# gergely-flamich/relative-entropy-coding

Measured on AMD Instinct MI355X. Metric: encoded latents/sec, higher is better.
Workload: dtype f32

## Files before the change

relative-entropy-coding_amd/csrc/irec_host.cpp:

```cpp
#include <hip/hip_runtime.h>

#include <algorithm>
#include <atomic>
#include <exception>
#include <cfloat>
#include <cmath>
#include <cstdarg>
#include <cstdio>
#include <cstdlib>
#include <cstring>
#include <string>
#include <thread>
#include <vector>

#include "irec_internal.h"
#include "irec_kernels.h"

namespace {

thread_local std::string g_last_error;

irec_status fail(irec_status code, const char *fmt, ...) {
  char buf[512];
  va_list ap;
// ... 85 lines not shown
  const float first = z - logf_det(z) / z;
  const float rz = 1.0f / z;
  const float x_far = first - poly(rz, p2) / poly(rz, q2) / z;
  const float x_tail = first - poly(rz, p1) / poly(rz, q1) / z;
  const float x = sp > lo_cut ? x_centre : (z >= 8.0f ? x_far : x_tail);
  return p > hi_cut ? x : -x;
}

void tf_seed_pair(int64_t global_seed, int64_t op_seed, uint64_t &s1, uint64_t &s2) {
  const int64_t M = 2147483647LL;
  int64_t a = global_seed % M; if (a < 0) a += M;
  int64_t b = op_seed % M;     if (b < 0) b += M;
  if (a == 0 && b == 0) b = M;
  s1 = (uint64_t)a; s2 = (uint64_t)b;
}

struct Philox {
  uint32_t key[2], ctr[4];
  Philox(uint64_t seed1, uint64_t seed2) {
    key[0] = (uint32_t)seed1; key[1] = (uint32_t)(seed1 >> 32);
    ctr[0] = ctr[1] = 0; ctr[2] = (uint32_t)seed2; ctr[3] = (uint32_t)(seed2 >> 32);
  }
  void block(uint64_t index, uint32_t out[4]) const {
    uint32_t c0 = (uint32_t)index, c1 = (uint32_t)(index >> 32), c2 = ctr[2], c3 = ctr[3];
    uint32_t k0 = key[0], k1 = key[1];
    for (int r = 0; r < 10; ++r) {
      const uint64_t a = (uint64_t)0xD2511F53u * c0, b = (uint64_t)0xCD9E8D57u * c2;
      const uint32_t n0 = (uint32_t)(b >> 32) ^ c1 ^ k0, n2 = (uint32_t)(a >> 32) ^ c3 ^ k1;
      c1 = (uint32_t)b; c3 = (uint32_t)a; c0 = n0; c2 = n2;
      k0 += 0x9E3779B9u; k1 += 0xBB67AE85u;
    }
    out[0] = c0; out[1] = c1; out[2] = c2; out[3] = c3;
  }
  uint32_t element(uint64_t e) const {
    uint32_t o[4];
    block(e >> 2, o);
    return o[e & 3];
  }
};

struct MT19937 {
  uint32_t mt[624];
  int idx;
  void init_genrand(uint32_t s) {
    mt[0] = s;
    for (int i = 1; i < 624; ++i) mt[i] = 1812433253u * (mt[i - 1] ^ (mt[i - 1] >> 30)) + (uint32_t)i;
    idx = 624;
  }
  void init_by_array(const std::vector<uint32_t> &key) {
    init_genrand(19650218u);
    size_t i = 1, j = 0;
    for (size_t k = std::max<size_t>(624, key.size()); k; --k) {
      mt[i] = (mt[i] ^ ((mt[i - 1] ^ (mt[i - 1] >> 30)) * 1664525u)) + key[j] + (uint32_t)j;
      if (++i >= 624) { mt[0] = mt[623]; i = 1; }
      if (++j >= key.size()) j = 0;
    }
    for (size_t k = 623; k; --k) {
      mt[i] = (mt[i] ^ ((mt[i - 1] ^ (mt[i - 1] >> 30)) * 1566083941u)) - (uint32_t)i;
      if (++i >= 624) { mt[0] = mt[623]; i = 1; }
    }
    mt[0] = 0x80000000u;
  }
  uint32_t next() {
    if (idx >= 624) {
      for (int k = 0; k < 624; ++k) {
        const uint32_t y = (mt[k] & 0x80000000u) | (mt[(k + 1) % 624] & 0x7fffffffu);
        mt[k] = mt[(k + 397) % 624] ^ (y >> 1) ^ ((y & 1u) ? 0x9908b0dfu : 0u);
      }
      idx = 0;
    }
    uint32_t y = mt[idx++];
    y ^= y >> 11; y ^= (y << 7) & 0x9d2c5680u; y ^= (y << 15) & 0xefc60000u; y ^= y >> 18;
    return y;
  }
};

int64_t py_first_randint31(int64_t seed) {
  const uint64_t a = seed < 0 ? (uint64_t)(-(seed + 1)) + 1u : (uint64_t)seed;
  std::vector<uint32_t> key{(uint32_t)a};
  if (a >> 32) key.push_back((uint32_t)(a >> 32));
  MT19937 g;
  g.init_by_array(key);
  uint32_t r;
  do r = g.next(); while (r >= 0x80000000u);
  return (int64_t)r;
}

inline float u32_to_unit_float(uint32_t x) {
  const uint32_t bits = (127u << 23) | (x & 0x7fffffu);
  float f;
  std::memcpy(&f, &bits, 4);
  return f - 1.0f;
}
inline void box_muller(uint32_t x0, uint32_t x1, float &f0, float &f1) {
  float u1 = u32_to_unit_float(x0);
  if (u1 < 1.0e-7f) u1 = 1.0e-7f;
  const float v1 = (float)(2.0 * 3.14159265358979323846 * (double)u32_to_unit_float(x1));
  const float u2 = std::sqrt(-2.0f * std::log(u1));
  f0 = std::sin(v1) * u2;
  f1 = std::cos(v1) * u2;
}
struct TfNormalStream {
  Philox gen;
  uint64_t have = ~0ull;
  float f[4];
  explicit TfNormalStream(int64_t seed) : gen(0, 0) {
    uint64_t s1, s2;
    tf_seed_pair(seed, py_first_randint31(seed), s1, s2);
    gen = Philox(s1, s2);
  }
  float element(uint64_t e) {
    if ((e >> 2) != have) {
      uint32_t o[4];
      gen.block(e >> 2, o);
      box_muller(o[0], o[1], f[0], f[1]);
      box_muller(o[2], o[3], f[2], f[3]);
      have = e >> 2;
    }
    return f[e & 3];
  }
};

struct TfStatelessNormalStream {
  Philox gen;
  uint64_t have = ~0ull;
  float f[4];
  TfStatelessNormalStream(int64_t seed0, int64_t seed1) : gen(0, 0) {
    const Philox scramble(((uint64_t)0x02461e29u << 32) | 0x3ec8f720u, (uint64_t)seed1);
    uint32_t mix[4];
    scramble.block((uint64_t)seed0, mix);
    gen = Philox(((uint64_t)mix[1] << 32) | mix[0], ((uint64_t)mix[3] << 32) | mix[2]);
  }
  float element(uint64_t e) {
    if ((e >> 2) != have) {
      uint32_t o[4];
      gen.block(e >> 2, o);
      box_muller(o[0], o[1], f[0], f[1]);
      box_muller(o[2], o[3], f[2], f[3]);
      have = e >> 2;
    }
    return f[e & 3];
  }
};

int round_up(int v, int m) { return (v + m - 1) / m * m; }
size_t round_up_sz(size_t v, size_t m) { return (v + m - 1) / m * m; }

}

struct irec_context {
  int device = -1;
  int n_cu = 0;
  int clock_mhz = 0;
  float *d_lut = nullptr;
  float *d_lut2 = nullptr;
  uint16_t *d_dlog4r = nullptr;
  float *d_rho = nullptr;
  int32_t n_rho = IREC_MAX_PARTITIONS;
  unsigned long long *d_dbg = nullptr;
};

namespace irec {
irec_status set_last_error(irec_status code, const char *who, const char *what) { return fail(code, "%s: %s", who, what); }
int context_device(const irec_context *ctx) { return ctx->device; }
int context_cus(const irec_context *ctx) { return ctx->n_cu > 0 ? ctx->n_cu : 256; }
}

extern "C" {

const char *irec_last_error(void) { return g_last_error.c_str(); }
const char *irec_version(void) { return "irec-hip 0.1 (gfx950)"; }

int32_t irec_n_samples(double kl_per_partition, double extra_samples) {
  const double s = std::exp(kl_per_partition * extra_samples);
  if (!(s >= 0.0)) return 0;
  return s >= 2147483647.0 ? INT32_MAX : (int32_t)s;
}

double irec_codelength(int64_t n_indices, int32_t n_samples) { return (double)n_indices * std::log((double)n_samples); }

irec_status irec_build_lut(float *lut) {
  if (!lut) return fail(IREC_E_INVALID, "irec_build_lut: null output");
  lut[0] = 0.0f;
  for (int k = 1; k < IREC_BIG_PRIME; ++k) lut[k] = ndtri_f32((float)k / (float)IREC_BIG_PRIME);
  return IREC_OK;
}

irec_status irec_tf_shuffle_perm(int64_t seed, int64_t n, int64_t *perm) {
  if (n < 0 || (n > 0 && !perm)) return fail(IREC_E_INVALID, "irec_tf_shuffle_perm: bad arguments");
  if (n > 0xFFFFFFFFLL) return fail(IREC_E_INVALID, "irec_tf_shuffle_perm: n too large");
  for (int64_t i = 0; i < n; ++i) perm[i] = i;
  if (n <= 1) return IREC_OK;
  uint64_t s1, s2;
  tf_seed_pair(seed, py_first_randint31(seed), s1, s2);
  const Philox gen(s1, s2);
  uint32_t blk[4];
  for (int64_t i = 0; i < n - 1; ++i) {
    if ((i & 3) == 0) gen.block((uint64_t)i >> 2, blk);
    const int64_t j = i + (int64_t)(blk[i & 3] % (uint32_t)(n - i));
    std::swap(perm[i], perm[j]);
  }
  return IREC_OK;
}

irec_status irec_philox_uniform_int(int64_t seed, int64_t n, int32_t *out) {
  if (n < 0 || (n > 0 && !out)) return fail(IREC_E_INVALID, "irec_philox_uniform_int: bad arguments");
  uint64_t s1, s2;
  tf_seed_pair(seed, seed, s1, s2);
  const Philox gen(s1, s2);
  for (int64_t e = 0; e < n; ++e) out[e] = 1 + (int32_t)(gen.element((uint64_t)e) % (uint32_t)(IREC_BIG_PRIME - 1));
  return IREC_OK;
}

int64_t irec_importance_n_samples(double coding_bits) {
  const float n = std::ceil(std::exp((float)coding_bits * std::log(2.0f)));
  if (!(n >= 1.0f) || !(n < 2147483648.0f)) return -1;
  return (int64_t)n;
}

irec_status irec_tf_random_normal(int64_t seed, int64_t count, float *out) {
  if (count < 0 || (count > 0 && !out)) return fail(IREC_E_INVALID, "irec_tf_random_normal: bad arguments");
  TfNormalStream st(seed);
  for (int64_t e = 0; e < count; ++e) out[e] = st.element((uint64_t)e);
  return IREC_OK;
}

irec_status irec_tf_stateless_normal(int64_t seed0, int64_t seed1, int64_t count, float *out) {
  if (count < 0 || (count > 0 && !out)) return fail(IREC_E_INVALID, "irec_tf_stateless_normal: bad arguments");
  TfStatelessNormalStream st(seed0, seed1);
  for (int64_t e = 0; e < count; ++e) out[e] = st.element((uint64_t)e);
  return IREC_OK;
}

irec_status irec_importance_encode(const float *t_loc, const float *t_scale, const float *p_loc, const float *p_scale,
                                   int64_t n, double coding_bits, double alpha, int64_t seed, int64_t *out_index,
                                   float *out_sample) try {
  if (!t_loc || !t_scale || !p_loc || !p_scale || !out_index || !out_sample || n < 1)
    return fail(IREC_E_INVALID, "irec_importance_encode: bad arguments");
  if (!(alpha >= 1.0)) return fail(IREC_E_INVALID, "Alpha must be in the range [1, inf), but %g was given!", alpha);
  const int64_t S = irec_importance_n_samples(coding_bits);
  if (S < 1) return fail(IREC_E_INVALID, "irec_importance_encode: coding_bits %g gives no valid sample count", coding_bits);
  const float half_log_2pi = (float)(0.5 * std::log(2.0 * 3.14159265358979323846));
  std::vector<float> tl(n), ts(n), ln_t(n);
  for (int64_t d = 0; d < n; ++d) {
    tl[d] = (t_loc[d] - p_loc[d]) / p_scale[d];
    ts[d] = t_scale[d] / p_scale[d];
    ln_t[d] = half_log_2pi + std::log(ts[d]);
  }
  TfNormalStream st(seed);
  const bool gumbel = !std::isinf(alpha);
  TfStatelessNormalStream gst(seed + 1, seed + 2);
  float best = -FLT_MAX;
  int64_t best_s = 0;
  for (int64_t s = 0; s < S; ++s) {
    double acc = 0.0;
    for (int64_t d = 0; d < n; ++d) {
      const float x = st.element((uint64_t)(s * n + d));
      const float dt = x / ts[d] - tl[d] / ts[d];
      const float lp_t = -0.5f * (dt * dt) - ln_t[d];
      const float dp = x / 1.0f - 0.0f / 1.0f;
      const float lp_p = -0.5f * (dp * dp) - (half_log_2pi + 0.0f);
      acc += (double)(lp_t - lp_p);
    }
    float w = (float)acc;
    if (gumbel) w = (float)alpha * w + (-std::log(-std::log(gst.element((uint64_t)s))));
    if (w > best) { best = w; best_s = s; }
  }
  *out_index = best_s;
  for (int64_t d = 0; d < n; ++d) out_sample[d] = p_scale[d] * st.element((uint64_t)(best_s * n + d)) + p_loc[d];
  return IREC_OK;
} catch (const std::exception &e) { return fail(IREC_E_INVALID, "irec_importance_encode: %s", e.what()); }

irec_status irec_importance_decode(const float *p_loc, const float *p_scale, int64_t n, int64_t index, int64_t seed,
                                   float *out_sample) {
  if (!p_loc || !p_scale || !out_sample || n < 1 || index < 0)
    return fail(IREC_E_INVALID, "irec_importance_decode: bad arguments");
  TfNormalStream st(seed);
  for (int64_t d = 0; d < n; ++d) out_sample[d] = p_scale[d] * st.element((uint64_t)(index * n + d)) + p_loc[d];
  return IREC_OK;
}

irec_status irec_create(int device, irec_context **out) { return irec_create_ex(device, nullptr, out); }

irec_status irec_create_ex(int device, const float *lut10007, irec_context **out) {
  irec_tables t{};
  t.lut10007 = lut10007;
  return irec_create_with(device, &t, out);
}

int32_t irec_max_partitions(const irec_context *ctx) { return ctx ? ctx->n_rho : 0; }

irec_status irec_create_with(int device, const irec_tables *tables, irec_context **out) try {
  if (!out) return fail(IREC_E_INVALID, "irec_create: null output");
  *out = nullptr;
  const float *lut10007 = tables ? tables->lut10007 : nullptr;
  const float *aux_ratios = tables ? tables->aux_ratios : nullptr;
  const int32_t n_aux = tables ? tables->n_aux_ratios : 0;
  if (aux_ratios) {
    if (n_aux < 1 || n_aux > IREC_MAX_PARTITIONS) return fail(IREC_E_INVALID, "irec_create_with: n_aux_ratios %d out of range [1, %d]", n_aux, IREC_MAX_PARTITIONS);
    for (int i = 0; i < n_aux; ++i)
      if (!(aux_ratios[i] > 0.0f) || !(aux_ratios[i] <= 1.0f)) return fail(IREC_E_INVALID, "irec_create_with: aux_ratios[%d] is not in (0, 1]", i);
  } else if (n_aux != 0) return fail(IREC_E_INVALID, "irec_create_with: n_aux_ratios without aux_ratios");
  if (lut10007)
    for (int k = 1; k < IREC_BIG_PRIME; ++k)
      if (!std::isfinite(lut10007[k])) return fail(IREC_E_INVALID, "irec_create_ex: lut10007[%d] is not finite", k);
  int count = 0;
  if (hipGetDeviceCount(&count) != hipSuccess || count <= 0)
    return fail(IREC_E_NO_DEVICE, "irec_create: no HIP device visible (this library has no CPU fallback)");
  if (device < 0 || device >= count) return fail(IREC_E_INVALID, "irec_create: device %d out of range (%d)", device, count);
  hipDeviceProp_t prop;
  HIP_TRY(hipGetDeviceProperties(&prop, device));
  if (std::strncmp(prop.gcnArchName, "gfx950", 6) != 0)
    return fail(IREC_E_NO_DEVICE, "irec_create: device %d is %s; this build targets gfx950 only", device, prop.gcnArchName);
  IREC_ON_DEVICE(device);

  const int P = IREC_BIG_PRIME;
  std::vector<float> lut(P);
  if (lut10007) { std::memcpy(lut.data(), lut10007, (size_t)P * sizeof(float)); lut[0] = 0.0f; }
  else irec_build_lut(lut.data());
  auto mulmod = [&](uint32_t a, uint32_t b) { return (uint32_t)(((uint64_t)a * b) % P); };
  uint32_t g = 0;
  std::vector<uint32_t> powers(P - 1);
  for (uint32_t cand = 2; cand < (uint32_t)P && !g; ++cand) {
    uint32_t x = 1;
    bool ok = true;
    std::vector<char> seen(P, 0);
    for (int e = 0; e < P - 1; ++e) {
      if (seen[x]) { ok = false; break; }
      seen[x] = 1; powers[e] = x; x = mulmod(x, cand);
    }
    if (ok) g = cand;
  }
  if (!g) return fail(IREC_E_INVALID, "irec_create: no primitive root found");
  std::vector<float> lut2(P - 1);
  std::vector<uint16_t> dlog4r(P - 1);
  for (int e = 0; e < P - 1; ++e) {
    lut2[e] = lut[powers[e]];
    dlog4r[powers[e] - 1] = (uint16_t)(4 * e);
  }
  std::vector<float> rho(IREC_MAX_PARTITIONS);
  for (int i = 0; i < IREC_MAX_PARTITIONS; ++i)
    rho[i] = (float)std::pow((double)i + 1.0, -0.7864636765648174);
  if (aux_ratios)
    for (int i = 0; i < IREC_MAX_PARTITIONS; ++i) rho[i] = i < n_aux ? aux_ratios[i] : 1.0f;

  irec_context *ctx = new irec_context();
  ctx->device = device;
  ctx->n_cu = prop.multiProcessorCount;
  ctx->clock_mhz = prop.clockRate / 1000;
  ctx->n_rho = aux_ratios ? n_aux : IREC_MAX_PARTITIONS;
  const irec_status st = [&]() -> irec_status {
    HIP_TRY(hipMalloc(&ctx->d_lut, P * sizeof(float)));
    HIP_TRY(hipMalloc(&ctx->d_lut2, (P - 1) * sizeof(float)));
    HIP_TRY(hipMalloc(&ctx->d_dlog4r, (P - 1) * sizeof(uint16_t)));
    HIP_TRY(hipMalloc(&ctx->d_rho, rho.size() * sizeof(float)));
    HIP_TRY(hipMemcpy(ctx->d_lut, lut.data(), P * sizeof(float), hipMemcpyHostToDevice));
    HIP_TRY(hipMemcpy(ctx->d_lut2, lut2.data(), (P - 1) * sizeof(float), hipMemcpyHostToDevice));
    HIP_TRY(hipMemcpy(ctx->d_dlog4r, dlog4r.data(), (P - 1) * sizeof(uint16_t), hipMemcpyHostToDevice));
    HIP_TRY(hipMemcpy(ctx->d_rho, rho.data(), rho.size() * sizeof(float), hipMemcpyHostToDevice));
#ifdef IREC_HOST_STAMPS
    if (const char *e = std::getenv("IREC_STAMPS"); e && e[0] == '1') {
      HIP_TRY(hipMalloc(&ctx->d_dbg, 4096 * 16 * sizeof(unsigned long long)));
    }
#endif
    return IREC_OK;
  }();
  if (st != IREC_OK) { irec_destroy(ctx); return st; }
  *out = ctx;
  return IREC_OK;
} catch (const std::exception &e) { return fail(IREC_E_INVALID, "irec_create: %s", e.what()); }

void irec_destroy(irec_context *ctx) {
  if (!ctx) return;
  DeviceGuard guard_;
  (void)guard_.enter(ctx->device);
  (void)hipFree(ctx->d_lut); (void)hipFree(ctx->d_lut2); (void)hipFree(ctx->d_dlog4r); (void)hipFree(ctx->d_rho);
  (void)hipFree(ctx->d_dbg);
  delete ctx;
}

}

namespace {

struct Plan {
  bool fast;
  bool table;
  bool team;
  bool team_only;
  bool lone;
  bool chunk;
  int shape;
  int grid_cap;
  int one_grid_cap;
  int fast_grid_cap;
  size_t ws_per_wg;
  int dpad;
  int K_tab;
  int n_tab;
  int tab_dim[4];
  size_t tab_off[4];
  size_t tab_bytes;
  int gang_blocks;
  size_t gang_stride, gang_bytes;
};
size_t plan_ws_bytes(const Plan &pl) { return irec::WS_HEAD_BYTES + pl.tab_bytes + (size_t)pl.grid_cap * pl.ws_per_wg + pl.gang_bytes; }

size_t table_steps_that_fit(size_t per_step, bool big = false) {
  const size_t soft = (big ? (size_t)IREC_TABLE_BYTES_BIG : (size_t)IREC_TABLE_BYTES_MAX) / per_step;
  const size_t hard = (big ? (size_t)IREC_TABLE_BYTES_BIG : (size_t)IREC_TABLE_BYTES_HARD) / per_step;
  return std::max(soft, std::min<size_t>((size_t)IREC_TABLE_STEPS_FLOOR, hard));
}

irec_status check_params(const irec_params *p) {
  if (!p) return fail(IREC_E_INVALID, "null irec_params");
  if (!(p->kl_per_partition > 0.0f)) return fail(IREC_E_INVALID, "kl_per_partition must be > 0");
  if (p->n_samples < 1 || p->n_samples > (1 << 24)) return fail(IREC_E_INVALID, "n_samples %d out of range", p->n_samples);
  if (p->n_beams < 1 || p->n_beams > IREC_MAX_BEAMS) return fail(IREC_E_INVALID, "n_beams %d out of range [1,%d]", p->n_beams, IREC_MAX_BEAMS);
  if (p->table_steps < 0) return fail(IREC_E_INVALID, "table_steps %d < 0", p->table_steps);
  { const int sh = (p->flags & IREC_FLAG_SHAPE_MASK) >> IREC_FLAG_SHAPE_SHIFT;
    if (sh > 6 || sh == 1 || sh == 4) return fail(IREC_E_INVALID, "unknown IREC_FLAG_SHAPE_* value"); }
  return IREC_OK;
}

Plan make_plan(const irec_context *ctx, const irec_params *p, int32_t max_dim, int32_t max_K) {
  Plan pl;
  const int B = p->n_beams, S = p->n_samples;
  const int n_cu = ctx->n_cu > 0 ? ctx->n_cu : 256;
  pl.shape = (p->flags & IREC_FLAG_SHAPE_MASK) >> IREC_FLAG_SHAPE_SHIFT;
  pl.dpad = round_up(max_dim > 0 ? max_dim : 1, 256);
  pl.fast = !(p->flags & IREC_FLAG_FORCE_GENERIC) && max_dim <= irec::FAST_MAX_DIM && irec::fast_nb_for(B) != 0 &&
            irec::fast_lds_for(B, S, false) <= irec::FAST_LDS_LIMIT && (int64_t)S * B < (1 << 24);
  pl.grid_cap = 2 * n_cu;
  pl.table = false; pl.team = false; pl.lone = false; pl.chunk = false; pl.n_tab = 0; pl.tab_bytes = 0;
  pl.gang_blocks = 0; pl.gang_stride = 0; pl.gang_bytes = 0;
  const int want = p->table_steps > 0 ? p->table_steps : IREC_TABLE_STEPS_DEFAULT;
  pl.K_tab = std::max(1, std::min(std::min(want, IREC_TABLE_STEPS_MAX), max_K > 0 ? max_K : 1));
  {
    size_t per_step = 0;
    for (int q = 0; q < 4 && p->table_dims[q] > 0; ++q) per_step += (size_t)S * round_up(p->table_dims[q], 4) * 2;
    if (per_step > 0) pl.K_tab = std::max(1, (int)std::min<size_t>((size_t)pl.K_tab, table_steps_that_fit(per_step, max_dim > irec::FAST_MAX_DIM)));
  }
  pl.team_only = !pl.fast && !(p->flags & IREC_FLAG_FORCE_GENERIC) && max_dim <= irec::FAST_MAX_DIM && (int64_t)S * B < (1 << 24) &&
                 !(p->flags & (IREC_FLAG_FUSED_PHILOX | IREC_FLAG_ONE_TABLE)) && irec::team_lds_for(B, S, pl.shape) != (size_t)-1;
  if ((pl.fast || pl.team_only) && !(p->flags & IREC_FLAG_FUSED_PHILOX) && p->table_dims[0] > 0) {
    pl.table = true;
    for (int q = 0; q < 4 && p->table_dims[q] > 0; ++q) {
      if (p->table_dims[q] > irec::FAST_MAX_DIM) { pl.table = false; break; }
      pl.tab_dim[pl.n_tab] = p->table_dims[q];
      pl.tab_off[pl.n_tab] = pl.tab_bytes;
      pl.tab_bytes += round_up_sz((size_t)pl.K_tab * S * round_up(p->table_dims[q], 4) * 2, 256);
      ++pl.n_tab;
    }
    if (!pl.table) { pl.n_tab = 0; pl.tab_bytes = 0; }
    pl.team = pl.table && !(p->flags & IREC_FLAG_ONE_TABLE) && irec::team_lds_for(B, S, pl.shape) != (size_t)-1;
    if (pl.team_only && !pl.team) { pl.table = false; pl.n_tab = 0; pl.tab_bytes = 0; }
    if (pl.team) pl.grid_cap = std::max(irec::team_count_for(B, S, pl.shape), (p->flags & IREC_FLAG_NO_TEN) ? 0 : irec::team_ten_teams(B, S, pl.shape)) * n_cu;
    pl.lone = pl.team && irec::lone_applies(B, pl.shape);
  }
  if (!pl.table) pl.team_only = false;
  pl.chunk = !pl.fast && !pl.team_only && !(p->flags & (IREC_FLAG_FORCE_GENERIC | IREC_FLAG_FUSED_PHILOX | IREC_FLAG_ONE_TABLE)) &&
             p->table_dims[0] > 0 && irec::chunk_applies(B, S, max_dim);
  if (pl.chunk) {
    pl.table = true;
    for (int q = 0; q < 4 && p->table_dims[q] > 0; ++q) {
      if (p->table_dims[q] > max_dim) { pl.table = false; break; }
      pl.tab_dim[pl.n_tab] = p->table_dims[q];
      pl.tab_off[pl.n_tab] = pl.tab_bytes;
      pl.tab_bytes += round_up_sz((size_t)pl.K_tab * S * round_up(p->table_dims[q], 4) * 2, 256);
      ++pl.n_tab;
    }
    if (!pl.table) { pl.chunk = false; pl.n_tab = 0; pl.tab_bytes = 0; }
  }
  auto one_cap = [&](bool table) { return (irec::fast_waves_for(B, S, table) == 8 ? 1 : 2) * n_cu; };
  if (pl.fast) {
    pl.one_grid_cap = one_cap(pl.table);
    pl.fast_grid_cap = pl.table ? one_cap(false) : 0;
    if (!pl.team) pl.grid_cap = pl.one_grid_cap;
    pl.grid_cap = std::max(pl.grid_cap, pl.fast_grid_cap);
    pl.ws_per_wg = round_up_sz(irec::fast_ws_for(B, max_K) + (pl.team ? irec::team_ws_extra_for(B, S, pl.shape) : 0), 256);
    if (pl.team) pl.ws_per_wg = std::max(pl.ws_per_wg, round_up_sz(irec::team_ws_bytes_for(B, S, pl.shape, max_K), 256));
    if (pl.lone) pl.ws_per_wg = std::max(pl.ws_per_wg, round_up_sz(((size_t)n_cu * irec::lone_ws_bytes_per_wg() + pl.grid_cap - 1) / pl.grid_cap, 256));
  } else {
    const size_t generic_ws = round_up_sz((size_t)10 * pl.dpad * 4 + (size_t)3 * B * pl.dpad * 4 +
                                          (size_t)(max_K > 0 ? max_K : 1) * B * 4 + (size_t)S * B * 4, 256);
    if (pl.team_only) {
      pl.one_grid_cap = 0;
      pl.fast_grid_cap = 2 * n_cu;
      pl.grid_cap = std::max(pl.grid_cap, pl.fast_grid_cap);
      pl.ws_per_wg = std::max(generic_ws, round_up_sz(irec::team_ws_bytes_for(B, S, pl.shape, max_K), 256));
    } else if (pl.chunk) {
      pl.one_grid_cap = 0;
      pl.fast_grid_cap = 0;
      pl.ws_per_wg = round_up_sz(irec::chunk_ws_for(B, pl.dpad, max_K), 256);
      const int teams = irec::chunk_teams(B, S);
      const size_t fit = (size_t)IREC_SLAB_BYTES_MAX / pl.ws_per_wg;
      pl.grid_cap = (int)std::max<size_t>((size_t)teams, std::min<size_t>((size_t)teams * n_cu, fit / teams * teams));
      if (const int gnb = irec::chunk_gang_nb(B, S); gnb && irec::chunk_gang_teams(B, S) > 0 && !(p->flags & (IREC_FLAG_NO_SPLIT | IREC_FLAG_MARGINS))) {
        pl.gang_stride = irec::gang_xch_bytes(gnb, S, pl.dpad);
        pl.gang_blocks = (int)std::min<size_t>((size_t)irec::GANG_MAX_BLOCKS, irec::GANG_XCH_BYTES_MAX / pl.gang_stride);
        pl.gang_bytes = (size_t)pl.gang_blocks * pl.gang_stride;
      }
    } else {
      pl.one_grid_cap = pl.grid_cap; pl.fast_grid_cap = 0;
      pl.ws_per_wg = generic_ws;
    }
  }
  if (p->flags & IREC_FLAG_MARGINS) {
    const size_t generic_ws = round_up_sz((size_t)10 * pl.dpad * 4 + (size_t)3 * B * pl.dpad * 4 +
                                          (size_t)(max_K > 0 ? max_K : 1) * B * 4 + (size_t)S * B * 4, 256);
    pl.ws_per_wg = std::max(pl.ws_per_wg, generic_ws);
    pl.grid_cap = std::max(pl.grid_cap, 2 * n_cu);
    if (max_dim > irec::FAST_MAX_DIM)
      pl.grid_cap = (int)std::max<size_t>(1, std::min<size_t>((size_t)pl.grid_cap, (size_t)IREC_SLAB_BYTES_MAX / pl.ws_per_wg));
  }
  if (!pl.table) pl.K_tab = 0;
  return pl;
}

static int chunk_grid(const irec_context *ctx, const Plan &pl, const irec_params *p, int64_t n_blocks);

static int batch_grid(int64_t n_blocks, int cap) {
  const int64_t g = std::min<int64_t>(n_blocks, cap), r = (g + 7) & ~(int64_t)7;
  return (int)(r <= cap ? r : g);
}

static int chunk_grid(const irec_context *ctx, const Plan &pl, const irec_params *p, int64_t n_blocks) {
  const int n_cu = ctx->n_cu > 0 ? ctx->n_cu : 256;
  const int teams = std::max(1, irec::chunk_teams(p->n_beams, p->n_samples));
  return batch_grid(n_blocks, std::min(n_cu, std::max(1, pl.grid_cap / teams)));
}
int gang_width(const irec_context *ctx, const Plan &pl, const irec_params *p, int64_t n_blocks, int32_t max_block_dim, int *grid, int *chunk_owners) {
  if (!pl.chunk || pl.gang_blocks < 1 || n_blocks < 1 || n_blocks > pl.gang_blocks || (p->flags & (IREC_FLAG_NO_SPLIT | IREC_FLAG_MARGINS))) return 0;
  if (!irec::IREC_COOP_GRANULES_ON) return 0;
  const int n_cu = ctx->n_cu > 0 ? ctx->n_cu : 256;
  const int teams = irec::chunk_gang_teams(p->n_beams, p->n_samples);
  if (teams < 1) return 0;
  const int wgs = std::min(n_cu, std::max(1, pl.grid_cap / teams));
  const int64_t slots = (int64_t)wgs * teams;
  const int64_t chunks = ((int64_t)max_block_dim + 1023) >> 10;
  const int64_t GC = std::min(chunks, slots / n_blocks);
  if (GC < 1) return 0;
  const int want = (p->flags & IREC_FLAG_SPLIT_MASK) >> IREC_FLAG_SPLIT_SHIFT;
  const int64_t n_sch = irec::chunk_gang_nb(p->n_beams, p->n_samples) == 32 ? p->n_samples : (p->n_samples + 1) / 2;
  int64_t SP = std::min<int64_t>(wgs / (n_blocks * GC), want >= 1 ? want : IREC_GANG_STRIPES);
  SP = std::max<int64_t>(1, std::min<int64_t>(SP, n_sch));
  SP = (n_sch + (n_sch + SP - 1) / SP - 1) / ((n_sch + SP - 1) / SP);
  const int64_t G = GC * SP;
  if (G < 2) return 0;
  const int64_t n_slots = n_blocks * G;
  if (grid) *grid = (int)std::min<int64_t>(wgs, n_slots);
  if (chunk_owners) *chunk_owners = (int)GC;
  return (int)G;
}

int small_call_blocks(const irec_context *ctx) {
  const int n_cu = ctx->n_cu > 0 ? ctx->n_cu : 256;
  return std::max(8, std::min(irec::COOP_SPLIT_MAX_BLOCKS, n_cu / 4));
}

int split_width(const irec_context *ctx, const Plan &pl, const irec_params *p, int64_t n_blocks) {
  if (!pl.table || pl.chunk || (p->flags & IREC_FLAG_NO_SPLIT)) return 0;
  const int B = p->n_beams, S = p->n_samples, nb = irec::fast_nb_for(B);
  if (!nb || irec::fast_waves_for(B, S, true) != 4 || (int64_t)S * nb > 1024) return 0;
  if (n_blocks < 1 || n_blocks > irec::COOP_SPLIT_MAX_BLOCKS) return 0;
  const int n_cu = ctx->n_cu > 0 ? ctx->n_cu : 256;
  int64_t W = (n_cu / 2) / n_blocks;
  W = std::min<int64_t>(W, S);
  const int want = (p->flags & IREC_FLAG_SPLIT_MASK) >> IREC_FLAG_SPLIT_SHIFT;
  W = std::min<int64_t>(W, want >= 2 ? want : 12);
  return W >= 2 ? (int)W : 0;
}
int split_beam_width(const irec_params *p, int W) {
  if (W < 2) return 0;
  const int B = p->n_beams;
  if (W > B) W = B;
  if (W < 2) return 0;
  const int per = (B + W - 1) / W;
  if (per > 2) return 0;
  while (W > 2 && (B + (W - 1) - 1) / (W - 1) == per) --W;
  return W;
}

bool share_all_auto(const irec_context *ctx, const Plan &pl, const irec_params *p, int64_t n_blocks) {
  if (!pl.team || pl.lone || pl.team_only || pl.chunk || !pl.table || (p->flags & IREC_FLAG_NO_SPLIT)) return false;
  if ((p->flags & IREC_FLAG_SHAPE_MASK) != 0 || n_blocks < small_call_blocks(ctx) || n_blocks > irec::COOP_MAX_BLOCKS) return false;
  const int n_cu = ctx->n_cu > 0 ? ctx->n_cu : 256;
  const int B = p->n_beams, S = p->n_samples;
  if (B > 20 || irec::team_shareable(B, S, 2) != 2 || irec::team_lds_for(B, S, 2) == (size_t)-1 ||
      irec::team_ws_extra_for(B, S, 2) > irec::team_ws_extra_for(B, S, 0) || irec::team_count_for(B, S, 0) < 2)
    return false;
  const int64_t W = std::min<int64_t>(std::min<int64_t>(8, S), 2LL * n_cu / n_blocks);
  if (B <= 10 && !(p->flags & IREC_FLAG_NO_TEN) && irec::ten_applies(B, S)) return false;
  return B > 10 ? W >= 3 : (W >= 2 && n_blocks <= n_cu);
}
int team_share_width(const irec_context *ctx, const Plan &pl, const irec_params *p, int64_t n_blocks, int shape, int64_t *first, int *grid) {
  if (!pl.team || pl.lone || pl.team_only || (p->flags & IREC_FLAG_NO_SPLIT)) return 0;
  const int n_cu = ctx->n_cu > 0 ? ctx->n_cu : 256;
  const int teams = irec::team_shareable(p->n_beams, p->n_samples, shape);
  if (teams < 2) return 0;
  const int want = (p->flags & IREC_FLAG_SPLIT_MASK) >> IREC_FLAG_SPLIT_SHIFT;
  const int64_t cap = std::min<int64_t>(8, p->n_samples);
  const int64_t slots = (int64_t)teams * n_cu;
  int64_t W = 0, f = 0;
  if (shape == 2 && share_all_auto(ctx, pl, p, n_blocks)) {
    if (n_blocks < small_call_blocks(ctx) || n_blocks > irec::COOP_MAX_BLOCKS || 2 * n_blocks > slots) return 0;
    W = slots / n_blocks;
  } else {
    if (p->n_beams <= 10 || n_blocks <= n_cu || n_blocks >= slots || n_blocks - n_cu > irec::COOP_MAX_BLOCKS) return 0;
    f = n_cu;
    W = (slots - n_cu) / (n_blocks - n_cu);
  }
  W = std::min(W, cap);
  if (want >= 2) W = std::min<int64_t>(W, want);
  if (W < 2) return 0;
  const int64_t n_slots = f + (n_blocks - f) * W;
  int64_t g = n_cu;
  if (f == 0) { g = (n_slots + teams - 1) / teams; g = std::min<int64_t>(n_cu, (g + 7) & ~(int64_t)7); }
  if (g * teams < n_slots) return 0;
  if (first) *first = f;
  if (grid) *grid = (int)g;
  return (int)W;
}

int call_teams(const irec_params *p, int shape, int share_W, bool margins) {
  const int tt = (share_W >= 2 || margins || (p->flags & IREC_FLAG_NO_TEN)) ? 0 : irec::team_ten_teams(p->n_beams, p->n_samples, shape);
  return tt ? tt : irec::team_count_for(p->n_beams, p->n_samples, shape);
}
bool team_for_call(const irec_context *ctx, const Plan &pl, const irec_params *p, int64_t n_blocks) {
  return pl.team && (pl.team_only || (p->flags & IREC_FLAG_TEAM) || n_blocks >= small_call_blocks(ctx));
}
int shape_for_call(const irec_context *ctx, const Plan &pl, const irec_params *p, int64_t n_blocks) {
  const int n_cu = ctx->n_cu > 0 ? ctx->n_cu : 256;
  const int B = p->n_beams, S = p->n_samples;
  if (share_all_auto(ctx, pl, p, n_blocks)) return 2;
  if (pl.shape != 0 || !pl.team || pl.lone || n_blocks < small_call_blocks(ctx) || n_blocks > 2 * (int64_t)n_cu || B > 20) return pl.shape;
  if (irec::team_count_for(B, S, 0) < 2) return pl.shape;
  if (n_blocks <= n_cu && B <= 10) return pl.shape;
  if (n_blocks > n_cu) {
    if (irec::team_count_for(B, S, 0) < 3 || irec::team_lds_for(B, S, 2) == (size_t)-1 ||
        irec::team_ws_extra_for(B, S, 2) > irec::team_ws_extra_for(B, S, 0))
      return pl.shape;
    return 2;
  }
  if (irec::team_lds_for(B, S, 5) == (size_t)-1 || irec::team_ws_extra_for(B, S, 5) > irec::team_ws_extra_for(B, S, 0))
    return pl.shape;
  return 5;
}

int margin_team_shape(const irec_context *ctx, const Plan &pl, const irec_params *p, int64_t n_blocks) {
  if (!pl.table || !pl.team || pl.lone || pl.chunk || (p->flags & (IREC_FLAG_FORCE_GENERIC | IREC_FLAG_FUSED_PHILOX | IREC_FLAG_ONE_TABLE))) return -1;
  const int shape = shape_for_call(ctx, pl, p, n_blocks);
  if (irec::team_margin_build(p->n_beams, p->n_samples, shape)) return shape;
  if (irec::team_margin_build(p->n_beams, p->n_samples, pl.shape)) return pl.shape;
  return -1;
}

struct CallDetail {
  int kind = 0;
  int grid = 0;
  int teams = 1;
  int W = 0;
  int coop_beams = 0;
  int gang_chunks = 0;
  int64_t share_first = 0;
  int64_t n_slots = 0;
  int placed = 0;
  int split_blocks = 0;
};
CallDetail call_detail(const irec_context *ctx, const Plan &pl, const irec_params *p, int64_t n_blocks, int32_t max_block_dim, bool margins) {
  CallDetail d;
  const int n_cu = ctx->n_cu > 0 ? ctx->n_cu : 256;
  d.n_slots = n_blocks;
  if (pl.table && !pl.team && split_width(ctx, pl, p, n_blocks) >= 2) d.split_blocks = (int)n_blocks;
  int share_grid = 0;
  const int share_W = (pl.table && pl.team) ? team_share_width(ctx, pl, p, n_blocks, pl.shape, &d.share_first, &share_grid) : 0;
  if (share_W >= 2) d.split_blocks = (int)(n_blocks - d.share_first);
  if (pl.chunk && gang_width(ctx, pl, p, n_blocks, max_block_dim, nullptr, nullptr) >= 2) d.split_blocks = (int)n_blocks;
  if (pl.table && pl.chunk) {
    d.kind = 1;
    d.teams = std::max(1, irec::chunk_teams(p->n_beams, p->n_samples));
    d.grid = chunk_grid(ctx, pl, p, n_blocks);
    int ggrid = 0, gchunks = 0;
    if (const int G = gang_width(ctx, pl, p, n_blocks, max_block_dim, &ggrid, &gchunks)) {
      d.W = G; d.gang_chunks = gchunks; d.grid = ggrid; d.n_slots = n_blocks * G;
      d.teams = std::max(1, irec::chunk_gang_teams(p->n_beams, p->n_samples));
    }
  } else if (pl.table && pl.team && pl.lone) {
    d.kind = 2; d.grid = batch_grid(n_blocks, n_cu); d.teams = irec::lone_waves();
  } else if (pl.table && pl.team) {
    d.kind = 3;
    d.teams = call_teams(p, pl.shape, share_W, margins);
    d.grid = batch_grid(n_blocks, std::min(pl.grid_cap / d.teams, n_cu));
    if (share_W >= 2) {
      d.W = share_W; d.grid = share_grid; d.n_slots = d.share_first + (n_blocks - d.share_first) * share_W;
    }
    if (!pl.lone && !pl.chunk && !(p->flags & IREC_FLAG_LISTED_ORDER) && n_blocks <= irec::COST_MAX_ROWS) {
      const int n_teams = irec::team_count_for(p->n_beams, p->n_samples, pl.shape);
      const int64_t tg = share_W >= 2 ? share_grid : batch_grid(n_blocks, std::min(pl.grid_cap / n_teams, n_cu));
      if (n_blocks > tg && d.n_slots <= tg * n_teams && n_teams == 2 && p->n_beams > 10 && irec::team_placeable(p->n_beams, p->n_samples, pl.shape)) d.placed = 1;
    }
  } else if (pl.table) {
    d.kind = 4;
    d.grid = (int)std::min<int64_t>(n_blocks, pl.one_grid_cap);
    int W = split_width(ctx, pl, p, n_blocks);
    if (const int wb = split_beam_width(p, W)) { W = wb; d.coop_beams = 1; }
    if (W >= 2) { d.W = W; d.grid = (int)(n_blocks * W); d.n_slots = n_blocks * W; }
  } else if (pl.fast) {
    d.kind = 5; d.grid = (int)std::min<int64_t>(n_blocks, pl.one_grid_cap);
  } else {
    d.kind = 6;
    d.grid = margins ? (int)std::min<int64_t>(n_blocks, std::min(pl.grid_cap, 2 * n_cu)) : (int)std::min<int64_t>(n_blocks, pl.grid_cap);
  }
  return d;
}

}

extern "C" {

size_t irec_encode_workspace_bytes(const irec_context *ctx, const irec_params *p, int32_t max_dim, int32_t max_K) {
  if (!ctx || check_params(p) != IREC_OK || max_dim < 1 || max_K < 0) return 0;
  const Plan pl = make_plan(ctx, p, max_dim, max_K);
  return plan_ws_bytes(pl);
}

size_t irec_encode_workspace_bytes_for(const irec_context *ctx, const irec_params *p, int64_t n_blocks, int32_t max_dim, int32_t max_K) {
  if (!ctx || check_params(p) != IREC_OK || max_dim < 1 || max_K < 0 || n_blocks < 0) return 0;
  irec_params pm = *p;
  if (pm.flags & IREC_FLAG_MARGINS) pm.flags |= IREC_FLAG_NO_SPLIT;
  Plan pl = make_plan(ctx, &pm, max_dim, max_K);
  if (pl.chunk && !(pm.flags & IREC_FLAG_MARGINS) && n_blocks > 0) {
    const int teams = std::max(1, irec::chunk_teams(pm.n_beams, pm.n_samples));
    int grid = chunk_grid(ctx, pl, &pm, n_blocks), ggrid = 0;
    int gteams = teams;
    if (gang_width(ctx, pl, &pm, n_blocks, max_dim, &ggrid, nullptr) >= 2) { grid = ggrid; gteams = std::max(1, irec::chunk_gang_teams(pm.n_beams, pm.n_samples)); }
    pl.grid_cap = std::min(pl.grid_cap, std::max(teams, grid * std::max(teams, gteams)));
  }
  return plan_ws_bytes(pl);
}

irec_status irec_encode_plan(const irec_context *ctx, const irec_params *p, int64_t n_blocks, int32_t max_block_dim,
                             int32_t max_K, irec_plan_info *out) {
  if (!ctx || !out) return fail(IREC_E_INVALID, "irec_encode_plan: null argument");
  if (irec_status s = check_params(p)) return s;
  if (n_blocks < 0 || max_block_dim < 1 || max_K < 0) return fail(IREC_E_INVALID, "irec_encode_plan: bad sizes");
  irec_params pm = *p;
  if (pm.flags & IREC_FLAG_MARGINS) { pm.flags |= IREC_FLAG_NO_SPLIT; p = &pm; }
  const Plan pl = make_plan(ctx, p, max_block_dim, max_K);
  const bool team = team_for_call(ctx, pl, p, n_blocks);
  std::memset(out, 0, sizeof(*out));
  const int B = p->n_beams, S = p->n_samples;
  if (p->flags & IREC_FLAG_MARGINS) {
    const int n_cu = ctx->n_cu > 0 ? ctx->n_cu : 256;
    const int mshape = margin_team_shape(ctx, pl, p, n_blocks);
    if (mshape >= 0) {
      const int n_teams = irec::team_count_for(B, S, mshape);
      std::string nm = irec::team_kernel_name(B, S, mshape);
      nm.insert(nm.size() - 1, ",margins");
      std::snprintf(out->kernel, sizeof out->kernel, "%s", nm.c_str());
      std::snprintf(out->table_kernel, sizeof out->table_kernel, "prep_kernel (copy bits)");
      out->grid = batch_grid(n_blocks, std::min(pl.grid_cap / n_teams, n_cu));
      out->waves_per_wg = irec::team_waves_for(B, S, mshape);
      out->teams_per_wg = n_teams;
      out->lds_bytes = (int32_t)irec::team_lds_for(B, S, mshape);
      out->table_steps = pl.K_tab; out->n_tables = pl.n_tab; out->table_bytes = (int64_t)pl.tab_bytes;
    } else {
      std::snprintf(out->kernel, sizeof out->kernel, "encode_generic_kernel (margins)");
      out->grid = (int32_t)std::min<int64_t>(n_blocks, std::min(pl.grid_cap, 2 * n_cu));
      out->waves_per_wg = 4; out->teams_per_wg = 1;
      out->lds_bytes = (int32_t)irec::generic_lds_bytes();
    }
    out->n_cu = ctx->n_cu; out->clock_mhz = ctx->clock_mhz;
    out->workspace_bytes = (int64_t)plan_ws_bytes(pl);
    return IREC_OK;
  }
  if (pl.chunk) {
    std::snprintf(out->kernel, sizeof out->kernel, "%s", irec::chunk_kernel_name(B, S));
    std::snprintf(out->table_kernel, sizeof out->table_kernel, "prep_kernel (copy bits)");
    out->grid = chunk_grid(ctx, pl, p, n_blocks);
    {
      int ggrid = 0;
      out->split = gang_width(ctx, pl, p, n_blocks, max_block_dim, &ggrid, nullptr);
      if (out->split >= 2) out->grid = ggrid;
    }
    out->waves_per_wg = irec::chunk_teams(B, S) * 4;
    out->teams_per_wg = irec::chunk_teams(B, S);
    out->lds_bytes = (int32_t)irec::chunk_lds_for(B, S);
    if (out->split >= 2) {
      std::snprintf(out->kernel, sizeof out->kernel, "%s", irec::chunk_gang_kernel_name(B, S));
      out->teams_per_wg = irec::chunk_gang_teams(B, S); out->waves_per_wg = out->teams_per_wg * 4;
      out->lds_bytes = (int32_t)irec::chunk_gang_lds_for(B, S);
    }
  } else if (team && pl.lone) {
    const int n_cu = ctx->n_cu > 0 ? ctx->n_cu : 256;
    std::snprintf(out->kernel, sizeof out->kernel, "%s", irec::lone_kernel_name());
    std::snprintf(out->table_kernel, sizeof out->table_kernel, "prep_kernel (copy bits)");
    out->grid = batch_grid(n_blocks, n_cu);
    out->waves_per_wg = irec::lone_waves();
    out->teams_per_wg = irec::lone_waves();
    out->lds_bytes = (int32_t)irec::lone_lds_bytes();
  } else if (team) {
    const int shape = shape_for_call(ctx, pl, p, n_blocks);
    const int n_teams = irec::team_count_for(B, S, shape);
    const int n_cu = ctx->n_cu > 0 ? ctx->n_cu : 256;
    std::snprintf(out->kernel, sizeof out->kernel, "%s", irec::team_kernel_name(B, S, shape));
    std::snprintf(out->table_kernel, sizeof out->table_kernel, "prep_kernel (copy bits)");
    out->grid = batch_grid(n_blocks, std::min(pl.grid_cap / n_teams, n_cu));
    {
      int sgrid = 0;
      out->split = team_share_width(ctx, pl, p, n_blocks, shape, nullptr, &sgrid);
      if (out->split >= 2) out->grid = sgrid;
    }
    out->waves_per_wg = irec::team_waves_for(B, S, shape);
    out->teams_per_wg = n_teams;
    out->lds_bytes = (int32_t)irec::team_lds_for(B, S, shape);
    if (const int tt = irec::team_ten_teams(B, S, shape); tt && out->split < 2 && !(p->flags & IREC_FLAG_NO_TEN)) {
      std::snprintf(out->kernel, sizeof out->kernel, "encode_ten_kernel<%d>", tt);
      out->lds_bytes = (int32_t)irec::ten_lds_for(tt);
      out->teams_per_wg = tt; out->waves_per_wg = 4 * tt;
      out->grid = batch_grid(n_blocks, std::min(pl.grid_cap / tt, n_cu));
    }
  } else if (pl.fast) {
    std::snprintf(out->kernel, sizeof out->kernel, "%s", irec::fast_kernel_name(B, S, pl.table));
    if (pl.table) std::snprintf(out->table_kernel, sizeof out->table_kernel, "prep_kernel (plain rows)");
    out->grid = (int32_t)std::min<int64_t>(n_blocks, pl.one_grid_cap);
    out->split = split_width(ctx, pl, p, n_blocks);
    if (const int wb = split_beam_width(p, out->split)) { out->split = wb; out->split_beams = 1; }
    if (out->split >= 2) {
      out->grid = (int32_t)(n_blocks * out->split);
      std::snprintf(out->kernel, sizeof out->kernel, "encode_fast_kernel<%d,%d,true,%d>", irec::fast_nb_for(B),
                    out->split_beams ? irec::fast_split_beam_waves(B) : 4, out->split_beams ? 2 : 1);
    }
    out->waves_per_wg = (out->split >= 2 && out->split_beams) ? irec::fast_split_beam_waves(B) : irec::fast_waves_for(B, S, pl.table);
    out->teams_per_wg = 1;
    out->lds_bytes = (int32_t)irec::fast_lds_for(B, S, pl.table) + (out->split >= 2 && out->split_beams ? 40024 : 0);
  } else {
    std::snprintf(out->kernel, sizeof out->kernel, "encode_generic_kernel");
    out->grid = (int32_t)std::min<int64_t>(n_blocks, pl.grid_cap);
    out->waves_per_wg = 4;
    out->teams_per_wg = 1;
    out->lds_bytes = (int32_t)irec::generic_lds_bytes();
  }
  out->table_steps = pl.K_tab;
  out->n_tables = pl.n_tab;
  out->n_cu = ctx->n_cu;
  out->clock_mhz = ctx->clock_mhz;
  out->table_bytes = (int64_t)pl.tab_bytes;
  out->workspace_bytes = (int64_t)plan_ws_bytes(pl);
  return IREC_OK;
}

irec_status irec_test_plan(int32_t n_cu, int32_t clock_mhz, const irec_params *p, int64_t n_blocks, int32_t max_block_dim, int32_t max_K,
                           irec_plan_info *info, irec_plan_detail *detail) {
  if (!info || !detail || n_cu < 1) return fail(IREC_E_INVALID, "irec_test_plan: bad argument");
  irec_context fake;
  fake.n_cu = n_cu; fake.clock_mhz = clock_mhz;
  if (irec_status st = irec_encode_plan(&fake, p, n_blocks, max_block_dim, max_K, info)) return st;
  const bool margins = (p->flags & IREC_FLAG_MARGINS) != 0;
  irec_params pm = *p;
  if (margins) pm.flags |= IREC_FLAG_NO_SPLIT;
  Plan pl = make_plan(&fake, &pm, max_block_dim, max_K);
  const int mshape = margins ? margin_team_shape(&fake, pl, &pm, n_blocks) : -1;
  if (margins && mshape < 0) { pl.table = false; pl.team = false; pl.lone = false; pl.chunk = false; pl.fast = false; pl.team_only = false; pl.n_tab = 0; pl.K_tab = 0; }
  pl.team = mshape >= 0 ? true : team_for_call(&fake, pl, &pm, n_blocks);
  if (mshape >= 0) pl.shape = mshape;
  else if (pl.team) pl.shape = shape_for_call(&fake, pl, &pm, n_blocks);
  const CallDetail cd = call_detail(&fake, pl, &pm, n_blocks, max_block_dim, margins);
  std::memset(detail, 0, sizeof(*detail));
  detail->kind = cd.kind; detail->grid = cd.grid; detail->teams_per_wg = cd.teams; detail->coop_width = cd.W; detail->coop_beams = cd.coop_beams;
  detail->gang_chunks = cd.gang_chunks; detail->placed = cd.placed; detail->split_blocks = cd.split_blocks;
  detail->share_first = cd.share_first; detail->n_slots = cd.n_slots;
  detail->slabs_in_workspace = pl.grid_cap; detail->slab_bytes = (int64_t)pl.ws_per_wg;
  detail->fixed_bytes = (int64_t)(irec::WS_HEAD_BYTES + pl.tab_bytes + pl.gang_bytes);
  detail->exchange_rows = irec::COOP_MAX_BLOCKS; detail->exchange_keys = irec::COOP_KEYS;
  return IREC_OK;
}

irec_status irec_block_kl(irec_context *ctx, const irec_params *p, int64_t n_blocks, const int64_t *block_base,
                          const int32_t *block_pos, const int32_t *block_dim, const int32_t *perm, const float *q_loc,
                          const float *q_scale, const float *p_loc, const float *p_scale, float *out_kl, int32_t *out_K,
                          void *hip_stream) {
  if (!ctx) return fail(IREC_E_INVALID, "irec_block_kl: null context");
  if (irec_status s = check_params(p)) return s;
  if (n_blocks < 0) return fail(IREC_E_INVALID, "irec_block_kl: n_blocks < 0");
  if (n_blocks == 0) return IREC_OK;
  if (!block_base || !block_pos || !block_dim || !q_loc || !q_scale || !p_loc || !p_scale || !out_K)
    return fail(IREC_E_INVALID, "irec_block_kl: null pointer argument");
  IREC_ON_DEVICE(ctx->device);
  irec::EncArgs A{};
  A.block_base = block_base; A.block_pos = block_pos; A.block_dim = block_dim; A.perm = perm;
  A.q_loc = q_loc; A.q_scale = q_scale; A.p_loc = p_loc; A.p_scale = p_scale;
  A.n_blocks = n_blocks; A.omega = p->kl_per_partition; A.S = p->n_samples; A.B = p->n_beams; A.out_K = out_K;
  A.K_limit = ctx->n_rho;
  const int grid = (int)std::min<int64_t>(n_blocks, 8LL * ctx->n_cu);
  HIP_TRY(irec::launch_block_kl(A, out_kl, grid, (hipStream_t)hip_stream));
  return IREC_OK;
}

irec_status irec_beam_encode(irec_context *ctx, const irec_params *p, int64_t n_blocks, const int64_t *block_base,
                             const int32_t *block_pos, const int32_t *block_dim, int32_t max_block_dim,
                             const int32_t *perm, const float *q_loc, const float *q_scale, const float *p_loc,
                             const float *p_scale, int64_t seed, int32_t max_K, int32_t *out_K, int32_t *out_indices,
                             float *out_sample, void *workspace, size_t workspace_bytes, void *hip_stream) {
  if (p && (p->flags & IREC_FLAG_MARGINS)) return fail(IREC_E_INVALID, "irec_beam_encode: IREC_FLAG_MARGINS needs irec_beam_encode_ex (out_margin)");
  return irec_beam_encode_ex(ctx, p, n_blocks, block_base, block_pos, block_dim, max_block_dim, perm, q_loc, q_scale, p_loc, p_scale, seed,
                             max_K, out_K, out_indices, out_sample, nullptr, workspace, workspace_bytes, hip_stream);
}

irec_status irec_beam_encode_ex(irec_context *ctx, const irec_params *p, int64_t n_blocks, const int64_t *block_base,
                                const int32_t *block_pos, const int32_t *block_dim, int32_t max_block_dim,
                                const int32_t *perm, const float *q_loc, const float *q_scale, const float *p_loc,
                                const float *p_scale, int64_t seed, int32_t max_K, int32_t *out_K, int32_t *out_indices,
                                float *out_sample, float *out_margin, void *workspace, size_t workspace_bytes, void *hip_stream) {
  if (!ctx) return fail(IREC_E_INVALID, "irec_beam_encode: null context");
  if (irec_status s = check_params(p)) return s;
  if (((p->flags & IREC_FLAG_MARGINS) != 0) != (out_margin != nullptr))
    return fail(IREC_E_INVALID, "irec_beam_encode_ex: out_margin and IREC_FLAG_MARGINS go together (the flag sizes the workspace)");
  irec_params pm = *p;
  if (out_margin) { pm.flags |= IREC_FLAG_NO_SPLIT; p = &pm; }
  if (n_blocks < 0) return fail(IREC_E_INVALID, "irec_beam_encode: n_blocks < 0");
  if (n_blocks > 0x7FFF0000ll) return fail(IREC_E_INVALID, "irec_beam_encode: more than 2^31 - 65536 blocks in one call");
  if (n_blocks == 0) return IREC_OK;
  if (!block_base || !block_pos || !block_dim || !q_loc || !q_scale || !p_loc || !p_scale || !out_K || !out_sample)
    return fail(IREC_E_INVALID, "irec_beam_encode: null pointer argument");
  if (max_K < 0 || max_K > IREC_MAX_PARTITIONS) return fail(IREC_E_INVALID, "irec_beam_encode: max_K %d out of range", max_K);
  if (max_K > 0 && !out_indices) return fail(IREC_E_INVALID, "irec_beam_encode: null out_indices");
  if (max_block_dim < 1 || max_block_dim > (1 << 22)) return fail(IREC_E_INVALID, "irec_beam_encode: max_block_dim %d out of range", max_block_dim);
  Plan pl = make_plan(ctx, p, max_block_dim, max_K);
  size_t need = plan_ws_bytes(pl);
  if (workspace && workspace_bytes < need && pl.chunk && !out_margin) {
    const int teams = std::max(std::max(1, irec::chunk_teams(p->n_beams, p->n_samples)), std::max(1, irec::chunk_gang_teams(p->n_beams, p->n_samples)));
    const size_t fixed = irec::WS_HEAD_BYTES + pl.tab_bytes + pl.gang_bytes;
    const size_t fit = workspace_bytes > fixed ? (workspace_bytes - fixed) / pl.ws_per_wg : 0;
    if (fit >= (size_t)teams) { pl.grid_cap = (int)std::min<size_t>((size_t)pl.grid_cap, fit / teams * teams); need = plan_ws_bytes(pl); }
  }
  if (!workspace || workspace_bytes < need)
    return fail(IREC_E_WORKSPACE, "irec_beam_encode: workspace %zu bytes < required %zu", workspace_bytes, need);
  const int mshape = out_margin ? margin_team_shape(ctx, pl, p, n_blocks) : -1;
  if (out_margin && mshape < 0) { pl.table = false; pl.team = false; pl.lone = false; pl.chunk = false; pl.fast = false; pl.team_only = false; pl.n_tab = 0; pl.K_tab = 0; }
  pl.team = mshape >= 0 ? true : team_for_call(ctx, pl, p, n_blocks);
  if (((uintptr_t)workspace & 255) != 0) return fail(IREC_E_WORKSPACE, "irec_beam_encode: workspace must be 256-byte aligned");
  IREC_ON_DEVICE(ctx->device);
  hipStream_t st = (hipStream_t)hip_stream;
  irec::EncArgs A{};
  A.block_base = block_base; A.block_pos = block_pos; A.block_dim = block_dim; A.perm = perm;
  A.q_loc = q_loc; A.q_scale = q_scale; A.p_loc = p_loc; A.p_scale = p_scale;
  A.n_blocks = n_blocks; A.seed = seed;
  A.omega = p->kl_per_partition; A.S = p->n_samples; A.B = p->n_beams; A.max_K = max_K;
  A.K_limit = ctx->n_rho;
  A.out_K = out_K; A.out_indices = out_indices; A.out_sample = out_sample;
  A.lut = ctx->d_lut; A.lut2 = ctx->d_lut2; A.dlog4r = ctx->d_dlog4r; A.rho = ctx->d_rho;
  A.counter = (unsigned int *)workspace;
  A.xcd_counter = (unsigned int *)workspace + irec::WS_XCD_WORD;
  A.defer_count = (unsigned int *)workspace + 1;
  if (mshape >= 0) pl.shape = mshape;
  else if (pl.team) pl.shape = shape_for_call(ctx, pl, p, n_blocks);
  A.K_tab = pl.K_tab; A.deferred_pass = 0; A.shape_override = pl.shape; A.no_ten = (p->flags & IREC_FLAG_NO_TEN) ? 1 : 0;
  A.coop_W = 1; A.coop_err = (unsigned int *)workspace + 3; A.coop_arrive = (unsigned int *)workspace + 64;
  A.coop_xch = (uint32_t *)((char *)workspace + irec::WS_COUNTER_BYTES);
  A.ws = (char *)workspace + irec::WS_HEAD_BYTES + pl.tab_bytes;
  A.ws_per_wg = pl.ws_per_wg;
  A.max_dim_pad = pl.dpad;
  A.out_margin = out_margin;
  irec::TableStamps stamps{};
  if (pl.table)
    for (int q = 0; q < pl.n_tab; ++q) {
      uint32_t *w = stamps.w[q];
      w[0] = 0x7ab1e000u | ((pl.team || pl.chunk) ? 1u : 2u);
      w[1] = (uint32_t)(uint64_t)seed; w[2] = (uint32_t)((uint64_t)seed >> 32);
      w[3] = (uint32_t)p->n_samples; w[4] = (uint32_t)pl.tab_dim[q]; w[5] = (uint32_t)pl.K_tab;
      w[6] = (uint32_t)pl.tab_off[q];
      w[7] = ~(w[1] ^ w[2] ^ w[3] ^ w[4] ^ w[5] ^ w[6]);
    }
  stamps.reuse = (p->flags & IREC_FLAG_REUSE_TABLES) ? 1 : 0;
  const CallDetail cd = call_detail(ctx, pl, p, n_blocks, max_block_dim, out_margin != nullptr);
  const int split_blocks = cd.split_blocks;
  if (cd.placed) A.row_cost = (const uint32_t *)((char *)workspace + irec::WS_COUNTER_BYTES + irec::WS_XCH_BYTES);
  int grid = (int)std::min<int64_t>(n_blocks, pl.one_grid_cap);
  A.dbg = nullptr;
#ifdef IREC_HOST_STAMPS
  A.dbg = ctx->d_dbg;
  if (ctx->d_dbg) HIP_TRY(hipMemsetAsync(ctx->d_dbg, 0, 4096 * 16 * sizeof(unsigned long long), st));
#endif
  irec::PrepArgs P{};
  P.head = (uint32_t *)workspace; P.ts = stamps;
  P.n_granule = irec::IREC_COOP_GRANULES_ON && split_blocks > 0 ? std::min(split_blocks, irec::COOP_MAX_BLOCKS) : 0;
  P.n_cost = A.row_cost ? (int32_t)n_blocks : 0;
  P.cost = const_cast<uint32_t *>(A.row_cost);
  P.seed = seed; P.S = p->n_samples; P.K_tab = pl.K_tab; P.dlog4r = ctx->d_dlog4r;
  A.ws_head = (uint32_t *)workspace;
  for (int q = 0; q < 4; ++q) { A.tab[q] = nullptr; A.tab_dim[q] = -1; }
  if (pl.table) {
    for (int q = 0; q < pl.n_tab; ++q) {
      uint16_t *tab = (uint16_t *)((char *)workspace + irec::WS_HEAD_BYTES + pl.tab_off[q]);
      A.tab[q] = tab; A.tab_dim[q] = pl.tab_dim[q];
      P.jobs.tab[q] = tab; P.jobs.keep[q] = nullptr;
    }
    if (pl.n_tab > 0 && !(p->flags & IREC_FLAG_TABLES_PRESENT)) {
      P.table_kind = (pl.team || pl.chunk) ? 1 : 2;
      P.n_table_wgs = (int32_t)irec::prep_table_wgs(P.table_kind, p->n_samples, pl.K_tab, pl.n_tab, pl.tab_dim, &P.jobs);
    }
  }
  HIP_TRY(irec::launch_prep(P, A, st));
  if (pl.table) {
    auto deferred_pass = [&]() -> irec_status {
      if (pl.K_tab >= max_K) return IREC_OK;
      irec::EncArgs A2 = A;
      A2.deferred_pass = 1; A2.coop_W = 1;
      A2.counter = (unsigned int *)workspace + 2;
      for (int q = 0; q < 4; ++q) { A2.tab[q] = nullptr; A2.tab_dim[q] = -1; }
      if (out_margin) HIP_TRY(irec::launch_encode_generic(A2, (int)std::min<int64_t>(n_blocks, std::min(pl.grid_cap, 2 * (ctx->n_cu > 0 ? ctx->n_cu : 256))), st));
      else if (pl.team_only || pl.chunk) HIP_TRY(irec::launch_encode_generic(A2, (int)std::min<int64_t>(n_blocks, pl.fast_grid_cap), st));
      else HIP_TRY(irec::launch_encode_fast(A2, false, (int)std::min<int64_t>(n_blocks, pl.fast_grid_cap), st));
      return IREC_OK;
    };
    if (pl.chunk) {
      const int cgrid = cd.grid;
      if (cd.W >= 2) {
        A.coop_W = cd.W; A.gang_chunks = cd.gang_chunks;
        A.gang_xch = (char *)workspace + irec::WS_HEAD_BYTES + pl.tab_bytes + (size_t)pl.grid_cap * pl.ws_per_wg;
        A.gang_stride = pl.gang_stride;
        A.coop_test_orphan = (p->flags & IREC_FLAG_TEST_SPLIT_ORPHAN) ? 1 : 0;
      }
      HIP_TRY(irec::launch_encode_chunk(A, cgrid, st));
    } else if (pl.team && pl.lone) {
      HIP_TRY(irec::launch_encode_lone(A, cd.grid, st));
      if (irec_status s2 = deferred_pass()) return s2;
#ifdef IREC_HOST_STAMPS
      if (ctx->d_dbg) {
        const int lgrid = batch_grid(n_blocks, ctx->n_cu > 0 ? ctx->n_cu : 256), nwv = irec::lone_waves();
        std::vector<unsigned long long> h((size_t)lgrid * nwv * 16);
        HIP_TRY(hipStreamSynchronize(st));
        HIP_TRY(hipMemcpy(h.data(), ctx->d_dbg, h.size() * sizeof(unsigned long long), hipMemcpyDeviceToHost));
        static const char *nm[6] = {"prologue (fetch, KL)", "step constants", "scoring", "selection", "update", "epilogue"};
        double sum[6] = {0}, tot = 0;
        for (size_t w = 0; w < (size_t)lgrid * nwv; ++w) for (int k = 0; k < 6; ++k) { sum[k] += (double)h[w * 16 + k]; tot += (double)h[w * 16 + k]; }
        fprintf(stderr, "[irec lone stamps] share of wave time:\n");
        for (int k = 0; k < 6; ++k) fprintf(stderr, "  %-22s %5.1f%%\n", nm[k], 100 * sum[k] / tot);
        fprintf(stderr, "  cycles per wave: %.0f\n", tot / (lgrid * nwv));
        return IREC_OK;
      }
#endif
    } else if (pl.team) {
      const int tgrid = cd.grid;
#ifdef IREC_HOST_STAMPS
      const int n_teams = cd.teams;
#endif
      if (cd.W >= 2) {
        A.coop_W = cd.W; A.tsplit_first = cd.share_first;
        A.coop_test_orphan = (p->flags & IREC_FLAG_TEST_SPLIT_ORPHAN) ? 1 : 0;
      }
      if (out_margin) HIP_TRY(irec::launch_encode_team_margin(A, tgrid, st));
      else HIP_TRY(irec::launch_encode_team(A, tgrid, st));
#ifndef IREC_HOST_STAMPS
      if (irec_status s2 = deferred_pass()) return s2;
#else
      if (!ctx->d_dbg) { if (irec_status s2 = deferred_pass()) return s2; }
      if (ctx->d_dbg) {
        const bool ten_call = !cd.W && !out_margin && !(p->flags & IREC_FLAG_NO_TEN) && irec::team_ten_teams(p->n_beams, p->n_samples, pl.shape) != 0;
        const int nwv = ten_call ? 4 * n_teams : irec::team_waves_for(p->n_beams, p->n_samples, pl.shape);
        std::vector<unsigned long long> h((size_t)tgrid * nwv * 16);
        HIP_TRY(hipStreamSynchronize(st));
        HIP_TRY(hipMemcpy(h.data(), ctx->d_dbg, h.size() * sizeof(unsigned long long), hipMemcpyDeviceToHost));
        static const char *nm[12] = {"fetch", "prologue", "scoring", "wait-score", "combine", "select", "update-tail", "wait-update", "epilogue",
                                     "upd:sel+issue+consts", "upd:batches", "-"};
        const int nwt = nwv / n_teams;
        double w0[12] = {0}, wo[12] = {0}, t0 = 0, to = 0;
        int n0 = 0, no = 0;
        for (int w = 0; w < tgrid * nwv; ++w) {
          if (h[(size_t)w * 16 + 1] == 0ull) continue;
          if ((w % nwt) == 0) ++n0; else ++no;
          for (int k = 0; k < 12; ++k) { const double v = (double)h[(size_t)w * 16 + k]; if ((w % nwt) == 0) { w0[k] += v; t0 += v; } else { wo[k] += v; to += v; } }
        }
        fprintf(stderr, "[irec team stamps] %d of %d teams coded blocks; share of wave time (cycles per wave), wave 0 of a team | the others:\n", n0, tgrid * n_teams);
        t0 -= w0[11]; to -= wo[11];
        for (int k = 0; k < 11; ++k) fprintf(stderr, "  %-20s %5.1f%% (%8.0f) | %5.1f%% (%8.0f)\n", nm[k], 100 * w0[k] / t0, w0[k] / (n0 ? n0 : 1), 100 * wo[k] / to, wo[k] / (no ? no : 1));
        fprintf(stderr, "  cycles per wave: %.0f | %.0f;  block-steps per wave: %.2f;  cycles per block-step: %.0f\n", t0 / (n0 ? n0 : 1), to / (no ? no : 1),
                w0[11] / (n0 ? n0 : 1), w0[11] > 0 ? t0 / w0[11] : 0.0);
        {
          double life_max = 0, life_sum = 0, life_min = 1e300;
          int nlife = 0;
          for (int w = 0; w < tgrid * nwv; ++w) {
            const double v = (double)h[(size_t)w * 16 + 12];
            if (v <= 0) continue;
            life_max = std::max(life_max, v); life_min = std::min(life_min, v); life_sum += v; ++nlife;
          }
          if (nlife) fprintf(stderr, "  idle tail: %.1f%% of the grid's wave-time lies behind a wave's exit (first exit at %.1f%% of the longest lifetime)\n",
                             100.0 * (1.0 - life_sum / (nlife * life_max)), 100.0 * life_min / life_max);
        }
        if (h[13]) fprintf(stderr, "  shader clock of workgroup 0, wave 0: %.0f MHz over %.3f ms (s_memtime / s_memrealtime)\n",
                           100.0 * (double)h[12] / (double)h[13], (double)h[13] / 1e5);
        return IREC_OK;
      }
#endif
    } else {
      const int W = cd.W;
      A.coop_beams = cd.coop_beams;
      if (W >= 2) {
        A.coop_W = W;
        A.coop_test_orphan = (p->flags & IREC_FLAG_TEST_SPLIT_ORPHAN) ? 1 : 0;
        HIP_TRY(irec::launch_encode_fast(A, true, cd.grid, st));
#ifdef IREC_HOST_STAMPS
        if (ctx->d_dbg) grid = cd.grid;
#endif
      } else HIP_TRY(irec::launch_encode_fast(A, true, grid, st));
      if (irec_status s2 = deferred_pass()) return s2;
    }
  } else if (pl.fast) {
    HIP_TRY(irec::launch_encode_fast(A, false, grid, st));
  } else {
    if (out_margin) grid = (int)std::min<int64_t>(n_blocks, std::min(pl.grid_cap, 2 * (ctx->n_cu > 0 ? ctx->n_cu : 256)));
    HIP_TRY(irec::launch_encode_generic(A, grid, st));
  }
#ifdef IREC_HOST_STAMPS
  if (ctx->d_dbg) {
    std::vector<unsigned long long> h((size_t)grid * 16);
    HIP_TRY(hipStreamSynchronize(st));
    HIP_TRY(hipMemcpy(h.data(), ctx->d_dbg, h.size() * sizeof(unsigned long long), hipMemcpyDeviceToHost));
    double sum[16] = {0};
    for (int w = 0; w < grid; ++w) for (int k = 0; k < 16; ++k) sum[k] += (double)h[(size_t)w * 16 + k];
    const double tot = sum[0] + sum[1] + sum[2] + sum[3];
    {
      int zero = 0; unsigned long long t0 = ~0ull, late = 0;
      for (int w = 0; w < grid; ++w) { if (h[(size_t)w * 16 + 4] == 0) ++zero; else if (h[(size_t)w * 16 + 5] < t0) t0 = h[(size_t)w * 16 + 5]; }
      for (int w = 0; w < grid; ++w) if (h[(size_t)w * 16 + 4] && h[(size_t)w * 16 + 5] - t0 > 100000ull) ++late;
      fprintf(stderr, "[irec stamps] census: %d of %d workgroups coded no block, %llu started > 1 ms after the first\n", zero, grid, late);
    }
    fprintf(stderr, "[irec stamps] top-B detail cycles/WG: combine %.0f, wait-for-keys barrier %.0f, wave-0 select %.0f, closing barrier %.0f\n",
            sum[11] / grid, sum[8] / grid, sum[9] / grid, sum[10] / grid);
    if (sum[12] + sum[13] + sum[14] > 0)
      fprintf(stderr, "[irec stamps] split exchange cycles/WG: publish %.0f, wait for partners %.0f, read back %.0f\n",
              sum[12] / grid, sum[13] / grid, sum[14] / grid);
    fprintf(stderr, "[irec stamps] waves/workgroup %d, LDS %zu B\n",
            irec::fast_waves_for(p->n_beams, p->n_samples, pl.table), irec::fast_lds_for(p->n_beams, p->n_samples, pl.table));
    fprintf(stderr, "[irec stamps] %s grid=%d cycles/WG: prologue %.0f (%.1f%%) scoring %.0f (%.1f%%) select %.0f (%.1f%%) update %.0f (%.1f%%)\n",
            pl.table ? "table" : pl.fast ? "fused" : "generic", grid, sum[0] / grid, 100 * sum[0] / tot, sum[1] / grid,
            100 * sum[1] / tot, sum[2] / grid, 100 * sum[2] / tot, sum[3] / grid, 100 * sum[3] / tot);
  }
#endif
  return IREC_OK;
}

struct DecPlan { int upb; int K_tab; int n_tab; int tab_dim[4]; size_t tab_off[4]; size_t bytes; };
static DecPlan make_dec_plan(const irec_params *p, int64_t n_blocks, int32_t max_block_dim, int32_t max_K, bool have_ws) {
  DecPlan d{};
  int maxd = max_block_dim;
  for (int q = 0; q < 4 && p->table_dims[q] > 0; ++q) maxd = std::max(maxd, p->table_dims[q]);
  d.upb = maxd > 0 ? (maxd + 255) / 256 : 0;
  if (!have_ws || p->table_dims[0] <= 0 || max_K < 1 || (p->flags & IREC_FLAG_FUSED_PHILOX)) return d;
  if (n_blocks >= 0 && (int64_t)p->n_samples > 2 * n_blocks) return d;
  size_t per_step = 0;
  for (int q = 0; q < 4 && p->table_dims[q] > 0; ++q) per_step += (size_t)p->n_samples * round_up(p->table_dims[q], 4) * 2;
  const int want = p->table_steps > 0 ? p->table_steps : IREC_TABLE_STEPS_DEFAULT;
// ... 299 lines not shown
```

relative-entropy-coding_amd/csrc/irec_internal.h:

```cpp
#ifndef IREC_INTERNAL_H_
#define IREC_INTERNAL_H_

#include "irec.h"

#ifdef __cplusplus
extern "C" {
#endif

#define IREC_FLAG_FUSED_PHILOX 2
#define IREC_FLAG_ONE_TABLE 4
#define IREC_FLAG_TEAM 8
#define IREC_FLAG_TEST_SPLIT_ORPHAN 32
#define IREC_FLAG_LISTED_ORDER 262144
#define IREC_FLAG_NO_TEN 1048576
#define IREC_FLAG_SPLIT_SHIFT 12
#define IREC_FLAG_SPLIT_MASK (0xF << IREC_FLAG_SPLIT_SHIFT)
#define IREC_FLAG_SHAPE_SHIFT 8
#define IREC_FLAG_SHAPE_MASK (0xF << IREC_FLAG_SHAPE_SHIFT)
#define IREC_FLAG_SHAPE_2 (2 << IREC_FLAG_SHAPE_SHIFT)
#define IREC_FLAG_SHAPE_3 (3 << IREC_FLAG_SHAPE_SHIFT)
#define IREC_FLAG_SHAPE_1X2 (5 << IREC_FLAG_SHAPE_SHIFT)
#define IREC_FLAG_SHAPE_TEAM (6 << IREC_FLAG_SHAPE_SHIFT)


typedef struct {
  int32_t kind, grid, teams_per_wg;
  int32_t coop_width;
  int32_t coop_beams, gang_chunks;
  int32_t placed;
  int32_t split_blocks;
  int64_t share_first, n_slots;
  int64_t slabs_in_workspace, slab_bytes, fixed_bytes;
  int32_t exchange_rows, exchange_keys;
} irec_plan_detail;
irec_status irec_test_plan(int32_t n_cu, int32_t clock_mhz, const irec_params *p, int64_t n_blocks, int32_t max_block_dim, int32_t max_K,
                           irec_plan_info *info, irec_plan_detail *detail);
irec_status irec_tf_random_normal(int64_t seed, int64_t count, float *out);
irec_status irec_tf_stateless_normal(int64_t seed0, int64_t seed1, int64_t count, float *out);

int32_t irec_test_fit_chunk(int32_t chunk);
irec_status irec_test_det_exp(const double *in, int64_t n, double *out);

irec_status irec_shim_stats(irec_context *ctx, const float *y, const float *infer_heads, float *out, int32_t n_stats, int32_t n,
                            int32_t channels_y, int32_t channels_infer, int32_t stochastic, int32_t hw, const float *bias_y,
                            const float *bias_infer, void *hip_stream);
irec_status irec_shim_cat_elu(irec_context *ctx, const float *y, const float *latent, float *out, int32_t n, int32_t channels_y,
                              int32_t channel_offset, int32_t deterministic, int32_t stochastic, int32_t hw, const float *bias_y,
                              void *hip_stream);
irec_status irec_shim_residual_elu(irec_context *ctx, const float *input, const float *tensor, float alpha, float *out, float *out_elu,
                                   int32_t n, int32_t channels, int32_t hw, const float *bias_tensor, void *hip_stream);

irec_status irec_device_uniform_int(irec_context *ctx, int64_t seed, int64_t n, int32_t *out, void *hip_stream);
irec_status irec_test_decoder_sqrt(irec_context *ctx, uint64_t *out2, void *hip_stream);
irec_status irec_test_reduce_scatter(irec_context *ctx, const float *in, float *out, int32_t width, void *hip_stream);
irec_status irec_test_select(irec_context *ctx, const float *scores, int32_t n, int32_t n_select, int32_t n_beams_cur,
                             uint32_t *scratch_keys, int32_t *out_sel, void *hip_stream);
irec_status irec_test_select_quick(irec_context *ctx, const float *scores, int32_t n, int32_t n_select, int32_t n_beams_cur,
                                   uint32_t *scratch_keys, int32_t *out_sel, void *hip_stream);
irec_status irec_test_proposal_table(irec_context *ctx, int64_t seed, int32_t n_samples, int32_t dim, int32_t n_steps,
                                     uint16_t *out_tab, void *hip_stream);
irec_status irec_device_tables(irec_context *ctx, const float **lut, const float **lut2, const uint16_t **dlog4r,
                               const float **rho);

#ifdef __cplusplus
}
#endif
#endif
```

relative-entropy-coding_amd/csrc/irec_kernels.h:

```cpp
#pragma once
#include <hip/hip_runtime.h>
#include <stddef.h>
#include <stdint.h>

#define IREC_MAX_PARTITIONS_DEV 65536

namespace irec {

constexpr int FAST_NW = 4;
constexpr int FAST_MAX_DIM = 1024;
constexpr size_t FAST_LDS_LIMIT = 160 * 1024;

struct EncArgs {
  const int64_t *block_base; const int32_t *block_pos; const int32_t *block_dim; const int32_t *perm;
  const float *q_loc, *q_scale, *p_loc, *p_scale;
  int64_t n_blocks; int64_t seed;
  float omega; int32_t S, B, max_K;
  int32_t K_limit;
  int32_t *out_K; int32_t *out_indices; float *out_sample;
  const float *lut;
  const float *lut2;
  const uint16_t *dlog4r;
  const float *rho;
  unsigned int *counter; char *ws; size_t ws_per_wg; int32_t max_dim_pad;
  unsigned int *xcd_counter;
  const uint16_t *tab[4]; int32_t tab_dim[4];
  int32_t K_tab; int32_t deferred_pass; unsigned int *defer_count;
  int32_t shape_override;
  int32_t no_ten;
  int32_t coop_W; unsigned int *coop_arrive; uint32_t *coop_xch; unsigned int *coop_err;
  int64_t tsplit_first;
  const uint32_t *row_cost;
  uint32_t *ws_head;
  char *gang_xch; size_t gang_stride;
  int32_t gang_chunks;
  int32_t coop_beams;
  int32_t coop_test_orphan;
  float *out_margin;
  unsigned long long *dbg;
};

struct DecArgs {
  const int64_t *block_base; const int32_t *block_pos; const int32_t *block_dim; const int32_t *perm;
  const float *p_loc, *p_scale;
  int64_t n_blocks; int64_t seed;
  int32_t max_K; const int32_t *K; const int32_t *indices; float *out_sample;
  int32_t K_limit;
  const float *lut; const float *rho;
  int32_t upb; int32_t S; int32_t K_tab;
  const float *lut2; const uint16_t *dlog4r;
  const uint16_t *tab[4]; int32_t tab_dim[4];
  int64_t n_tensors; int32_t tn, tbs, tbpt; const int32_t *block_row;
};

hipError_t launch_block_kl(const EncArgs &A, float *out_kl, int grid, hipStream_t st);
size_t generic_lds_bytes();
hipError_t launch_encode_generic(const EncArgs &A, int grid, hipStream_t st);
int fast_nb_for(int B);
size_t fast_lds_for(int B, int S, bool table);
size_t fast_ws_for(int B, int max_K);
size_t fast_ws_bytes_nb(int NB, int max_K);
hipError_t launch_encode_fast(const EncArgs &A, bool table, int grid, hipStream_t st);
int fast_waves_for(int B, int S, bool table);
int fast_split_beam_waves(int B);
hipError_t launch_alpha_table(int64_t seed, int32_t S, int32_t D, int32_t K_tab, const uint16_t *dlog4r, uint16_t *tab,
                              const uint32_t *keep, hipStream_t st);
int team_count_for(int B, int S, int shape_override);
int team_shareable(int B, int S, int shape_override);
bool team_placeable(int B, int S, int shape_override);
int team_waves_for(int B, int S, int shape_override);
size_t team_ws_extra_for(int B, int S, int shape_override);
size_t team_ws_bytes_for(int B, int S, int shape_override, int max_K);
size_t team_lds_for(int B, int S, int shape_override);
hipError_t launch_encode_team(const EncArgs &A, int grid, hipStream_t st);
bool team_margin_build(int B, int S, int shape_override);
hipError_t launch_encode_team_margin(const EncArgs &A, int grid, hipStream_t st);
const char *team_kernel_name(int B, int S, int shape_override);
const char *fast_kernel_name(int B, int S, bool table);
hipError_t launch_alpha_choice(int64_t seed, int32_t S, int32_t D, int32_t K_tab, const uint16_t *dlog4r, uint16_t *tab,
                               const uint32_t *keep, hipStream_t st);
hipError_t launch_alpha_choice_all(int64_t seed, int32_t S, int32_t K_tab, const uint16_t *dlog4r, int n, const int32_t *dims,
                                   uint16_t *const *tabs, const uint32_t *const *keeps, hipStream_t st);
bool ten_applies(int B, int S);
size_t ten_lds_for(int teams);
hipError_t launch_encode_ten(const EncArgs &A, int teams, int grid, hipStream_t st);
int team_ten_teams(int B, int S, int shape_override);
bool chunk_applies(int B, int S, int max_dim);
int chunk_teams(int B, int S);
size_t chunk_lds_for(int B, int S);
size_t chunk_ws_for(int B, int dpad, int max_K);
const char *chunk_kernel_name(int B, int S);
int chunk_gang_teams(int B, int S);
int chunk_gang_nb(int B, int S);
size_t chunk_gang_lds_for(int B, int S);
const char *chunk_gang_kernel_name(int B, int S);
hipError_t launch_encode_chunk_gang(const EncArgs &A, int grid, hipStream_t st);
hipError_t launch_encode_chunk(const EncArgs &A, int grid, hipStream_t st);
bool lone_applies(int B, int shape_override);
int lone_waves();
size_t lone_lds_bytes();
size_t lone_ws_bytes_per_wg();
const char *lone_kernel_name();
hipError_t launch_encode_lone(const EncArgs &A, int grid, hipStream_t st);
constexpr int WS_KEEP_WORD = 8, WS_STAMP_WORD = 16, WS_STAMP_WORDS = 8, WS_XCD_WORD = 128, WS_XCD_STRIDE = 64;
constexpr int WS_PENDING_WORD = 132;
struct TableStamps { uint32_t w[4][WS_STAMP_WORDS]; int32_t reuse; };
struct ChoiceJobs { int32_t D[4]; uint16_t *tab[4]; const uint32_t *keep[4]; int64_t hw_end[4]; int32_t n; };
struct PrepArgs {
  uint32_t *head; TableStamps ts;
  int32_t n_granule, n_cost, n_table_wgs, table_kind;
  int64_t seed; int32_t S, K_tab; const uint16_t *dlog4r; ChoiceJobs jobs; uint32_t *cost;
};
hipError_t launch_prep(const PrepArgs &P, const EncArgs &A, hipStream_t st);
int64_t prep_table_wgs(int kind, int32_t S, int32_t K_tab, int n, const int32_t *dims, ChoiceJobs *jobs);
constexpr size_t WS_COUNTER_BYTES = 512 + 8 * 256;
constexpr int COOP_MAX_BLOCKS = 384, COOP_KEYS = 1024;
constexpr unsigned long long COOP_GIVE_UP_TICKS = 10000000ull;
constexpr int COOP_SPLIT_MAX_BLOCKS = 64;
#ifndef IREC_COOP_GRANULES
#define IREC_COOP_GRANULES 1
#endif
constexpr bool IREC_COOP_GRANULES_ON = IREC_COOP_GRANULES != 0;
constexpr size_t WS_XCH_BYTES = (size_t)2 * COOP_MAX_BLOCKS * COOP_KEYS * 8;
__host__ __device__ inline size_t gang_xch_bytes(int nb, int S, int dpad) {
  const size_t NGm = (size_t)4 * (((size_t)dpad + 1023) >> 10), NC_ = (size_t)S * nb;
  return (4 * NGm * (NC_ + nb) + 8 * NGm + 4 * NC_ + 255) & ~(size_t)255;
}
#ifndef IREC_GANG_STRIPES
#define IREC_GANG_STRIPES 9
#endif
constexpr int GANG_MAX_BLOCKS = COOP_MAX_BLOCKS;
constexpr size_t GANG_XCH_BYTES_MAX = (size_t)1 << 30;
constexpr int COST_MAX_ROWS = 1024;
constexpr size_t WS_COST_BYTES = (size_t)COST_MAX_ROWS * 4;
constexpr size_t WS_HEAD_BYTES = WS_COUNTER_BYTES + WS_XCH_BYTES + WS_COST_BYTES;
hipError_t launch_decode(const DecArgs &A, int n_cu, hipStream_t st);
int decode_tensor_waves(int n, int bs, bool table, size_t *lds_out);
hipError_t launch_shim_stats(const float *y, const float *inf, float *out, int n_stats, int N, int Cy, int Ci, int s, int HW,
                             const float *by, const float *bi, hipStream_t st);
hipError_t launch_shim_cat_elu(const float *y, const float *latent, float *out, int N, int Cy, int c_off, int d, int s, int HW,
                               const float *by, hipStream_t st);
hipError_t launch_shim_residual_elu(const float *inp, const float *t, float alpha, float *out, float *out_elu, int64_t count,
                                    const float *bt, int C, int HW, hipStream_t st);
constexpr int GC_MAX_DIM = 1024;
struct GcArgs {
  const int64_t *block_base; const int32_t *block_pos; const int32_t *block_dim; const int32_t *perm;
  const float *q_loc, *q_scale, *p_loc, *p_scale;
  int64_t n_blocks;
  int32_t S, S_pad, steps, max_K;
  int32_t K_limit;
  const float *rho;
  const float *tab[4]; int32_t tab_dim[4];
  int32_t *out_K; int32_t *out_indices;
  const int32_t *K; const int32_t *indices;
  float *out_sample;
};
int gc_encode_threads(int S);
hipError_t launch_gc_importance_encode(const GcArgs &A, int grid, hipStream_t st);
hipError_t launch_gc_importance_decode(const GcArgs &A, int grid, hipStream_t st);
hipError_t launch_dec_sqrt_test(unsigned long long *out, hipStream_t st);
hipError_t launch_uniform_int(int64_t seed, int64_t n, int32_t *out, hipStream_t st);
hipError_t launch_select_test(const float *scores, int N, int Bnew, int Bcur, uint32_t *keys, int32_t *sel, bool quick, hipStream_t st);
hipError_t launch_reduce_scatter_test(const float *in, float *out, int width, hipStream_t st);

}
```

relative-entropy-coding_amd/csrc/irec_team.hip:

```cpp
#include <hip/hip_runtime.h>
#include <algorithm>
#include <stdint.h>
#include <stdio.h>

#include "irec_device.h"
#include "irec_kernels.h"
#include "irec_fast_common.h"
#include "irec_team_common.h"

#ifndef IREC_GANG_ABLATE
#define IREC_GANG_ABLATE 0
#endif
#ifndef IREC_PK_ADDR
#define IREC_PK_ADDR 1
#endif
#if defined(IREC_TEAM_MARGIN_TU) || defined(IREC_TEAM_GANG_TU)
#define IREC_TEAM_AUX_TU 1
#endif
namespace irec {

__host__ __device__ constexpr int team_mb(int NB) { return NB <= 32 ? 32 : 64; }
template <int NB> using TeamLdsT = SmallLdsT<(NB <= 32 ? 32 : 64), (NB <= 32 ? 32 : 64), (NB <= 32 ? 64 : 512)>;
__host__ __device__ inline size_t team_small_bytes(int NB) {
  return NB <= 32 ? ((sizeof(TeamLdsT<32>) + 15) & ~(size_t)15) : ((sizeof(TeamLdsT<64>) + 15) & ~(size_t)15);
}
__host__ __device__ inline int team_row(int NB, int B) { return (NB == 10 && B == 1) ? 1 : NB; }
__host__ __device__ inline size_t team_key_bytes(int ps, int S) { return (((size_t)S * ps * 4) + 15) & ~(size_t)15; }
__host__ __device__ inline bool team_keys_in_lds(int NB, int S, int teams, bool passes, int ps = 0) {
  if (ps <= 0) ps = NB;
  const long long avail = (long long)((FAST_LDS_LIMIT - T3_BYTES) / (size_t)teams) - (long long)team_key_bytes(ps, S) -
                          (long long)team_small_bytes(NB) - 32;
  return (teams > 1 && !passes) || avail / (4LL * ps * 4) >= (S < 16 ? S : 16);
}
__host__ __device__ inline bool team_keys_alias(int NB, int teams) { return teams >= 3 && NB == 20; }
__host__ __device__ inline int team_s_pass(int NB, int S, int teams, int cmax, bool passes = false, int ps = 0) {
  if (ps <= 0) ps = NB;
  const long long avail = (long long)((FAST_LDS_LIMIT - T3_BYTES) / (size_t)teams) -
                          ((team_keys_in_lds(NB, S, teams, passes, ps) && !(team_keys_alias(NB, teams) && !passes)) ? (long long)team_key_bytes(ps, S) : 0) -
                          (long long)team_small_bytes(NB) - 32;
  long long fit = avail / (4LL * ps * 4);
  if (fit > cmax / ps) fit = cmax / ps;
  if (fit < 1) return 0;
  if (fit >= S) return S;
  const int n_pass = (int)((S + fit - 1) / fit);
  return (S + n_pass - 1) / n_pass;
}
__host__ __device__ inline size_t team_part_bytes(int ps, int SP) { return (((size_t)4 * SP * ps * 4) + 15) & ~(size_t)15; }
__host__ __device__ inline size_t team_lds_one(int NB, int S, int SP, int teams, bool passes = false, int ps = 0) {
  if (ps <= 0) ps = NB;
  return team_part_bytes(ps, SP) + ((team_keys_in_lds(NB, S, teams, passes, ps) && !(team_keys_alias(NB, teams) && !passes)) ? team_key_bytes(ps, S) : 0) +
         team_small_bytes(NB) + 16;
}
__host__ __device__ inline size_t team_lds_total(int NB, int S, int SP, int teams, bool passes = false, int ps = 0) {
  return T3_BYTES + (size_t)teams * team_lds_one(NB, S, SP, teams, passes, ps);
}

#ifdef IREC_TEAM_STAMPS
#define TSTAMP(slot) do { const unsigned long long now_ = __builtin_amdgcn_s_memtime(); st_acc[slot] += now_ - st_prev; st_prev = now_; } while (0)
#else
#define TSTAMP(slot) do { } while (0)
#endif

template <int NB, int TEAMS, int BS, bool PASSES = false, bool ONE = false, bool SHARE = false, bool MARGIN = false>
__global__ __launch_bounds__(TEAMS * BS * TEAM_NT, 1) void encode_team_kernel(EncArgs A) {
  using TeamLds = TeamLdsT<NB>;
  constexpr int TEAM_MB = team_mb(NB);
  constexpr size_t TEAM_SMALL_BYTES = (sizeof(TeamLds) + 15) & ~(size_t)15;
  constexpr bool MULTI_PASS = TEAMS == 1 || PASSES;
  constexpr bool SHORT = TEAMS * BS >= 3 && NB / BS == 20;
  constexpr int NW = TEAM_NW;
  constexpr int NWT = TEAM_NW * BS, NT = 64 * NWT;
  constexpr int NBW = NB / BS;
  static_assert(NB % BS == 0, "beam stripes must divide the beam count");
  static_assert(NBW == 10 || NBW == 16 || NBW == 18 || NBW == 20, "the team encoder is built for 10, 16, 18 or 20 beams per wave");
  static_assert(NB <= TEAM_MB && NB <= 64, "beam indices are lane indices and 6-bit back-pointers");
  constexpr int CMAX = TEAMS == 1 ? 2048 : 1024;
  constexpr int SPC = BS >= 2 ? 1 : 20 / NBW;
  constexpr int RW = NBW * SPC;
  constexpr int ACC_ROOM = rsn_room(RW);
  extern __shared__ __attribute__((aligned(16))) char smem[];
  const int S = A.S, B = A.B;
  const int lane = threadIdx.x & 63;
  const int wave_wg = __builtin_amdgcn_readfirstlane((int)(threadIdx.x >> 6));
  const int team = wave_wg / NWT, wave_t = wave_wg % NWT;
  const int wave = wave_t & 3, bs = wave_t >> 2;
  const int b_lo = bs * NBW;
  const int tid = (int)threadIdx.x - team * NT;
  const int PS = NB == 10 ? team_row(NB, B) : NB;
  const int SP = MULTI_PASS ? team_s_pass(NB, S, TEAMS, CMAX, PASSES, PS) : S;
  const bool keys_lds = !MULTI_PASS || team_keys_in_lds(NB, S, TEAMS, PASSES, PS);
  constexpr bool KEYS_ALIAS = TEAMS >= 3 && NB == 20 && !PASSES;
  const size_t key_lds_bytes = (keys_lds && !KEYS_ALIAS) ? team_key_bytes(PS, S) : 0;
  char *tbase = smem + T3_BYTES + (size_t)team * team_lds_one(NB, S, SP, TEAMS, PASSES, PS);
  float *part_s = reinterpret_cast<float *>(tbase);
  TeamLds *sm = reinterpret_cast<TeamLds *>(tbase + team_part_bytes(PS, SP) + key_lds_bytes);
  uint32_t *bar_word = reinterpret_cast<uint32_t *>(tbase + team_part_bytes(PS, SP) + key_lds_bytes + TEAM_SMALL_BYTES);
  double *gpart = sm->gpart;
  int32_t *sel_s = sm->sel_s, *sel_b = sm->sel_b;
  int32_t *hsum = &sm->hsum[0][0];
  uint32_t *beta4 = &sm->beta4[0][0];
  int32_t *misc = sm->misc;
  float *cpart_s = &sm->cpart[0][0];
  const uint16_t *dlog_s = A.dlog4r;
  const int rs_p = rsn_owner<RW>(lane);
  const int rs_p20 = RW == 20 ? rs20_owner(lane) : -1;
  const int rs_c = rsn_owner<NBW>(lane);

  if ((uint32_t)(uintptr_t)(__attribute__((address_space(3))) char *)smem != 0u) __builtin_trap();
  commit_table_stamps(A);
  constexpr bool CAN_SHARE = SHARE && TEAMS >= 2 && BS == 1 && !PASSES && !ONE;
  const int Wsh = (CAN_SHARE && A.coop_W > 1) ? A.coop_W : 1;
  const int64_t n_whole = Wsh > 1 ? (A.tsplit_first < A.n_blocks ? A.tsplit_first : A.n_blocks) : A.n_blocks;
  const int64_t n_slots = n_whole + (A.n_blocks - n_whole) * Wsh;
  const int64_t n_static = (int64_t)TEAMS * (int64_t)gridDim.x < n_slots ? (int64_t)TEAMS * (int64_t)gridDim.x : n_slots;
  constexpr bool CAN_PLACE = NB == 20 && TEAMS == 2 && BS == 1 && !PASSES && !ONE;
  const bool placed = CAN_PLACE && A.row_cost != nullptr && n_static == n_slots;
  const int64_t lo_rank = (int64_t)gridDim.x < n_whole ? (int64_t)gridDim.x : n_whole;
  int32_t placed_row = -1;
  if (placed) {
    uint32_t *cs = reinterpret_cast<uint32_t *>(smem);
    const int n = (int)A.n_blocks;
    for (int k = (int)threadIdx.x; k < n; k += TEAMS * NT) cs[k] = A.row_cost[k];
    if ((int)threadIdx.x < TEAMS) cs[n + (int)threadIdx.x] = 0xFFFFFFFFu;
    int want[TEAMS];
#pragma unroll
    for (int tm = 0; tm < TEAMS; ++tm) {
      const int64_t u = (int64_t)tm * (int64_t)gridDim.x + (int64_t)blockIdx.x;
      want[tm] = u >= n_static ? -1 : u < lo_rank ? (int)u : n - 1 - (int)((u - lo_rank) / (u < n_whole ? 1 : Wsh));
    }
    __syncthreads();
    for (int i = (int)threadIdx.x; i < n; i += TEAMS * NT) {
      const uint32_t ci = cs[i];
      int rk = 0;
#pragma unroll 8
      for (int j = 0; j < n; ++j) rk += cs[j] < ci ? 1 : 0;
#pragma unroll
      for (int tm = 0; tm < TEAMS; ++tm)
        if (rk == want[tm]) cs[n + tm] = (uint32_t)i;
    }
    __syncthreads();
    placed_row = (int32_t)cs[n + team];
    __syncthreads();
  }
  {
    float *l3 = reinterpret_cast<float *>(smem);
    for (int k = (int)threadIdx.x; k < (int)IREC_PM1; k += TEAMS * NT) {
      const float v = A.lut2[k];
      l3[k] = v; l3[k + IREC_PM1] = v; l3[k + 2 * IREC_PM1] = v;
    }
    if (tid == 0) *bar_word = 0u;
  }
  __syncthreads();
  TeamBarrier tsync{bar_word, 0u, (uint32_t)NWT};

  char *slab = A.ws + ((size_t)blockIdx.x * TEAMS + team) * A.ws_per_wg;
  const size_t key_glb_bytes = keys_lds ? 0 : ((team_key_bytes(PS, S) + 255) & ~(size_t)255);
  uint32_t *key_s = KEYS_ALIAS ? reinterpret_cast<uint32_t *>(tbase)
                    : keys_lds ? reinterpret_cast<uint32_t *>(tbase + team_part_bytes(PS, SP))
                               : reinterpret_cast<uint32_t *>(slab + A.ws_per_wg - key_glb_bytes);
  int32_t *bp = reinterpret_cast<int32_t *>(slab);
  float *beams_g = reinterpret_cast<float *>(slab + A.ws_per_wg - key_glb_bytes - (size_t)2 * NB * FAST_MAX_DIM * 4);
  float *stats_g = beams_g - 3 * FAST_MAX_DIM;
  float *park_g = stats_g - 2 * FAST_MAX_DIM;
  constexpr bool PARK = SHORT;
  constexpr bool LATE_G = false;

#ifdef IREC_TEAM_STAMPS
  unsigned long long st_acc[12] = {0, 0, 0, 0, 0, 0, 0, 0, 0, 0, 0, 0};
  unsigned long long st_prev = __builtin_amdgcn_s_memtime();
  const unsigned long long st_t0 = st_prev, st_r0 = __builtin_amdgcn_s_memrealtime();
#endif
  bool first_block = true;
  int steal = 0;
  for (;;) {
    tsync();
    if (tid == 0) {
      int64_t r;
      if (first_block) {
        r = (int64_t)team * (int64_t)gridDim.x + (int64_t)blockIdx.x;
        r = r < n_static ? (placed ? r : xcd_static_row(r, n_static, (int)gridDim.x)) : n_slots;
      } else r = placed ? n_slots : xcd_pull_row(A, n_static, n_slots, steal);
      misc[0] = (int32_t)r;
      misc[6] = 0;
    }
    first_block = false;
    tsync();
    const int64_t slot = misc[0];
    TSTAMP(0);
    if (slot >= n_slots) break;
    int64_t blk = slot < n_whole ? slot : n_whole + (slot - n_whole) / Wsh;
    const int64_t xrow = slot < n_whole ? 0 : (slot - n_whole) / Wsh;
    const int qsh = slot < n_whole ? 0 : (int)((slot - n_whole) % Wsh);
    const int Wrow = slot < n_whole ? 1 : Wsh;
    if (placed) {
      blk = placed_row;
      if (blk < 0 || blk >= A.n_blocks) __builtin_trap();
    }
    if (Wrow > 1 && A.coop_test_orphan && qsh != 0) continue;
    const int D = A.block_dim[blk];
    const int64_t base = A.block_base[blk];
    const int32_t pos = A.block_pos[blk];
    const uint16_t *tab = nullptr;
#pragma unroll
    for (int q = 0; q < 4; ++q)
      if (A.tab_dim[q] == D) tab = A.tab[q];
    if (D < 1 || D > FAST_MAX_DIM || tab == nullptr) {
      if (tid == 0 && qsh == 0) A.out_K[blk] = -1;
      continue;
    }
    const int Dp = (D + 3) & ~3;
    const int NG = (D + 255) >> 8;
    const int NSW = NW / NG;
    const bool active = wave < NG * NSW;
    const int g = wave % NG, sw = wave / NG;
    const int NSWe = NSW * Wrow, swe = sw * Wrow + qsh;
    const int d0 = g * 256 + lane * 4;

    float c[4];
    bool valid[4];
    float own_dmu[4], own_vq[4], own_vp[4];
    const bool own_stats = active && sw == 0 && bs == 0 && TEAMS < 3 && !SHORT;
    double klacc = 0.0;
#pragma unroll
    for (int i = 0; i < 4; ++i) {
      const int d = d0 + i;
      valid[i] = d < D;
      c[i] = 0.f;
      const int64_t ixi = valid[i] ? src_index(A, base, pos, d) : src_index(A, base, pos, 0);
      float st3[3] = {0.f, 1.f, 1.f};
      if (valid[i] && active && sw == 0 && bs == 0) {
        const float mq_ = A.q_loc[ixi], sq_ = A.q_scale[ixi], mp_ = A.p_loc[ixi], sp_ = A.p_scale[ixi];
        klacc = klacc + kl_dim(mq_, sq_, mp_, sp_);
        st3[0] = mq_ - mp_; st3[1] = sq_ * sq_; st3[2] = sp_ * sp_;
      }
      own_dmu[i] = st3[0]; own_vq[i] = st3[1]; own_vp[i] = st3[2];
      if (active && sw == 0 && bs == 0 && (NSW > 1 || BS > 1 || TEAMS >= 3)) {
        stats_g[d0 + i] = st3[0]; stats_g[FAST_MAX_DIM + d0 + i] = st3[1]; stats_g[2 * FAST_MAX_DIM + d0 + i] = st3[2];
      }
    }
    {
      const double gs = wave_tree_sum(klacc);
      if (sw == 0 && bs == 0 && active && lane == 0) gpart[g] = gs;
      tsync();
      if (tid == 0) {
        double tot = gpart[0];
        for (int gg = 1; gg < NG; ++gg) tot = tot + gpart[gg];
        const int32_t K = num_aux((float)tot, A.omega);
        misc[1] = K;
        if (qsh == 0) A.out_K[blk] = K;
        hsum[0] = 0;
        beta4[0] = 0u;
        if constexpr (MARGIN) { if (qsh == 0) margin_write(A.out_margin, blk, MarginAcc()); }
      }
      tsync();
    }
    const int K = misc[1];
    MarginAcc macc;
    if (K > A.max_K || K > A.K_limit) continue;
    if (K > A.K_tab) {
      if (tid == 0 && qsh == 0) atomicAdd(A.defer_count, 1u);
      continue;
    }
    if (K == 0) {
      if (active && sw == 0 && bs == 0 && qsh == 0) {
#pragma unroll
        for (int i = 0; i < 4; ++i)
          if (valid[i]) { const int64_t ixo = src_index(A, base, pos, d0 + i); A.out_sample[ixo] = 0.f + A.p_loc[ixo]; }
      }
      continue;
    }

    float sa[4], cH[4];
    float G[NBW][4];
    auto step_consts = [&](int t_next, float (&m)[4], float (&cA)[4], float (&cBv)[4]) {
      const float rho = A.rho[K - 1 - t_next];
      float dmu_[4], vq_[4], vp_[4];
      if (own_stats) {
#pragma unroll
        for (int i = 0; i < 4; ++i) { dmu_[i] = own_dmu[i]; vq_[i] = own_vq[i]; vp_[i] = own_vp[i]; }
      } else {
        const float4 q0 = *reinterpret_cast<const float4 *>(stats_g + d0);
        const float4 q1 = *reinterpret_cast<const float4 *>(stats_g + FAST_MAX_DIM + d0);
        const float4 q2 = *reinterpret_cast<const float4 *>(stats_g + 2 * FAST_MAX_DIM + d0);
        dmu_[0] = q0.x; dmu_[1] = q0.y; dmu_[2] = q0.z; dmu_[3] = q0.w;
        vq_[0] = q1.x; vq_[1] = q1.y; vq_[2] = q1.z; vq_[3] = q1.w;
        vp_[0] = q2.x; vp_[1] = q2.y; vp_[2] = q2.z; vp_[3] = q2.w;
      }
#pragma unroll
      for (int i = 0; i < 4; ++i) {
        const StepConst sc = step_constants(rho, dmu_[i], vq_[i], vp_[i], c[i]);
        sa[i] = valid[i] ? sc.sa : 0.f; cH[i] = valid[i] ? sc.H : 0.f;
        m[i] = valid[i] ? sc.m : 0.f; cA[i] = valid[i] ? sc.A : 0.f; cBv[i] = valid[i] ? sc.Bv : 0.f;
        c[i] = c[i] + sc.a;
        __builtin_amdgcn_sched_barrier(0);
      }
    };
    auto park = [&]() {
      if (PARK && active) {
        *reinterpret_cast<float4 *>(park_g + d0) = make_float4(c[0], c[1], c[2], c[3]);
        *reinterpret_cast<float4 *>(park_g + FAST_MAX_DIM + d0) = make_float4(sa[0], sa[1], sa[2], sa[3]);
      }
    };
    auto unpark = [&]() {
      if (PARK && active) {
        asm volatile("" ::: "memory");
        const float4 pc = *reinterpret_cast<const float4 *>(park_g + d0);
        const float4 ps = *reinterpret_cast<const float4 *>(park_g + FAST_MAX_DIM + d0);
        c[0] = pc.x; c[1] = pc.y; c[2] = pc.z; c[3] = pc.w;
        sa[0] = ps.x; sa[1] = ps.y; sa[2] = ps.z; sa[3] = ps.w;
      }
    };
    {
      float m[4], cA[4], cBv[4];
      step_consts(0, m, cA, cBv);
      park();
      float cacc = 0.f;
#pragma unroll
      for (int b = 0; b < NBW; ++b)
#pragma unroll
        for (int i = 0; i < 4; ++i) G[b][i] = 0.f;
#pragma unroll
      for (int i = 0; i < 4; ++i) {
        if (bs == 0) G[0][i] = beam_G(0.f, m[i], cA[i], cBv[i], sa[i]);
        cacc = beam_C_term(cacc, 0.f, m[i], cA[i], cBv[i]);
      }
      const float cg = wave_tree_sum(cacc);
      if (active && sw == 0 && bs == 0 && lane == 0) cpart_s[g * TEAM_MB + 0] = cg;
    }

    TSTAMP(1);
    bool abandoned = false;
    int cur = 0, Bcur = 1;
    uint32_t bv_cur = 0u;
    for (int t = 0; t < K; ++t) {
#ifdef IREC_TEAM_STAMPS
      st_acc[11] += 1ull;
#endif
      const uint16_t *tab_tu = tab + (size_t)t * S * Dp;
      const uint32_t tab_lo = (uint32_t)(d0 < Dp ? d0 : Dp - 4);
      const uint16_t *tab_t = tab_tu + tab_lo;
      uint32_t bet[NBW];
      {
#pragma unroll
        for (int b = 0; b < NBW; ++b) bet[b] = (uint32_t)__builtin_amdgcn_readlane((int)bv_cur, b_lo + b);
      }
      const int nlive = Bcur - b_lo < 0 ? 0 : (Bcur - b_lo < NBW ? Bcur - b_lo : NBW);

      const int N = S * Bcur;
      for (int s_base = 0; s_base < S; s_base += SP) {
      const int s_end = s_base + SP < S ? s_base + SP : S;
      const int Sp = s_end - s_base;
#ifdef IREC_ABLATE_SCORING
      if (false) {
#else
      if (active && Bcur > 1 && (nlive == NBW || 2 * nlive >= NBW)) {
        const int n_mine = Sp > swe ? (Sp - swe + NSWe - 1) / NSWe : 0;
        const int n_chunks = (n_mine + SPC - 1) / SPC;
        auto row = [&](int m) {
          uint2 r = make_uint2(0u, 0u);
          if (m < n_mine) r = *reinterpret_cast<const uint2 *>(tab_tu + ((uint32_t)(s_base + m * NSWe + swe) * (uint32_t)Dp + tab_lo));
          return r;
        };
        uint2 ap_cur[SPC], ap_nxt[SPC];
#pragma unroll
        for (int cc = 0; cc < SPC; ++cc) { ap_cur[cc] = row(cc); ap_nxt[cc] = row(SPC + cc); }
#define IREC_AL(CC, I) ((((I) & 2) ? (((I) & 1) ? (ap_cur[CC].y >> 16) : (ap_cur[CC].y & 0xFFFFu)) : (((I) & 1) ? (ap_cur[CC].x >> 16) : (ap_cur[CC].x & 0xFFFFu))) << 2)
        typedef float f2 __attribute__((ext_vector_type(2)));
        constexpr int NP = NBW / 2;
        constexpr int NQ = 4 * SPC;
        static_assert(NBW % 2 == 0, "beams are processed in pairs");
        constexpr int NH = SHORT ? 2 : 1;
        constexpr int HP = NP / NH;
        constexpr int NQH = NQ * NH;
        static_assert(NP % NH == 0 && NQH % 2 == 0, "granules must tile the slots and alternate buffers cleanly");
        f2 zz[2][HP];
#if IREC_PK_ADDR
        f2 betf[NP];
#pragma unroll
        for (int k = 0; k < NP; ++k) betf[k] = (f2){__uint_as_float(bet[2 * k]), __uint_as_float(bet[2 * k + 1])};
#define IREC_ISSUE(Z, AD, K0) do { const float adf_ = __uint_as_float(AD); const f2 ad2_ = {adf_, adf_}; \
                               _Pragma("unroll") for (int k = 0; k < HP; ++k) { const f2 a2_ = ad2_ + betf[(K0) + k]; \
                                 Z[k].x = lds_abs_f32(__float_as_uint(a2_.x)); Z[k].y = lds_abs_f32(__float_as_uint(a2_.y)); } \
                               __builtin_amdgcn_sched_barrier(0); } while (0)
#else
#define IREC_ISSUE(Z, AD, K0) do { _Pragma("unroll") for (int k = 0; k < HP; ++k) { Z[k].x = lds_abs_f32((AD) + bet[2 * ((K0) + k)]); Z[k].y = lds_abs_f32((AD) + bet[2 * ((K0) + k) + 1]); } \
                               __builtin_amdgcn_sched_barrier(0); } while (0)
#endif
#define IREC_CONSUME(Z, I, ACC, K0) do { _Pragma("unroll") for (int k = 0; k < HP; ++k) asm volatile("" : "+v"(Z[k])); \
                                f2 t2_[HP]; \
                                _Pragma("unroll") for (int k = 0; k < HP; ++k) { \
                                  const f2 h2 = {cH[I], cH[I]}, g2 = {G[2 * ((K0) + k)][I], G[2 * ((K0) + k) + 1][I]}; \
                                  t2_[k] = __builtin_elementwise_fma(h2, Z[k], g2); }  \
                                _Pragma("unroll") for (int k = 0; k < HP; ++k)  \
                                  ACC[(K0) + k] = __builtin_elementwise_fma(t2_[k], Z[k], ACC[(K0) + k]); \
                                _Pragma("unroll") for (int k = 0; k < HP; ++k) asm volatile("" : "+v"(ACC[(K0) + k])); \
                                __builtin_amdgcn_sched_barrier(0); } while (0)
        if constexpr (PARK) {
#pragma unroll
          for (int b = 0; b < NBW; ++b)
#pragma unroll
            for (int i = 0; i < 4; ++i) asm volatile("" : "+v"(G[b][i]));
        }
        IREC_ISSUE(zz[0], IREC_AL(0, 0), 0);
        for (int ch = 0; ch < n_chunks; ++ch) {
          if constexpr (BS >= 2) {
            if ((((ch >> 2) + bs) % BS) == 0) __builtin_amdgcn_s_setprio(1);
            else __builtin_amdgcn_s_setprio(0);
          }
          f2 acc2[SPC][NP];
#pragma unroll
          for (int cc = 0; cc < SPC; ++cc)
#pragma unroll
            for (int k = 0; k < NP; ++k) acc2[cc][k] = (f2){0.f, 0.f};
          uint2 ap_new[SPC];
#pragma unroll
          for (int cc = 0; cc < SPC; ++cc) ap_new[cc] = row((ch + 2) * SPC + cc);
#pragma unroll
          for (int qh = 0; qh < NQH; ++qh) {
            constexpr int dummy_ = 0; (void)dummy_;
            const int q = qh / NH, h = qh % NH;
            if (qh + 1 < NQH) {
              const int qn = (qh + 1) / NH, hn = (qh + 1) % NH;
              IREC_ISSUE(zz[(qh + 1) & 1], IREC_AL(qn >> 2, qn & 3), hn * HP);
            } else {
#pragma unroll
              for (int cc = 0; cc < SPC; ++cc) { ap_cur[cc] = ap_nxt[cc]; ap_nxt[cc] = ap_new[cc]; }
              IREC_ISSUE(zz[0], IREC_AL(0, 0), 0);
            }
            IREC_CONSUME(zz[qh & 1], q & 3, acc2[q >> 2], h * HP);
          }
          float tot;
          int own;
          if constexpr (RW == 20) {
            rs_f2 a20[10];
#pragma unroll
            for (int cc = 0; cc < SPC; ++cc)
#pragma unroll
              for (int k = 0; k < NP; ++k) a20[cc * NP + k] = acc2[cc][k];
            tot = reduce_scatter_20(a20, lane);
            own = rs_p20;
          } else {
            float acc[ACC_ROOM];
#pragma unroll
            for (int cc = 0; cc < SPC; ++cc)
#pragma unroll
              for (int k = 0; k < NP; ++k) { acc[cc * NBW + 2 * k] = acc2[cc][k].x; acc[cc * NBW + 2 * k + 1] = acc2[cc][k].y; }
            tot = reduce_scatter_n<RW>(acc, lane);
            own = rs_p;
          }
          const int cc = own / NBW, b = own - cc * NBW;
          const int m = ch * SPC + cc;
          if (own >= 0 && (lane & 1) == 0 && m < n_mine && b < nlive) part_s[((size_t)g * SP + m * NSWe + swe) * PS + b_lo + b] = tot;
        }
        if constexpr (BS >= 2) __builtin_amdgcn_s_setprio(0);
#pragma unroll
        for (int k = 0; k < HP; ++k) asm volatile("" : "+v"(zz[0][k]));
#undef IREC_ISSUE
#undef IREC_CONSUME
#undef IREC_AL
      } else if (active && Bcur == 1 && bs == 0) {
        const int n_mine = Sp > swe ? (Sp - swe + NSWe - 1) / NSWe : 0;
        const uint32_t bet0 = bet[0];
        if constexpr (ONE) {
        constexpr int HA = ((RW / 2) + 1) & ~1, HBb = RW - HA;
        static_assert(RW % 2 == 0 && HBb >= 2 && HBb % 2 == 0, "half batches of sample pairs");
        typedef float f2w __attribute__((ext_vector_type(2)));
        const uint32_t lane_off = tab_lo * 2u;
        auto rows = [&](int m_first, auto &ap) {
          constexpr int H = (int)(sizeof(ap) / sizeof(ap[0]));
#pragma unroll
          for (int k = 0; k < H; ++k) {
            int m = m_first + k;
            m = m < n_mine ? m : n_mine - 1;
            const char *rowp = reinterpret_cast<const char *>(tab_tu) + (size_t)((uint32_t)(s_base + m * NSWe + swe) * (uint32_t)Dp) * 2u;
            ap[k] = *reinterpret_cast<const uint2 *>(rowp + lane_off);
          }
        };
        auto half = [&](const auto &ap, f2w *acc2) {
          constexpr int H = (int)(sizeof(ap) / sizeof(ap[0]));
#pragma unroll
          for (int i = 0; i < 4; ++i) {
            float z[H];
#pragma unroll
            for (int k = 0; k < H; ++k) {
              const uint32_t w = (i & 2) ? ap[k].y : ap[k].x;
              const uint32_t e = __builtin_amdgcn_ubfe(w, (i & 1) ? 16u : 0u, 16u);
              z[k] = lds_abs_f32((e << 2) + bet0);
            }
            const f2w h2 = {cH[i], cH[i]}, g2 = {G[0][i], G[0][i]};
#pragma unroll
            for (int k = 0; k < H / 2; ++k) {
              const f2w z2 = {z[2 * k], z[2 * k + 1]};
              acc2[k] = __builtin_elementwise_fma(__builtin_elementwise_fma(h2, z2, g2), z2, acc2[k]);
            }
            __builtin_amdgcn_sched_barrier(0);
          }
        };
        uint2 apA[HA], apB[HBb];
        rows(0, apA);
        for (int m0 = 0; m0 < n_mine; m0 += RW) {
          f2w acc2[RW / 2];
#pragma unroll
          for (int p = 0; p < RW / 2; ++p) acc2[p] = (f2w){0.f, 0.f};
          rows(m0 + HA, apB);
          half(apA, &acc2[0]);
          rows(m0 + RW, apA);
          half(apB, &acc2[HA / 2]);
          float tot;
          int own;
          if constexpr (RW == 20) {
            rs_f2 a20[10];
#pragma unroll
            for (int k = 0; k < 10; ++k) a20[k] = acc2[k];
            tot = reduce_scatter_20(a20, lane);
            own = rs_p20;
          } else {
            float acc[ACC_ROOM];
#pragma unroll
            for (int k = 0; k < RW / 2; ++k) { acc[2 * k] = acc2[k].x; acc[2 * k + 1] = acc2[k].y; }
            tot = reduce_scatter_n<RW>(acc, lane);
            own = rs_p;
          }
          const int m = m0 + own;
          if (own >= 0 && (lane & 1) == 0 && m < n_mine) part_s[((size_t)g * SP + m * NSWe + swe) * PS] = tot;
        }
        } else {
          constexpr int HB = RW / 2;
          static_assert(RW % 2 == 0, "half batches");
          for (int m0 = 0; m0 < n_mine; m0 += RW) {
            float acc[ACC_ROOM];
#pragma unroll
            for (int p = 0; p < RW; ++p) acc[p] = 0.f;
#pragma unroll
            for (int h = 0; h < 2; ++h) {
              uint2 ap[HB];
#pragma unroll
              for (int k = 0; k < HB; ++k) {
                const int m = m0 + h * HB + k;
                ap[k] = make_uint2(0u, 0u);
                if (m < n_mine) ap[k] = *reinterpret_cast<const uint2 *>(tab_tu + ((uint32_t)(s_base + m * NSWe + swe) * (uint32_t)Dp + tab_lo));
              }
#pragma unroll
              for (int i = 0; i < 4; ++i) {
                float z[HB];
#pragma unroll
                for (int k = 0; k < HB; ++k) {
                  const uint32_t w = (i & 2) ? ap[k].y : ap[k].x;
                  z[k] = lds_abs_f32((((i & 1) ? (w >> 16) : (w & 0xFFFFu)) << 2) + bet0);
                }
#pragma unroll
                for (int k = 0; k < HB; ++k) acc[h * HB + k] = proposal_term(acc[h * HB + k], z[k], cH[i], G[0][i]);
                __builtin_amdgcn_sched_barrier(0);
              }
            }
            const float tot = reduce_scatter_n<RW>(acc, lane);
            const int m = m0 + rs_p;
            if (rs_p >= 0 && (lane & 1) == 0 && m < n_mine) part_s[((size_t)g * SP + m * NSWe + swe) * PS] = tot;
// ... 43 lines not shown
                  if (b < nlive) {
#pragma unroll
                    for (int i = 0; i < 4; ++i) {
                      const float z = lds_abs_f32(al[i] + bet[b]);
                      acc[cc * NBW + b] = proposal_term(acc[cc * NBW + b], z, cH[i], G[b][i]);
                    }
                  }
                }
              }
            }
          }
          const float tot = reduce_scatter_n<RW>(acc, lane);
          const int cc = rs_p / NBW, b = rs_p - cc * NBW;
          const int s = (ch * SPC + cc) * NSWe + swe;
          if (rs_p >= 0 && (lane & 1) == 0 && s < Sp && b < nlive) part_s[((size_t)g * SP + s) * PS + b_lo + b] = tot;
        }
      }
      TSTAMP(2);
      tsync();
      TSTAMP(3);
      {
        constexpr int MK = (CMAX + NT - 1) / NT;
        const int Np = Sp * Bcur, f_base = s_base * Bcur;
        {
          float pr[MK][4], cbv[MK][4];
          const int gstride = SP * PS;
#pragma unroll
          for (int q = 0; q < MK; ++q) {
            const int f = q * NT + tid, fs = f < Np ? f : 0;
            const int s = Bcur == NB ? fs / NB : fs / Bcur, b = fs - s * Bcur;
#pragma unroll
            for (int gg = 0; gg < 4; ++gg) pr[q][gg] = part_s[(gg < NG ? gg : 0) * gstride + s * PS + b];
#pragma unroll
            for (int gg = 0; gg < 4; ++gg) cbv[q][gg] = cpart_s[(gg < NG ? gg : 0) * TEAM_MB + b];
          }
          if (KEYS_ALIAS && Bcur != NB) {
#pragma unroll
            for (int q = 0; q < MK; ++q)
#pragma unroll
              for (int gg = 0; gg < 4; ++gg) asm volatile("" : "+v"(pr[q][gg]));
            tsync();
          }
          unsigned long long *xg = nullptr;
          if (CAN_SHARE && Wrow > 1)
            xg = reinterpret_cast<unsigned long long *>(A.coop_xch) + ((size_t)(t & 1) * COOP_MAX_BLOCKS + (size_t)xrow) * COOP_KEYS;
          const unsigned long long tag64 = (unsigned long long)(uint32_t)(t + 1) << 32;
          uint32_t foreign = 0u;
#pragma unroll
          for (int q = 0; q < MK; ++q) {
            float sc = pr[q][0];
            if (NG > 1) sc = sc + pr[q][1];
            if (NG > 2) sc = sc + pr[q][2];
            if (NG > 3) sc = sc + pr[q][3];
            float cb = cbv[q][0];
            if (NG > 1) cb = cb + cbv[q][1];
            if (NG > 2) cb = cb + cbv[q][2];
            if (NG > 3) cb = cb + cbv[q][3];
            const int f = q * NT + tid;
            if (f < Np) {
              bool mine = true;
              if (CAN_SHARE && Wrow > 1) {
                const int s_ = Bcur == NB ? f / NB : f / Bcur;
                mine = ((s_ % NSWe) % Wrow) == qsh;
              }
              if (mine) {
                const uint32_t key = score_key(sc + cb);
                key_s[f_base + f] = key;
                if (CAN_SHARE && Wrow > 1) __hip_atomic_store(&xg[f], tag64 | (unsigned long long)key, __ATOMIC_RELAXED, __HIP_MEMORY_SCOPE_AGENT);
              } else foreign |= 1u << q;
            }
          }
          if (CAN_SHARE && Wrow > 1) {
            const uint32_t tag = (uint32_t)(t + 1);
            const unsigned long long t0 = __builtin_amdgcn_s_memrealtime();
            int32_t bad = 0;
            for (uint32_t turn = 1; foreign != 0u; ++turn) {
              unsigned long long gq[MK];
#pragma unroll
              for (int q = 0; q < MK; ++q)
                gq[q] = (foreign >> q) & 1u ? __hip_atomic_load(&xg[q * NT + tid], __ATOMIC_RELAXED, __HIP_MEMORY_SCOPE_AGENT) : 0ull;
#pragma unroll
              for (int q = 0; q < MK; ++q)
                if (((foreign >> q) & 1u) && (uint32_t)(gq[q] >> 32) == tag) { key_s[f_base + q * NT + tid] = (uint32_t)gq[q]; foreign &= ~(1u << q); }
              if (foreign == 0u || (turn & 63u) != 0u) continue;
              if (__hip_atomic_load(A.coop_err, __ATOMIC_RELAXED, __HIP_MEMORY_SCOPE_AGENT) != 0u) { bad = 1; break; }
              if (__builtin_amdgcn_s_memrealtime() - t0 > COOP_GIVE_UP_TICKS) {
                __hip_atomic_store(A.coop_err, 1u, __ATOMIC_RELAXED, __HIP_MEMORY_SCOPE_AGENT);
                bad = 1; break;
              }
            }
            if (bad) misc[6] = 1;
          }
        }
      }
      if (s_end < S) tsync();
      }
      if (CAN_SHARE && Wrow > 1) {
        tsync();
        if (misc[6]) { abandoned = true; break; }
      }
      const int Bnew = B < N ? B : N;
      TSTAMP(4);
#ifdef IREC_ABLATE_SELECT
      tsync();
      if (tid < Bnew) { sel_s[tid] = tid % S; sel_b[tid] = tid % Bcur; sm->sel_bo[tid] = beta4[cur * TEAM_MB + tid % Bcur];
                        hsum[(cur ^ 1) * TEAM_MB + tid] = 0; beta4[(cur ^ 1) * TEAM_MB + tid] = 0u; }
      tsync();
#else
      constexpr bool QUICK_SEL = TEAMS <= 2 && !MULTI_PASS;
      if constexpr (QUICK_SEL) __builtin_assume(N <= 1024);
      select_topB_sync<NT, QUICK_SEL>(key_s, N, Bnew, Bcur, sm, tid, tsync, nullptr, [&](int j, int32_t sp_, int32_t bp_, uint32_t key_) {
        const int32_t nh = (int32_t)((uint32_t)hsum[cur * TEAM_MB + bp_] + (uint32_t)sp_ * (uint32_t)(69 + t));
        hsum[(cur ^ 1) * TEAM_MB + j] = nh;
        sm->sel_bo[j] = beta4[cur * TEAM_MB + bp_];
        bp[(size_t)t * NB + j] = (sp_ << 6) | bp_;
        if constexpr (MARGIN) margin_stash(sm, j, key_);
      });
      if constexpr (MARGIN) {
        if (tid < 64) margin_step(key_s, N, Bnew, Bcur, sm, lane, t == K - 1, macc);
        tsync();
      }
#endif
      TSTAMP(5);
      const bool last = (t == K - 1);
      __builtin_amdgcn_s_setprio(2);
      uint32_t bv_new;
      {
        const int32_t nh = hsum[(cur ^ 1) * TEAM_MB + (lane < Bnew ? lane : 0)];
        bv_new = dlog_s[hash_from_sum(nh) - 1u];
      }
#ifdef IREC_ABLATE_UPDATE
      if (false) {
#else
      if (active) {
#endif
        unpark();
        const float sa_t[4] = {sa[0], sa[1], sa[2], sa[3]};
        const float *bold = beams_g + ((size_t)cur * NB) * FAST_MAX_DIM + d0;
        float *bnew = beams_g + ((size_t)(cur ^ 1) * NB) * FAST_MAX_DIM + d0;
#pragma unroll
        for (int j = 0; j < NBW; ++j)
#pragma unroll
          for (int i = 0; i < 4; ++i) G[j][i] = 0.f;
        float m[4], cA[4], cBv[4];
#pragma unroll
        for (int i = 0; i < 4; ++i) { m[i] = 0.f; cA[i] = 0.f; cBv[i] = 0.f; }
        float cacc[rsn_room(NBW)];
#pragma unroll
        for (int j = 0; j < rsn_room(NBW); ++j) cacc[j] = 0.f;
        constexpr int UB = (TEAMS >= 3 || BS >= 2) ? 5 : NBW;
        const int Bupd = last ? 1 : Bnew;
        const int32_t v_sp = sel_s[lane < Bnew ? lane : 0], v_bp = sel_b[lane < Bnew ? lane : 0];
        const uint32_t v_bo = sm->sel_bo[lane < Bnew ? lane : 0];
#pragma unroll
        for (int j0 = 0; j0 < NBW; j0 += UB) {
          uint2 apv[UB];
          float4 obv4[UB];
          uint32_t bet_old[UB];
#pragma unroll
          for (int u = 0; u < UB; ++u) {
            const int jj = j0 + u, j = b_lo + jj;
            apv[u] = make_uint2(0u, 0u);
            obv4[u] = make_float4(0.f, 0.f, 0.f, 0.f);
            bet_old[u] = 0u;
            if (jj < NBW && j < Bupd) {
              const int32_t sp_ = __builtin_amdgcn_readlane(v_sp, j);
              const int32_t bp_ = __builtin_amdgcn_readlane(v_bp, j);
              bet_old[u] = (uint32_t)__builtin_amdgcn_readlane((int)v_bo, j);
              apv[u] = *reinterpret_cast<const uint2 *>(tab_t + (size_t)sp_ * Dp);
#ifndef IREC_ABLATE_SLAB
              if (t) obv4[u] = *reinterpret_cast<const float4 *>(bold + (size_t)bp_ * FAST_MAX_DIM);
#endif
            }
          }
          if (j0 == 0 && !last) { step_consts(t + 1, m, cA, cBv); park(); }
          if (j0 == 0) TSTAMP(9);
          constexpr int YB = 5;
          float zy[YB][4];
#pragma unroll
          for (int u = 0; u < UB; ++u) {
            if (u % YB == 0) {
#pragma unroll
              for (int v = 0; v < YB; ++v) {
                const int uu = u + v < UB ? u + v : UB - 1;
                const uint32_t al[4] = {(apv[uu].x & 0xFFFFu) << 2, (apv[uu].x >> 16) << 2, (apv[uu].y & 0xFFFFu) << 2, (apv[uu].y >> 16) << 2};
#pragma unroll
                for (int i = 0; i < 4; ++i) zy[v][i] = lds_abs_f32(al[i] + bet_old[uu]);
              }
            }
            const int jj = j0 + u, j = b_lo + jj;
            if (jj < NBW && j < Bupd) {
              const float obv[4] = {obv4[u].x, obv4[u].y, obv4[u].z, obv4[u].w};
              float nb[4];
#pragma unroll
              for (int i = 0; i < 4; ++i) {
                const float y = sa_t[i] * zy[u % YB][i];
                nb[i] = obv[i] + y;
              }
              if (last) {
                if (j == 0 && sw == 0 && qsh == 0) {
#pragma unroll
                  for (int i = 0; i < 4; ++i)
                    if (valid[i]) {
                      const int64_t ixo = src_index(A, base, pos, d0 + i);
                      A.out_sample[ixo] = nb[i] + A.p_loc[ixo];
                    }
                }
              } else {
#ifndef IREC_ABLATE_SLAB
                if (sw == 0) *reinterpret_cast<float4 *>(bnew + (size_t)j * FAST_MAX_DIM) = make_float4(nb[0], nb[1], nb[2], nb[3]);
#endif
                if constexpr (LATE_G) {
#pragma unroll
                  for (int i = 0; i < 4; ++i) G[jj][i] = nb[i];
                } else {
#pragma unroll
                  for (int i = 0; i < 4; ++i) {
                    G[jj][i] = beam_G(nb[i], m[i], cA[i], cBv[i], sa[i]);
                    cacc[jj] = beam_C_term(cacc[jj], nb[i], m[i], cA[i], cBv[i]);
                  }
                }
              }
            }
          }
          __builtin_amdgcn_sched_barrier(0);
        }
        if constexpr (LATE_G) {
          if (!last) {
#pragma unroll
            for (int jj = 0; jj < NBW; ++jj) {
              if (b_lo + jj < Bnew) {
#pragma unroll
                for (int i = 0; i < 4; ++i) {
                  const float nbv = G[jj][i];
                  G[jj][i] = beam_G(nbv, m[i], cA[i], cBv[i], sa[i]);
                  cacc[jj] = beam_C_term(cacc[jj], nbv, m[i], cA[i], cBv[i]);
                }
              }
              __builtin_amdgcn_sched_barrier(0);
            }
          }
        }
        TSTAMP(10);
        if (!last) {
          const float ctot = reduce_scatter_n<NBW>(cacc, lane);
          if (sw == 0 && (lane & 1) == 0 && rs_c >= 0 && b_lo + rs_c < Bnew) cpart_s[g * TEAM_MB + b_lo + rs_c] = ctot;
        }
      }
      TSTAMP(6);
      __builtin_amdgcn_s_setprio(0);
      if (tid < Bnew) beta4[(cur ^ 1) * TEAM_MB + tid] = bv_new;
      bv_cur = bv_new;
      cur ^= 1;
      Bcur = Bnew;
    }
    tsync();
    if (abandoned) {
      if (tid == 0 && qsh == 0) A.out_K[blk] = -2;
      continue;
    }
    if (tid == 0 && qsh == 0) {
      int j = 0;
      for (int t = K - 1; t >= 0; --t) {
        const int32_t v = __builtin_nontemporal_load(&bp[(size_t)t * NB + j]);
        A.out_indices[blk * (int64_t)A.max_K + t] = v >> 6;
        j = v & 63;
      }
      if constexpr (MARGIN) margin_write(A.out_margin, blk, macc);
    }
    TSTAMP(8);
  }
#ifdef IREC_TEAM_STAMPS
  if (A.dbg && lane == 0)
    for (int k = 0; k < 12; ++k) A.dbg[((size_t)blockIdx.x * (TEAMS * BS * 4) + wave_wg) * 16 + k] = st_acc[k];
  if (A.dbg && lane == 0) {
    A.dbg[((size_t)blockIdx.x * (TEAMS * BS * 4) + wave_wg) * 16 + 12] = __builtin_amdgcn_s_memtime() - st_t0;
    A.dbg[((size_t)blockIdx.x * (TEAMS * BS * 4) + wave_wg) * 16 + 13] = __builtin_amdgcn_s_memrealtime() - st_r0;
  }
#endif
}

#ifndef IREC_TEAM_MARGIN_TU
constexpr int CHUNK_MAX_DIM = 1 << 22;
__host__ __device__ inline size_t chunk_ws_bytes(int NB, int dpad, int max_K) {
  return (size_t)(6 + 2 * NB) * dpad * 4 + ((((size_t)(max_K > 0 ? max_K : 1) * NB * 4) + 255) & ~(size_t)255);
}
__host__ __device__ inline size_t chunk_lds_one(int NB, int NBP, int S) {
  return team_part_bytes(NBP, S) + team_key_bytes(NB, S) + team_small_bytes(NB) + 16;
}
__host__ __device__ inline size_t chunk_lds_total(int NB, int NBP, int S, int teams) { return T3_BYTES + (size_t)teams * chunk_lds_one(NB, NBP, S); }

template <int NB, int NBP, int TEAMS, bool GANG = false>
__global__ __launch_bounds__(TEAMS * TEAM_NT, 1) void encode_chunk_kernel(EncArgs A) {
  using TeamLds = TeamLdsT<NB>;
  constexpr int TEAM_MB = team_mb(NB);
  constexpr size_t TEAM_SMALL_BYTES = (sizeof(TeamLds) + 15) & ~(size_t)15;
  constexpr int NT = TEAM_NT;
  constexpr int SPC = NBP <= 10 ? 20 / NBP : 1;
  constexpr int RW = NBP * SPC;
  static_assert(NB % NBP == 0 && (NBP == 10 || NBP == 16 || NBP == 20) && NB <= 60, "chunked encoder: passes of 10, 16 or 20 beams, at most 60 beam slots (6-bit back-pointers)");
  extern __shared__ __attribute__((aligned(16))) char smem[];
  const int S = A.S, B = A.B;
  const int lane = threadIdx.x & 63;
  const int wave_wg = __builtin_amdgcn_readfirstlane((int)(threadIdx.x >> 6));
  const int team = wave_wg / TEAM_NW, g = wave_wg % TEAM_NW;
  const int tid = (int)threadIdx.x - team * NT;
  char *tbase = smem + T3_BYTES + (size_t)team * chunk_lds_one(NB, NBP, S);
  float *part_s = reinterpret_cast<float *>(tbase);
  float *run_s = reinterpret_cast<float *>(tbase + team_part_bytes(NBP, S));
  uint32_t *key_s = reinterpret_cast<uint32_t *>(run_s);
  TeamLds *sm = reinterpret_cast<TeamLds *>(tbase + team_part_bytes(NBP, S) + team_key_bytes(NB, S));
  uint32_t *bar_word = reinterpret_cast<uint32_t *>(tbase + team_part_bytes(NBP, S) + team_key_bytes(NB, S) + TEAM_SMALL_BYTES);
  double *gpart = sm->gpart;
  int32_t *sel_s = sm->sel_s, *sel_b = sm->sel_b;
  int32_t *hsum = &sm->hsum[0][0];
  uint32_t *beta4 = &sm->beta4[0][0];
  int32_t *misc = sm->misc;
  float *cpart_s = &sm->cpart[0][0];
  float *Cb_s = sm->Cb;
  const uint16_t *dlog_s = A.dlog4r;
  const int rs_p = rsn_owner<RW>(lane), rs_c = rsn_owner<NBP>(lane);
  const int rs_p20 = RW == 20 ? rs20_owner(lane) : -1;
  double *kl_tot = reinterpret_cast<double *>(sm->wb);

  if ((uint32_t)(uintptr_t)(__attribute__((address_space(3))) char *)smem != 0u) __builtin_trap();
  commit_table_stamps(A);
  {
    float *l3 = reinterpret_cast<float *>(smem);
    for (int k = (int)threadIdx.x; k < (int)IREC_PM1; k += TEAMS * NT) {
      const float v = A.lut2[k];
      l3[k] = v; l3[k + IREC_PM1] = v; l3[k + 2 * IREC_PM1] = v;
    }
    if (tid == 0) *bar_word = 0u;
  }
  __syncthreads();
  TeamBarrier tsync{bar_word, 0u, (uint32_t)TEAM_NW};

  const int Dpad = A.max_dim_pad;
  char *slab = A.ws + ((size_t)blockIdx.x * TEAMS + team) * A.ws_per_wg;
  float *stats_g = reinterpret_cast<float *>(slab);
  float *cvar_g = stats_g + (size_t)3 * Dpad;
  float *sa_g = cvar_g + (size_t)2 * Dpad;
  float *beams_g = sa_g + Dpad;
  int32_t *bp = reinterpret_cast<int32_t *>(beams_g + (size_t)2 * NB * Dpad);

  const int64_t n_static = (int64_t)TEAMS * (int64_t)gridDim.x < A.n_blocks ? (int64_t)TEAMS * (int64_t)gridDim.x : A.n_blocks;
  bool first_block = true;
  int steal = 0;
  constexpr int ABL = GANG ? IREC_GANG_ABLATE : 0;
  const int G = GANG ? A.coop_W : 1;
  const int GC = GANG ? A.gang_chunks : 1, SP = GANG ? G / GC : 1;
  uint32_t gang_epoch = 0u;
  for (;;) {
    tsync();
    if (tid == 0) {
      int64_t r;
      if constexpr (GANG) {
        const int64_t slot = (int64_t)team * (int64_t)gridDim.x + (int64_t)blockIdx.x;
        r = first_block && slot < A.n_blocks * (int64_t)G ? slot / G : A.n_blocks;
        misc[2] = (int32_t)(slot % G);
      } else if (first_block) {
        r = (int64_t)team * (int64_t)gridDim.x + (int64_t)blockIdx.x;
        r = r < n_static ? xcd_static_row(r, n_static, (int)gridDim.x) : A.n_blocks;
// ... 490 lines not shown
                  if (d0 + i < D && sp == 0) {
                    const int64_t ixo = src_index(A, base, pos, d0 + i);
                    A.out_sample[ixo] = nb[i] + A.p_loc[ixo];
                  }
              } else {
                *reinterpret_cast<float4 *>(bnew + (size_t)j * Dpad) = make_float4(nb[0], nb[1], nb[2], nb[3]);
              }
            }
          }
        }
      }
      if (tid < Bnew) beta4[(cur ^ 1) * TEAM_MB + tid] = bv_new;
      bv_cur = bv_new;
      cur ^= 1;
      Bcur = Bnew;
    }
    tsync();
    if (gang_lost) {
      if (tid == 0) A.out_K[blk] = -2;
      continue;
    }
    if (tid == 0 && gm == 0) {
      int j = 0;
      for (int t = K - 1; t >= 0; --t) {
        const int32_t v = __builtin_nontemporal_load(&bp[(size_t)t * NB + j]);
        A.out_indices[blk * (int64_t)A.max_K + t] = v >> 6;
        j = v & 63;
      }
    }
  }
}

#endif
#ifndef IREC_TEAM_AUX_TU
#ifndef IREC_CHOICE_WPE
#define IREC_CHOICE_WPE 2
#endif
__device__ __forceinline__ void choice_table_rows(int64_t seed, int32_t S, int32_t K_tab, const uint16_t *__restrict__ dlog4r,
                                                  const ChoiceJobs &jobs, uint32_t skip, int64_t wg, int64_t n_wg) {
  __shared__ uint32_t n_s[8][4][32];
  __shared__ uint8_t x_s[8][4][32];
  const int hwl = threadIdx.x >> 5, j = threadIdx.x & 31;
  const int64_t n_hw = jobs.hw_end[jobs.n - 1];
  for (int64_t hw0 = wg * 8; hw0 < n_hw; hw0 += n_wg * 8) {
    const int64_t hwg = hw0 + hwl;
    int q = 0;
    while (q + 1 < jobs.n && hwg >= jobs.hw_end[q]) ++q;
    const int64_t hw = hwg - (q ? jobs.hw_end[q - 1] : 0);
    const bool hw_ok = hwg < n_hw && !((skip >> q) & 1u) && !(jobs.keep[q] && *jobs.keep[q]);
    const int D = jobs.D[q];
    const int Dp = (D + 3) & ~3;
    const int NQ = Dp >> 2;
    const int NM = (NQ + 31) >> 5;
    const int64_t row = hw_ok ? hw / NM : 0;
    const int m = hw_ok ? (int)(hw - row * NM) : 0;
    const int t = (int)(row / S), s = (int)(row - (int64_t)t * S);
    const int quad = 32 * m + j;
    const bool q_ok = hw_ok && quad < NQ;
    uint32_t al[4] = {0u, 0u, 0u, 0u};
#pragma unroll
    for (int i = 0; i < 4; ++i) n_s[hwl][i][j] = 0u;
    if (q_ok) {
      const StepSeed ss = make_step_seed(seed + t);
      uint32_t rm1[4];
      draw_rm1_x4(ss, (uint64_t)s * (uint64_t)D + (uint64_t)(4 * quad), rm1);
#pragma unroll
      for (int i = 0; i < 4; ++i)
        if (4 * quad + i < D) al[i] = (uint32_t)dlog4r[rm1[i]] >> 2;
    }
    __syncthreads();
    uint32_t rank[4] = {0u, 0u, 0u, 0u};
    if (q_ok) {
#pragma unroll
      for (int i = 0; i < 4; ++i) rank[i] = atomicAdd(&n_s[hwl][i][al[i] & 31u], 1u);
    }
    __syncthreads();
    if (j < 8 && hw_ok) {
      const int slot = j >> 1, ring = j & 1;
      int n[16];
      int tot = 0;
#pragma unroll
      for (int p = 0; p < 16; ++p) { n[p] = (int)n_s[hwl][slot][(ring + 22 * p) & 31]; tot += n[p]; }
      int Lf = 32, x0f = n[0];
      bool done = false;
      for (int L = tot > 16 ? (tot + 15) >> 4 : 1; L < 32 && !done; ++L)
        for (int x0 = 0; x0 <= n[0] && !done; ++x0) {
          int xp = x0;
          bool ok = true;
#pragma unroll
          for (int p = 1; p < 16; ++p) {
            const int ub = L - n[p - 1] + xp;
            ok = ok && ub >= 0;
            xp = n[p] < ub ? n[p] : (ub < 0 ? 0 : ub);
          }
          if (ok && x0 + n[15] - xp <= L) { done = true; Lf = L; x0f = x0; }
        }
      int xp = x0f;
      x_s[hwl][slot][ring] = (uint8_t)xp;
#pragma unroll
      for (int p = 1; p < 16; ++p) {
        const int ub = Lf - n[p - 1] + xp;
        xp = n[p] < ub ? n[p] : (ub < 0 ? 0 : ub);
        x_s[hwl][slot][(ring + 22 * p) & 31] = (uint8_t)xp;
      }
    }
    __syncthreads();
    if (q_ok) {
      uint32_t v[4];
#pragma unroll
      for (int i = 0; i < 4; ++i) v[i] = al[i] + (rank[i] < (uint32_t)x_s[hwl][i][al[i] & 31u] ? 0u : IREC_PM1);
      *reinterpret_cast<uint2 *>(jobs.tab[q] + (row * Dp + 4 * quad)) = make_uint2(v[0] | (v[1] << 16), v[2] | (v[3] << 16));
    }
    __syncthreads();
  }
}
__global__ __launch_bounds__(256, IREC_CHOICE_WPE) void alpha_choice_kernel(int64_t seed, int32_t S, int32_t K_tab,
                                                           const uint16_t *__restrict__ dlog4r, ChoiceJobs jobs) {
  choice_table_rows(seed, S, K_tab, dlog4r, jobs, 0u, (int64_t)blockIdx.x, (int64_t)gridDim.x);
}

struct CostRow { float v[4][4]; bool ok[4]; bool okD; int D; };
__device__ __forceinline__ void cost_row_issue(const EncArgs &A, int64_t blk, int t, CostRow &c) {
  c.D = A.block_dim[blk];
  const int64_t base = A.block_base[blk];
  const int32_t pos = A.block_pos[blk];
  c.okD = c.D >= 1 && c.D <= FAST_MAX_DIM;
  int64_t ix[4];
#pragma unroll
  for (int i = 0; i < 4; ++i) { const int d = t + 256 * i; c.ok[i] = c.okD && d < c.D; ix[i] = c.ok[i] ? src_index(A, base, pos, d) : 0; }
#pragma unroll
  for (int i = 0; i < 4; ++i) {
    c.v[i][0] = c.v[i][1] = c.v[i][2] = c.v[i][3] = 1.f;
    if (c.ok[i]) { c.v[i][0] = A.q_loc[ix[i]]; c.v[i][1] = A.q_scale[ix[i]]; c.v[i][2] = A.p_loc[ix[i]]; c.v[i][3] = A.p_scale[ix[i]]; }
  }
}
__device__ __forceinline__ void cost_row_finish(const PrepArgs &P, const EncArgs &A, int64_t blk, int t, const CostRow &c) {
  __shared__ double part[4];
  double acc = 0.0;
#pragma unroll
  for (int i = 0; i < 4; ++i)
    if (c.ok[i]) acc = acc + kl_dim(c.v[i][0], c.v[i][1], c.v[i][2], c.v[i][3]);
  const double ws = wave_tree_sum(acc);
  if ((t & 63) == 0) part[t >> 6] = ws;
  __syncthreads();
  if (t == 0) {
    const double tot = ((part[0] + part[1]) + part[2]) + part[3];
    int32_t K = c.okD ? num_aux((float)tot, A.omega) : 0;
    K = K < 0 ? 0 : (K > (1 << 20) ? (1 << 20) : K);
    const uint32_t cst = (uint32_t)K * (uint32_t)(c.okD ? c.D : 0);
    P.cost[blk] = ((cst < (1u << 22) ? cst : (1u << 22) - 1u) << 10) | (uint32_t)blk;
  }
}

__global__ __launch_bounds__(256, IREC_CHOICE_WPE) void prep_kernel(PrepArgs P, EncArgs A) {
  const int t = (int)threadIdx.x;
  uint32_t *p = P.head;
  int wg = (int)blockIdx.x;
  if (wg == 0) {
    for (int w = t; w < (int)(WS_COUNTER_BYTES / 4); w += 256) {
      const bool book = (w >= WS_KEEP_WORD && w < WS_KEEP_WORD + 4) || (w >= WS_STAMP_WORD && w < WS_STAMP_WORD + 4 * WS_STAMP_WORDS) ||
                        (w >= WS_PENDING_WORD && w < WS_PENDING_WORD + 4 * WS_STAMP_WORDS);
      if (!book) p[w] = 0u;
    }
    if (t < 4) {
      uint32_t *stamp = p + WS_STAMP_WORD + t * WS_STAMP_WORDS, *pend = p + WS_PENDING_WORD + t * WS_STAMP_WORDS;
      bool same = P.ts.reuse != 0 && P.ts.w[t][0] != 0u;
#pragma unroll
      for (int k = 0; k < WS_STAMP_WORDS; ++k) same = same && stamp[k] == P.ts.w[t][k];
      p[WS_KEEP_WORD + t] = same ? 1u : 0u;
#pragma unroll
      for (int k = 0; k < WS_STAMP_WORDS; ++k) pend[k] = P.ts.w[t][k];
      if (!same) {
#pragma unroll
        for (int k = 0; k < WS_STAMP_WORDS; ++k) stamp[k] = ~P.ts.w[t][k];
      }
    }
    return;
  }
  wg -= 1;
  if (wg < P.n_granule) {
    uint4 *x = reinterpret_cast<uint4 *>(reinterpret_cast<char *>(p) + WS_COUNTER_BYTES);
#pragma unroll
    for (int par = 0; par < 2; ++par) {
      uint4 *xb = x + ((size_t)par * COOP_MAX_BLOCKS + (size_t)wg) * (COOP_KEYS * 8 / 16);
      for (int k = t; k < COOP_KEYS * 8 / 16; k += 256) xb[k] = make_uint4(0u, 0u, 0u, 0u);
    }
    return;
  }
  wg -= P.n_granule;
  if (wg < P.n_table_wgs) {
    uint32_t skip = 0u;
#pragma unroll
    for (int q = 0; q < 4; ++q) {
      bool same = P.ts.reuse != 0 && P.ts.w[q][0] != 0u;
#pragma unroll
      for (int k = 0; k < WS_STAMP_WORDS; ++k) same = same && __builtin_nontemporal_load(p + WS_STAMP_WORD + q * WS_STAMP_WORDS + k) == P.ts.w[q][k];
      skip |= same ? (1u << q) : 0u;
    }
    if (P.table_kind == 1) choice_table_rows(P.seed, P.S, P.K_tab, P.dlog4r, P.jobs, skip, (int64_t)wg, (int64_t)P.n_table_wgs);
    else if (P.table_kind == 2) {
      int q = 0;
      while (q + 1 < P.jobs.n && (int64_t)wg >= P.jobs.hw_end[q]) ++q;
      const int64_t first = q ? P.jobs.hw_end[q - 1] : 0;
      if (!((skip >> q) & 1u)) plain_table_rows(P.seed, P.S, P.jobs.D[q], P.K_tab, P.dlog4r, P.jobs.tab[q], (int64_t)wg - first, P.jobs.hw_end[q] - first);
    }
    return;
  }
  wg -= P.n_table_wgs;
  if (wg < P.n_cost) {
    CostRow cr;
    cost_row_issue(A, wg, t, cr);
    cost_row_finish(P, A, wg, t, cr);
  }
}

#endif
#ifndef IREC_TEAM_GANG_TU
static int team_cfg(int shape_override) {
  switch (shape_override) {
    case 2: return 20;
    case 3: return 3;
    case 5: return 12;
    default: return 2;
  }
}
struct TeamShape { int nb, teams, bs; bool passes; bool one = false; };
static TeamShape team_shape(int B, int S, int ovr) {
  const int cfg = team_cfg(ovr);
  if (B == 1 && cfg == 2) {
    return TeamShape{10, 3, 1, team_s_pass(10, S, 3, 1024, false, 1) != S, true};
  }
  if (B <= 10) {
    const int ps = team_row(10, B);
    if (cfg == 3 || (cfg == 2 && team_s_pass(10, S, 3, 1024, false, ps) == S)) return TeamShape{10, 3, 1, false};
    if (cfg != 2 || team_s_pass(10, S, 2, 1024, false, ps) == S) return TeamShape{10, 2, 1, false};
    return TeamShape{10, 3, 1, true};
  }
  if (B <= 20) {
    if (cfg == 20) return TeamShape{20, 2, 1, false};
    if (cfg == 12) return TeamShape{20, 1, 2, false};
    if (team_s_pass(20, S, 3, 1024) == S) return TeamShape{20, 3, 1, false};
    if (team_s_pass(20, S, 2, 1024) != S) return TeamShape{20, 1, 2, false};
    return TeamShape{20, 2, 1, false};
  }
  if (B <= 30) return TeamShape{30, 1, 3, false};
  if (B <= 32) return TeamShape{32, 1, 2, false};
  if (cfg != 3 && B > 48 && B <= 54 && S >= 128) return TeamShape{54, 1, 3, false};
  if (B <= 60) return TeamShape{60, 1, 3, false};
  return TeamShape{0, 0, 0, false};
}
#ifndef IREC_TEAM_AUX_TU
int team_count_for(int B, int S, int ovr) { return team_shape(B, S, ovr).teams; }
int team_shareable(int B, int S, int ovr) {
  const TeamShape sh = team_shape(B, S, ovr);
  return (sh.nb && sh.teams >= 2 && sh.bs == 1 && !sh.passes && !sh.one && (int64_t)S * sh.nb <= COOP_KEYS) ? sh.teams : 0;
}
bool team_placeable(int B, int S, int ovr) {
  const TeamShape sh = team_shape(B, S, ovr);
  return sh.nb == 20 && sh.teams == 2 && sh.bs == 1 && !sh.passes && !sh.one;
}
int team_waves_for(int B, int S, int ovr) { const TeamShape sh = team_shape(B, S, ovr); return sh.teams * sh.bs * TEAM_NW; }
size_t team_ws_extra_for(int B, int S, int ovr) {
  const TeamShape sh = team_shape(B, S, ovr);
  const int ps = sh.nb ? team_row(sh.nb, B) : 0;
  return (sh.nb && !team_keys_in_lds(sh.nb, S, sh.teams, sh.passes, ps)) ? ((team_key_bytes(ps, S) + 255) & ~(size_t)255) : 0;
}
size_t team_ws_bytes_for(int B, int S, int ovr, int max_K) {
  const TeamShape sh = team_shape(B, S, ovr);
  return sh.nb ? fast_ws_bytes(sh.nb, max_K) + team_ws_extra_for(B, S, ovr) : 0;
}
int team_ten_teams(int B, int S, int ovr) {
  const TeamShape sh = team_shape(B, S, ovr);
  if (!(sh.nb == 10 && sh.bs == 1 && !sh.passes && !sh.one && (sh.teams == 2 || sh.teams == 3) && ten_applies(B, S))) return 0;
  return sh.teams;
}
const char *team_kernel_name(int B, int S, int ovr) {
  static thread_local char buf[64];
  const TeamShape sh = team_shape(B, S, ovr);
  snprintf(buf, sizeof buf, "encode_team_kernel<%d,%d,%d%s%s>", sh.nb, sh.teams, sh.bs, sh.passes ? ",passes" : "", sh.one ? ",one" : "");
  return buf;
}

size_t team_lds_for(int B, int S, int ovr) {
  const TeamShape sh = team_shape(B, S, ovr);
  if (!sh.nb) return (size_t)-1;
  if ((int64_t)S * sh.nb >= (1 << 24)) return (size_t)-1;
  const int ps = team_row(sh.nb, B);
  const int sp = team_s_pass(sh.nb, S, sh.teams, sh.teams == 1 ? 2048 : 1024, sh.passes, ps);
  if (sp < 1 || (sp < S && (sp < 16 || (sh.teams > 1 && !sh.passes)))) return (size_t)-1;
  const size_t b = team_lds_total(sh.nb, S, sp, sh.teams, sh.passes, ps);
  return b <= FAST_LDS_LIMIT ? b : (size_t)-1;
}

#endif

template <int NB, int TEAMS, int BS, bool PASSES = false, bool ONE = false, bool SHARE = false, bool MARGIN = false>
static hipError_t launch_team_t(const EncArgs &A, int grid, hipStream_t st) {
  const int ps = team_row(NB, A.B);
  const int sp = (TEAMS == 1 || PASSES) ? team_s_pass(NB, A.S, TEAMS, TEAMS == 1 ? 2048 : 1024, PASSES, ps) : A.S;
  const size_t lds = team_lds_total(NB, A.S, sp, TEAMS, PASSES, ps);
  hipError_t e = hipFuncSetAttribute(reinterpret_cast<const void *>(encode_team_kernel<NB, TEAMS, BS, PASSES, ONE, SHARE, MARGIN>),
                                     hipFuncAttributeMaxDynamicSharedMemorySize, (int)lds);
  if (e != hipSuccess) return e;
  hipLaunchKernelGGL((encode_team_kernel<NB, TEAMS, BS, PASSES, ONE, SHARE, MARGIN>), dim3(grid), dim3(TEAMS * BS * TEAM_NT), lds, st, A);
  return hipGetLastError();
}

#ifdef IREC_TEAM_MARGIN_TU
static int team_margin_key(int B, int S, int ovr) {
  const TeamShape sh = team_shape(B, S, ovr);
  if (!sh.nb || sh.passes || sh.one) return 0;
  const int key = sh.nb * 100 + sh.teams * 10 + sh.bs;
  return (key == 2031 || key == 2021 || key == 1031 || key == 1021 || key == 3013) ? key : 0;
}
bool team_margin_build(int B, int S, int shape_override) { return team_margin_key(B, S, shape_override) != 0; }
hipError_t launch_encode_team_margin(const EncArgs &A, int grid, hipStream_t st) {
  if (A.out_margin == nullptr || A.coop_W > 1) return hipErrorInvalidValue;
  switch (team_margin_key(A.B, A.S, A.shape_override)) {
    case 2031: return launch_team_t<20, 3, 1, false, false, false, true>(A, grid, st);
    case 2021: return launch_team_t<20, 2, 1, false, false, false, true>(A, grid, st);
    case 1031: return launch_team_t<10, 3, 1, false, false, false, true>(A, grid, st);
    case 1021: return launch_team_t<10, 2, 1, false, false, false, true>(A, grid, st);
    case 3013: return launch_team_t<30, 1, 3, false, false, false, true>(A, grid, st);
    default: return hipErrorInvalidValue;
  }
}
#else

hipError_t launch_encode_team(const EncArgs &A, int grid, hipStream_t st) {
  const TeamShape sh = team_shape(A.B, A.S, A.shape_override);
  const int key = sh.nb * 100 + sh.teams * 10 + sh.bs + (sh.passes ? 10000 : 0) + (sh.one ? 100000 : 0);
  if (A.coop_W > 1) {
    switch (key) {
      case 1021: return launch_team_t<10, 2, 1, false, false, true>(A, grid, st);
      case 2021: return launch_team_t<20, 2, 1, false, false, true>(A, grid, st);
      case 2031: return launch_team_t<20, 3, 1, false, false, true>(A, grid, st);
      default: return hipErrorInvalidValue;
    }
  }
  if ((key == 1031 || key == 1021) && !A.no_ten && ten_applies(A.B, A.S)) return launch_encode_ten(A, team_ten_teams(A.B, A.S, A.shape_override), grid, st);
  switch (key) {
    case 101031: return launch_team_t<10, 3, 1, false, true>(A, grid, st);
    case 111031: return launch_team_t<10, 3, 1, true, true>(A, grid, st);
    case 11031: return launch_team_t<10, 3, 1, true>(A, grid, st);
    case 6013: return launch_team_t<60, 1, 3>(A, grid, st);
    case 5413: return launch_team_t<54, 1, 3>(A, grid, st);
    case 1021: return launch_team_t<10, 2, 1>(A, grid, st);
    case 1031: return launch_team_t<10, 3, 1>(A, grid, st);
    case 2021: return launch_team_t<20, 2, 1>(A, grid, st);
    case 2031: return launch_team_t<20, 3, 1>(A, grid, st);
    case 2012: return launch_team_t<20, 1, 2>(A, grid, st);
    case 3013: return launch_team_t<30, 1, 3>(A, grid, st);
    case 3212: return launch_team_t<32, 1, 2>(A, grid, st);
    default: return hipErrorInvalidValue;
  }
}

#endif
#endif

#ifndef IREC_TEAM_MARGIN_TU
struct ChunkShape { int nb, nbp, teams; };
static int chunk_nb(int B) { return B <= 10 ? 10 : B <= 20 ? 20 : B <= 30 ? 30 : B <= 32 ? 32 : B <= 40 ? 40 : B <= 50 ? 50 : B <= 60 ? 60 : 0; }
static ChunkShape chunk_shape(int B, int S) {
  static const ChunkShape cand[] = {{10, 10, 3}, {10, 10, 2}, {10, 10, 1}, {20, 10, 3}, {20, 10, 1},
                                    {30, 10, 3}, {30, 10, 2}, {30, 10, 1}, {32, 16, 2}, {32, 16, 1},
                                    {40, 10, 2}, {40, 10, 1}, {50, 10, 2}, {50, 10, 1}, {60, 10, 2}, {60, 10, 1}};
  const int nb = chunk_nb(B);
  if (!nb || (int64_t)S * nb > 4096) return ChunkShape{0, 0, 0};
  for (const ChunkShape &c : cand)
    if (c.nb == nb && chunk_lds_total(c.nb, c.nbp, S, c.teams) <= FAST_LDS_LIMIT) return c;
  return ChunkShape{0, 0, 0};
}
template <int NB, int NBP, int TEAMS, bool GANG = false>
static hipError_t launch_chunk_t(const EncArgs &A, int grid, hipStream_t st) {
  const size_t lds = chunk_lds_total(NB, NBP, A.S, TEAMS);
  hipError_t e = hipFuncSetAttribute(reinterpret_cast<const void *>(encode_chunk_kernel<NB, NBP, TEAMS, GANG>),
                                     hipFuncAttributeMaxDynamicSharedMemorySize, (int)lds);
  if (e != hipSuccess) return e;
  hipLaunchKernelGGL((encode_chunk_kernel<NB, NBP, TEAMS, GANG>), dim3(grid), dim3(TEAMS * TEAM_NT), lds, st, A);
  return hipGetLastError();
}
#ifdef IREC_TEAM_GANG_TU
static ChunkShape chunk_gang_shape(int B, int S) {
  const ChunkShape c = chunk_shape(B, S);
  if (!c.teams) return c;
  if (c.nb <= 30 && c.nbp == 10 && c.teams == 3) return c;
  return ChunkShape{c.nb, c.nb == 32 ? 16 : 10, 1};
}
int chunk_gang_teams(int B, int S) { return chunk_gang_shape(B, S).teams; }
int chunk_gang_nb(int B, int S) { return chunk_gang_shape(B, S).nb; }
size_t chunk_gang_lds_for(int B, int S) { const ChunkShape c = chunk_gang_shape(B, S); return chunk_lds_total(c.nb, c.nbp, S, c.teams); }
const char *chunk_gang_kernel_name(int B, int S) {
  static thread_local char buf[56];
  const ChunkShape c = chunk_gang_shape(B, S);
  snprintf(buf, sizeof buf, "encode_chunk_kernel<%d,%d,%d,gang>", c.nb, c.nbp, c.teams);
  return buf;
}
hipError_t launch_encode_chunk_gang(const EncArgs &A, int grid, hipStream_t st) {
  const ChunkShape c = chunk_gang_shape(A.B, A.S);
  if (!c.teams || A.max_dim_pad <= FAST_MAX_DIM || A.max_dim_pad > CHUNK_MAX_DIM) return hipErrorInvalidValue;
  if (A.coop_W < 2 || A.gang_chunks < 1 || A.coop_W % A.gang_chunks != 0 || !A.gang_xch || A.n_blocks > GANG_MAX_BLOCKS ||
      A.n_blocks * (int64_t)A.coop_W > (int64_t)grid * c.teams)
    return hipErrorInvalidValue;
  switch (c.nb * 1000 + c.nbp * 10 + c.teams) {
    case 10103: return launch_chunk_t<10, 10, 3, true>(A, grid, st);
    case 20103: return launch_chunk_t<20, 10, 3, true>(A, grid, st);
    case 30103: return launch_chunk_t<30, 10, 3, true>(A, grid, st);
    case 10101: return launch_chunk_t<10, 10, 1, true>(A, grid, st);
    case 20101: return launch_chunk_t<20, 10, 1, true>(A, grid, st);
    case 30101: return launch_chunk_t<30, 10, 1, true>(A, grid, st);
    case 32161: return launch_chunk_t<32, 16, 1, true>(A, grid, st);
    case 40101: return launch_chunk_t<40, 10, 1, true>(A, grid, st);
    case 50101: return launch_chunk_t<50, 10, 1, true>(A, grid, st);
    case 60101: return launch_chunk_t<60, 10, 1, true>(A, grid, st);
    default: return hipErrorInvalidValue;
  }
}
#else
int chunk_teams(int B, int S) { return chunk_shape(B, S).teams; }
bool chunk_applies(int B, int S, int max_dim) {
  return max_dim > FAST_MAX_DIM && max_dim <= CHUNK_MAX_DIM && chunk_shape(B, S).teams != 0;
}
size_t chunk_lds_for(int B, int S) { const ChunkShape c = chunk_shape(B, S); return chunk_lds_total(c.nb, c.nbp, S, c.teams); }
size_t chunk_ws_for(int B, int dpad, int max_K) { return chunk_ws_bytes(chunk_nb(B) ? chunk_nb(B) : 60, dpad, max_K); }
const char *chunk_kernel_name(int B, int S) {
  static thread_local char buf[48];
  const ChunkShape c = chunk_shape(B, S);
  snprintf(buf, sizeof buf, "encode_chunk_kernel<%d,%d,%d>", c.nb, c.nbp, c.teams);
  return buf;
}
hipError_t launch_encode_chunk(const EncArgs &A, int grid, hipStream_t st) {
  if (!chunk_applies(A.B, A.S, A.max_dim_pad)) return hipErrorInvalidValue;
  if (A.coop_W > 1) return launch_encode_chunk_gang(A, grid, st);
  const ChunkShape c = chunk_shape(A.B, A.S);
  switch (c.nb * 1000 + c.nbp * 10 + c.teams) {
    case 10103: return launch_chunk_t<10, 10, 3>(A, grid, st);
    case 10102: return launch_chunk_t<10, 10, 2>(A, grid, st);
    case 10101: return launch_chunk_t<10, 10, 1>(A, grid, st);
    case 20103: return launch_chunk_t<20, 10, 3>(A, grid, st);
    case 20101: return launch_chunk_t<20, 10, 1>(A, grid, st);
    case 30103: return launch_chunk_t<30, 10, 3>(A, grid, st);
    case 30102: return launch_chunk_t<30, 10, 2>(A, grid, st);
    case 30101: return launch_chunk_t<30, 10, 1>(A, grid, st);
    case 32162: return launch_chunk_t<32, 16, 2>(A, grid, st);
    case 32161: return launch_chunk_t<32, 16, 1>(A, grid, st);
    case 40102: return launch_chunk_t<40, 10, 2>(A, grid, st);
    case 40101: return launch_chunk_t<40, 10, 1>(A, grid, st);
    case 50102: return launch_chunk_t<50, 10, 2>(A, grid, st);
    case 50101: return launch_chunk_t<50, 10, 1>(A, grid, st);
    case 60102: return launch_chunk_t<60, 10, 2>(A, grid, st);
    case 60101: return launch_chunk_t<60, 10, 1>(A, grid, st);
    default: return hipErrorInvalidValue;
  }
}
#endif
#endif

#ifndef IREC_TEAM_AUX_TU
int64_t prep_table_wgs(int kind, int32_t S, int32_t K_tab, int n, const int32_t *dims, ChoiceJobs *jobs) {
  int64_t end = 0;
  for (int q = 0; q < n; ++q) {
    if (kind == 1) end += (int64_t)K_tab * S * ((((dims[q] + 3) >> 2) + 31) >> 5);
    else {
      const int64_t total = (int64_t)K_tab * S * ((dims[q] + 3) & ~3);
      end += std::min<int64_t>((total + 1023) / 1024, 1024);
    }
    jobs->D[q] = dims[q]; jobs->hw_end[q] = end;
  }
  jobs->n = n;
  if (kind == 1) { const int64_t want = (end + 7) / 8; return want < 4096 ? want : 4096; }
  return end;
}
hipError_t launch_prep(const PrepArgs &P, const EncArgs &A, hipStream_t st) {
  const int64_t grid = 1 + (int64_t)P.n_granule + P.n_table_wgs + P.n_cost;
  hipLaunchKernelGGL(prep_kernel, dim3((unsigned)grid), dim3(256), 0, st, P, A);
  return hipGetLastError();
}
hipError_t launch_alpha_choice_all(int64_t seed, int32_t S, int32_t K_tab, const uint16_t *dlog4r, int n, const int32_t *dims,
                                   uint16_t *const *tabs, const uint32_t *const *keeps, hipStream_t st) {
  if (n < 1 || n > 4) return hipErrorInvalidValue;
  ChoiceJobs jobs{};
  const int64_t grid = prep_table_wgs(1, S, K_tab, n, dims, &jobs);
  for (int q = 0; q < n; ++q) { jobs.tab[q] = tabs[q]; jobs.keep[q] = keeps ? keeps[q] : nullptr; }
  hipLaunchKernelGGL(alpha_choice_kernel, dim3(grid > 0 ? (unsigned)grid : 1u), dim3(256), 0, st, seed, S, K_tab, dlog4r, jobs);
  return hipGetLastError();
}
hipError_t launch_alpha_choice(int64_t seed, int32_t S, int32_t D, int32_t K_tab, const uint16_t *dlog4r, uint16_t *tab,
                               const uint32_t *keep, hipStream_t st) {
  return launch_alpha_choice_all(seed, S, K_tab, dlog4r, 1, &D, &tab, &keep, st);
}

#endif

}
```

relative-entropy-coding_amd/irec/_lib.py:

```python
import ctypes
import os

from .errors import IrecLibraryError

_HERE = os.path.dirname(os.path.abspath(__file__))
LIB_PATH = os.path.join(os.path.dirname(_HERE), "csrc", "libirec_hip.so")

IREC_OK = 0
IREC_E_INVALID = -1
IREC_E_HIP = -2
IREC_E_NO_DEVICE = -3
IREC_E_WORKSPACE = -4
IREC_FLAG_FORCE_GENERIC = 1
IREC_FLAG_FUSED_PHILOX = 2
IREC_FLAG_ONE_TABLE = 4
IREC_FLAG_TEAM = 8
IREC_FLAG_NO_SPLIT = 16
IREC_FLAG_TEST_SPLIT_ORPHAN = 32
IREC_FLAG_LISTED_ORDER = 262144
IREC_FLAG_MARGINS = 524288
IREC_FLAG_NO_TEN = 1048576
IREC_FLAG_TABLES_PRESENT = 65536
IREC_FLAG_REUSE_TABLES = 64
IREC_FLAG_SHAPE_SHIFT = 8
IREC_FLAG_SHAPE = {"default": 0, "2": 2 << 8, "3": 3 << 8, "1x2": 5 << 8, "team": 6 << 8}
IREC_TABLE_STEPS_DEFAULT = 32
IREC_TABLE_STEPS_MAX = 4096
IREC_NORMAL_TABLE_PAD = 16
BIG_PRIME = 10007
MAX_BEAMS = 256
MAX_PARTITIONS = 65536


class IrecParams(ctypes.Structure):
    _fields_ = [("kl_per_partition", ctypes.c_float), ("n_samples", ctypes.c_int32), ("n_beams", ctypes.c_int32),
                ("flags", ctypes.c_int32), ("table_dims", ctypes.c_int32 * 4), ("table_steps", ctypes.c_int32)]


class IrecTables(ctypes.Structure):
    _fields_ = [("lut10007", ctypes.c_void_p), ("aux_ratios", ctypes.c_void_p), ("n_aux_ratios", ctypes.c_int32)]


class IrecNormalTables(ctypes.Structure):
    _fields_ = [("table", ctypes.c_void_p * 4), ("dim", ctypes.c_int32 * 4), ("n_samples", ctypes.c_int32), ("steps", ctypes.c_int32)]


class IrecFitParams(ctypes.Structure):
    _fields_ = [("kl_per_partition", ctypes.c_float), ("relative_tolerance", ctypes.c_double), ("learning_rate", ctypes.c_double),
                ("max_iters", ctypes.c_int32)]


class IrecPlanInfo(ctypes.Structure):
    _fields_ = [("kernel", ctypes.c_char * 64), ("table_kernel", ctypes.c_char * 32), ("grid", ctypes.c_int32),
                ("waves_per_wg", ctypes.c_int32), ("teams_per_wg", ctypes.c_int32), ("lds_bytes", ctypes.c_int32),
                ("table_steps", ctypes.c_int32), ("n_tables", ctypes.c_int32), ("split", ctypes.c_int32), ("n_cu", ctypes.c_int32),
                ("clock_mhz", ctypes.c_int32), ("split_beams", ctypes.c_int32), ("table_bytes", ctypes.c_int64), ("workspace_bytes", ctypes.c_int64)]

    def as_dict(self):
        return {name: (getattr(self, name).decode() if isinstance(getattr(self, name), bytes) else int(getattr(self, name)))
                for name, _ in self._fields_}


class IrecPlanDetail(ctypes.Structure):
    _fields_ = [("kind", ctypes.c_int32), ("grid", ctypes.c_int32), ("teams_per_wg", ctypes.c_int32), ("coop_width", ctypes.c_int32),
                ("coop_beams", ctypes.c_int32), ("gang_chunks", ctypes.c_int32), ("placed", ctypes.c_int32), ("split_blocks", ctypes.c_int32),
                ("share_first", ctypes.c_int64), ("n_slots", ctypes.c_int64), ("slabs_in_workspace", ctypes.c_int64),
                ("slab_bytes", ctypes.c_int64), ("fixed_bytes", ctypes.c_int64), ("exchange_rows", ctypes.c_int32), ("exchange_keys", ctypes.c_int32)]

    def as_dict(self):
        return {name: int(getattr(self, name)) for name, _ in self._fields_}


_vp = ctypes.c_void_p
_i64 = ctypes.c_int64
_i32 = ctypes.c_int32
_PP = ctypes.POINTER(IrecParams)

SIGNATURES = {
    "irec_last_error": (ctypes.c_char_p, []),
    "irec_version": (ctypes.c_char_p, []),
    "irec_n_samples": (_i32, [ctypes.c_double, ctypes.c_double]),
    "irec_codelength": (ctypes.c_double, [_i64, _i32]),
    "irec_build_lut": (ctypes.c_int, [_vp]),
    "irec_tf_shuffle_perm": (ctypes.c_int, [_i64, _i64, _vp]),
    "irec_philox_uniform_int": (ctypes.c_int, [_i64, _i64, _vp]),
    "irec_importance_encode": (ctypes.c_int, [_vp, _vp, _vp, _vp, _i64, ctypes.c_double, ctypes.c_double, _i64,
                                              ctypes.POINTER(_i64), _vp]),
    "irec_tf_stateless_normal": (ctypes.c_int, [_i64, _i64, _i64, _vp]),
    "irec_importance_decode": (ctypes.c_int, [_vp, _vp, _i64, _i64, _i64, _vp]),
    "irec_importance_n_samples": (_i64, [ctypes.c_double]),
    "irec_tf_random_normal": (ctypes.c_int, [_i64, _i64, _vp]),
    "irec_create": (ctypes.c_int, [ctypes.c_int, ctypes.POINTER(_vp)]),
    "irec_create_ex": (ctypes.c_int, [ctypes.c_int, _vp, ctypes.POINTER(_vp)]),
    "irec_create_with": (ctypes.c_int, [ctypes.c_int, ctypes.POINTER(IrecTables), ctypes.POINTER(_vp)]),
    "irec_max_partitions": (_i32, [_vp]),
    "irec_destroy": (None, [_vp]),
    "irec_encode_workspace_bytes": (ctypes.c_size_t, [_vp, _PP, _i32, _i32]),
    "irec_encode_workspace_bytes_for": (ctypes.c_size_t, [_vp, _PP, _i64, _i32, _i32]),
    "irec_test_plan": (ctypes.c_int, [_i32, _i32, _PP, _i64, _i32, _i32, _vp, _vp]),
    "irec_encode_plan": (ctypes.c_int, [_vp, _PP, _i64, _i32, _i32, ctypes.POINTER(IrecPlanInfo)]),
    "irec_block_kl": (ctypes.c_int, [_vp, _PP, _i64, _vp, _vp, _vp, _vp, _vp, _vp, _vp, _vp, _vp, _vp, _vp]),
    "irec_beam_encode": (ctypes.c_int, [_vp, _PP, _i64, _vp, _vp, _vp, _i32, _vp, _vp, _vp, _vp, _vp, _i64, _i32,
                                        _vp, _vp, _vp, _vp, ctypes.c_size_t, _vp]),
    "irec_beam_encode_ex": (ctypes.c_int, [_vp, _PP, _i64, _vp, _vp, _vp, _i32, _vp, _vp, _vp, _vp, _vp, _i64, _i32,
                                           _vp, _vp, _vp, _vp, _vp, ctypes.c_size_t, _vp]),
    "irec_beam_decode": (ctypes.c_int, [_vp, _PP, _i64, _vp, _vp, _vp, _vp, _vp, _vp, _i64, _i32, _vp, _vp, _vp, _vp]),
    "irec_decode_workspace_bytes": (ctypes.c_size_t, [_vp, _PP, _i32]),
    "irec_beam_decode_ws": (ctypes.c_int, [_vp, _PP, _i64, _vp, _vp, _vp, _i32, _vp, _vp, _vp, _i64, _i32, _vp, _vp, _vp, _vp,
                                           ctypes.c_size_t, _vp]),
    "irec_decode_tensors_supported": (_i32, [_PP, _i32, _i32]),
    "irec_beam_decode_tensors": (ctypes.c_int, [_vp, _PP, _i64, _i32, _i32, _vp, _vp, _vp, _vp, _i64, _i32, _vp, _vp, _vp, _vp,
                                                ctypes.c_size_t, _vp]),
    "irec_normal_table_floats": (ctypes.c_size_t, [_i32, _i32, _i32]),
    "irec_normal_table_build": (ctypes.c_int, [_i64, _i32, _i32, _i32, _vp, _i32]),
    "irec_gc_importance_encode": (ctypes.c_int, [_vp, _i64, _vp, _vp, _vp, _vp, _vp, _vp, _vp, _vp, ctypes.POINTER(IrecNormalTables),
                                                 ctypes.c_float, _i32, _vp, _vp, _vp, _vp]),
    "irec_gc_importance_decode": (ctypes.c_int, [_vp, _i64, _vp, _vp, _vp, _vp, _vp, _vp, ctypes.POINTER(IrecNormalTables), _i32,
                                                 _vp, _vp, _vp, _vp]),
    "irec_fit_workspace_bytes": (ctypes.c_size_t, [_i64, _i32]),
    "irec_fit_partitions": (ctypes.c_int, [_vp, ctypes.c_float, _i64, _i32, _vp, _vp, _vp, _vp, _vp, _vp, _vp, ctypes.c_size_t, _vp]),
    "irec_fit_partitions_host": (ctypes.c_int, [ctypes.c_float, _i64, _i32, _vp, _vp, _vp, _vp, _vp, _vp, _i32]),
    "irec_fit_aux_ratios": (ctypes.c_int, [_vp, ctypes.POINTER(IrecFitParams), _i64, _i32, _vp, _vp, _vp, _vp, _vp, _i32, _vp, _vp, _i32,
                                           ctypes.POINTER(_i32), _vp, _vp, ctypes.c_size_t, _vp]),
    "irec_fit_aux_ratios_host": (ctypes.c_int, [ctypes.POINTER(IrecFitParams), _i64, _i32, _vp, _vp, _vp, _vp, _vp, _i32, _vp, _vp, _i32,
                                                ctypes.POINTER(_i32), _vp, _vp, ctypes.c_size_t, _i32]),
    "irec_test_fit_chunk": (_i32, [_i32]),
    "irec_test_det_exp": (ctypes.c_int, [_vp, _i64, _vp]),
    "irec_io_last_error": (ctypes.c_char_p, []),
    "irec_ac_encode": (ctypes.c_int, [_vp, _i32, _vp, _i64, _i32, _vp, _i64, ctypes.POINTER(_i64)]),
    "irec_ac_decode": (ctypes.c_int, [_vp, _i32, _vp, _i64, _i32, _vp, _i64, ctypes.POINTER(_i64)]),
    "irec_rec_pack_bits": (_i64, [_vp, _i64, _vp, _i64]),
    "irec_rec_unpack_bits": (_i64, [_vp, _i64, _vp, _i64]),
    "irec_rec_encode_file": (_i64, [ctypes.c_uint32] * 6 + [_i32, _vp, _vp, _vp, _vp, _i64]),
    "irec_rec_decode_file": (ctypes.c_int, [_vp, _i64, _vp, _vp, _vp, _i64, _vp, _i64, _vp, _i64]),
    "irec_rec_encode_files": (_i64, [ctypes.c_uint32] * 6 + [_i32, _i32, _i32, _i32, _vp, _vp, _vp, _i64, _vp, _i32]),
    "irec_rec_decode_files": (ctypes.c_int, [_vp, _vp, _i32, _i32, _i32, _i32, _vp, _vp, _vp, _i32]),
    "irec_device_uniform_int": (ctypes.c_int, [_vp, _i64, _i64, _vp, _vp]),
    "irec_shim_stats": (ctypes.c_int, [_vp, _vp, _vp, _vp, _i32, _i32, _i32, _i32, _i32, _i32, _vp, _vp, _vp]),
    "irec_shim_cat_elu": (ctypes.c_int, [_vp, _vp, _vp, _vp, _i32, _i32, _i32, _i32, _i32, _i32, _vp, _vp]),
    "irec_shim_residual_elu": (ctypes.c_int, [_vp, _vp, _vp, ctypes.c_float, _vp, _vp, _i32, _i32, _i32, _vp, _vp]),
    "irec_test_decoder_sqrt": (ctypes.c_int, [_vp, _vp, _vp]),
    "irec_test_reduce_scatter": (ctypes.c_int, [_vp, _vp, _vp, _i32, _vp]),
    "irec_test_select": (ctypes.c_int, [_vp, _vp, _i32, _i32, _i32, _vp, _vp, _vp]),
    "irec_test_select_quick": (ctypes.c_int, [_vp, _vp, _i32, _i32, _i32, _vp, _vp, _vp]),
    "irec_test_proposal_table": (ctypes.c_int, [_vp, _i64, _i32, _i32, _i32, _vp, _vp]),
    "irec_device_tables": (ctypes.c_int, [_vp, ctypes.POINTER(_vp), ctypes.POINTER(_vp), ctypes.POINTER(_vp),
                                          ctypes.POINTER(_vp)]),
}

_lib = None


_lib_path = None


def load(path=None):
    global _lib, _lib_path
    if _lib is not None:
        if path is not None and os.path.abspath(path) != _lib_path:
            raise IrecLibraryError(f"irec._lib.load({path!r}): {_lib_path} is loaded already")
        return _lib
    variant = path is not None
    path = os.path.abspath(path) if variant else LIB_PATH
    if not os.path.exists(path):
        raise IrecLibraryError(
            f"{path} not found: build it with `make -C relative-entropy-coding_amd/csrc` "
            "(or `python -c 'import __graft_entry__ as g; g.build()'`).  irec has no CPU fallback.")
    lib = ctypes.CDLL(path)
    for name, (res, args) in SIGNATURES.items():
        if variant and not hasattr(lib, name):
            continue
        fn = getattr(lib, name)
        fn.restype = res
        fn.argtypes = args
    _lib, _lib_path = lib, path
    return _lib


def check(status, what=""):
    if status != IREC_OK:
        msg = load().irec_last_error().decode("utf-8", "replace")
        raise IrecLibraryError(f"{what}: irec_status {status}: {msg}")
```

Baseline: 173,200.

## Precompute second-step candidate rows into an L2-sized float table and stream them

Adds a per-call precomputed float table (z1) holding the candidate sample values for the second search step, for the first S1 samples per first-step choice. S1 is sized so the table fits in about three quarters of L2. The prep kernel fills the table. The team kernel then streams these rows with wave-uniform vector loads through a small register ring, instead of rebuilding them from alpha tables and the LUT. This cuts the lookup and gather arithmetic in step one, at the cost of extra prep work, workspace memory and L2 pressure. It applies only to the 20-beam, 3-team shape when the batch is large enough. Optional nontemporal slab loads and stores are also added but are off by default.

Result: slower. 141,300 (-18.4%).

```diff
diff --git a/relative-entropy-coding_amd/csrc/irec_host.cpp b/relative-entropy-coding_amd/csrc/irec_host.cpp
--- a/relative-entropy-coding_amd/csrc/irec_host.cpp
+++ b/relative-entropy-coding_amd/csrc/irec_host.cpp
@@ -261,6 +261,7 @@
   int device = -1;
   int n_cu = 0;
   int clock_mhz = 0;
+  int64_t l2_bytes = 4 << 20;
   float *d_lut = nullptr;
   float *d_lut2 = nullptr;
   uint16_t *d_dlog4r = nullptr;
@@ -457,6 +458,7 @@
   ctx->device = device;
   ctx->n_cu = prop.multiProcessorCount;
   ctx->clock_mhz = prop.clockRate / 1000;
+  if (prop.l2CacheSize > 0) ctx->l2_bytes = prop.l2CacheSize;
   ctx->n_rho = aux_ratios ? n_aux : IREC_MAX_PARTITIONS;
   const irec_status st = [&]() -> irec_status {
     HIP_TRY(hipMalloc(&ctx->d_lut, P * sizeof(float)));
@@ -489,6 +491,11 @@
 }
 
 }
+
+#ifndef IREC_STREAM_L2_NUM
+#define IREC_STREAM_L2_NUM 3
+#define IREC_STREAM_L2_DEN 4
+#endif
 
 namespace {
 
@@ -510,6 +517,8 @@
   int tab_dim[4];
   size_t tab_off[4];
   size_t tab_bytes;
+  int z1_S1;
+  size_t z1_off[4];
   int gang_blocks;
   size_t gang_stride, gang_bytes;
 };
@@ -530,6 +539,17 @@
   { const int sh = (p->flags & IREC_FLAG_SHAPE_MASK) >> IREC_FLAG_SHAPE_SHIFT;
     if (sh > 6 || sh == 1 || sh == 4) return fail(IREC_E_INVALID, "unknown IREC_FLAG_SHAPE_* value"); }
   return IREC_OK;
+}
+
+int stream_samples(const irec_context *ctx, const irec_params *p, int n_tab, const int *tab_dim) {
+  const int S = p->n_samples;
+  const int pin = (p->flags & IREC_FLAG_STREAM_MASK) >> IREC_FLAG_STREAM_SHIFT;
+  if (pin > 0) return std::min(pin - 1, S);
+  size_t per_sample = 0;
+  for (int q = 0; q < n_tab; ++q) per_sample += irec::team_z1_bytes(S, 1, tab_dim[q]);
+  if (per_sample == 0) return 0;
+  const size_t fit = (size_t)ctx->l2_bytes * IREC_STREAM_L2_NUM / IREC_STREAM_L2_DEN / per_sample;
+  return (int)std::min<size_t>((size_t)S, fit);
 }
 
 Plan make_plan(const irec_context *ctx, const irec_params *p, int32_t max_dim, int32_t max_K) {
@@ -541,7 +561,7 @@
   pl.fast = !(p->flags & IREC_FLAG_FORCE_GENERIC) && max_dim <= irec::FAST_MAX_DIM && irec::fast_nb_for(B) != 0 &&
             irec::fast_lds_for(B, S, false) <= irec::FAST_LDS_LIMIT && (int64_t)S * B < (1 << 24);
   pl.grid_cap = 2 * n_cu;
-  pl.table = false; pl.team = false; pl.lone = false; pl.chunk = false; pl.n_tab = 0; pl.tab_bytes = 0;
+  pl.table = false; pl.team = false; pl.lone = false; pl.chunk = false; pl.n_tab = 0; pl.tab_bytes = 0; pl.z1_S1 = 0;
   pl.gang_blocks = 0; pl.gang_stride = 0; pl.gang_bytes = 0;
   const int want = p->table_steps > 0 ? p->table_steps : IREC_TABLE_STEPS_DEFAULT;
   pl.K_tab = std::max(1, std::min(std::min(want, IREC_TABLE_STEPS_MAX), max_K > 0 ? max_K : 1));
@@ -566,6 +586,13 @@
     if (pl.team_only && !pl.team) { pl.table = false; pl.n_tab = 0; pl.tab_bytes = 0; }
     if (pl.team) pl.grid_cap = std::max(irec::team_count_for(B, S, pl.shape), (p->flags & IREC_FLAG_NO_TEN) ? 0 : irec::team_ten_teams(B, S, pl.shape)) * n_cu;
     pl.lone = pl.team && irec::lone_applies(B, pl.shape);
+    if (pl.team && !pl.lone && pl.K_tab >= 2 && !(p->flags & IREC_FLAG_MARGINS) && irec::team_streams(B, S, pl.shape)) {
+      pl.z1_S1 = stream_samples(ctx, p, pl.n_tab, pl.tab_dim);
+      for (int q = 0; q < pl.n_tab && pl.z1_S1 > 0; ++q) {
+        pl.z1_off[q] = pl.tab_bytes;
+        pl.tab_bytes += round_up_sz(irec::team_z1_bytes(S, pl.z1_S1, pl.tab_dim[q]), 256);
+      }
+    }
   }
   if (!pl.table) pl.team_only = false;
   pl.chunk = !pl.fast && !pl.team_only && !(p->flags & (IREC_FLAG_FORCE_GENERIC | IREC_FLAG_FUSED_PHILOX | IREC_FLAG_ONE_TABLE)) &&
@@ -581,6 +608,7 @@
     }
     if (!pl.table) { pl.chunk = false; pl.n_tab = 0; pl.tab_bytes = 0; }
   }
+  if (!pl.table) pl.z1_S1 = 0;
   auto one_cap = [&](bool table) { return (irec::fast_waves_for(B, S, table) == 8 ? 1 : 2) * n_cu; };
   if (pl.fast) {
     pl.one_grid_cap = one_cap(pl.table);
@@ -765,6 +793,14 @@
   return -1;
 }
 
+int stream_for_call(const irec_context *ctx, const Plan &pl, const irec_params *p, int64_t n_blocks, bool margins) {
+  if (pl.z1_S1 < 1 || !pl.table || !pl.team || pl.lone || pl.chunk || margins || pl.K_tab < 2) return 0;
+  if (!irec::team_streams(p->n_beams, p->n_samples, pl.shape)) return 0;
+  if ((p->flags & IREC_FLAG_STREAM_MASK) != 0) return pl.z1_S1;
+  const int n_cu = ctx->n_cu > 0 ? ctx->n_cu : 256;
+  return n_blocks >= (int64_t)irec::team_count_for(p->n_beams, p->n_samples, pl.shape) * n_cu ? pl.z1_S1 : 0;
+}
+
 struct CallDetail {
   int kind = 0;
   int grid = 0;
@@ -776,6 +812,7 @@
   int64_t n_slots = 0;
   int placed = 0;
   int split_blocks = 0;
+  int stream_S1 = 0;
 };
 CallDetail call_detail(const irec_context *ctx, const Plan &pl, const irec_params *p, int64_t n_blocks, int32_t max_block_dim, bool margins) {
   CallDetail d;
@@ -800,6 +837,7 @@
   } else if (pl.table && pl.team) {
     d.kind = 3;
     d.teams = call_teams(p, pl.shape, share_W, margins);
+    d.stream_S1 = share_W >= 2 ? 0 : stream_for_call(ctx, pl, p, n_blocks, margins);
     d.grid = batch_grid(n_blocks, std::min(pl.grid_cap / d.teams, n_cu));
     if (share_W >= 2) {
       d.W = share_W; d.grid = share_grid; d.n_slots = d.share_first + (n_blocks - d.share_first) * share_W;
@@ -983,6 +1021,8 @@
   detail->slabs_in_workspace = pl.grid_cap; detail->slab_bytes = (int64_t)pl.ws_per_wg;
   detail->fixed_bytes = (int64_t)(irec::WS_HEAD_BYTES + pl.tab_bytes + pl.gang_bytes);
   detail->exchange_rows = irec::COOP_MAX_BLOCKS; detail->exchange_keys = irec::COOP_KEYS;
+  detail->stream_samples = cd.stream_S1; detail->stream_bytes = 0;
+  for (int q = 0; q < pl.n_tab && cd.stream_S1 > 0; ++q) detail->stream_bytes += (int64_t)irec::team_z1_bytes(p->n_samples, cd.stream_S1, pl.tab_dim[q]);
   return IREC_OK;
 }
 
@@ -1072,18 +1112,18 @@
   A.ws_per_wg = pl.ws_per_wg;
   A.max_dim_pad = pl.dpad;
   A.out_margin = out_margin;
+  const CallDetail cd = call_detail(ctx, pl, p, n_blocks, max_block_dim, out_margin != nullptr);
   irec::TableStamps stamps{};
   if (pl.table)
     for (int q = 0; q < pl.n_tab; ++q) {
       uint32_t *w = stamps.w[q];
-      w[0] = 0x7ab1e000u | ((pl.team || pl.chunk) ? 1u : 2u);
+      w[0] = 0x7ab1e000u | ((pl.team || pl.chunk) ? 1u : 2u) | ((uint32_t)cd.stream_S1 << 4);
       w[1] = (uint32_t)(uint64_t)seed; w[2] = (uint32_t)((uint64_t)seed >> 32);
       w[3] = (uint32_t)p->n_samples; w[4] = (uint32_t)pl.tab_dim[q]; w[5] = (uint32_t)pl.K_tab;
       w[6] = (uint32_t)pl.tab_off[q];
       w[7] = ~(w[1] ^ w[2] ^ w[3] ^ w[4] ^ w[5] ^ w[6]);
     }
   stamps.reuse = (p->flags & IREC_FLAG_REUSE_TABLES) ? 1 : 0;
-  const CallDetail cd = call_detail(ctx, pl, p, n_blocks, max_block_dim, out_margin != nullptr);
   const int split_blocks = cd.split_blocks;
   if (cd.placed) A.row_cost = (const uint32_t *)((char *)workspace + irec::WS_COUNTER_BYTES + irec::WS_XCH_BYTES);
   int grid = (int)std::min<int64_t>(n_blocks, pl.one_grid_cap);
@@ -1105,10 +1145,16 @@
       uint16_t *tab = (uint16_t *)((char *)workspace + irec::WS_HEAD_BYTES + pl.tab_off[q]);
       A.tab[q] = tab; A.tab_dim[q] = pl.tab_dim[q];
       P.jobs.tab[q] = tab; P.jobs.keep[q] = nullptr;
-    }
+      if (cd.stream_S1 > 0) {
+        float *z1 = (float *)((char *)workspace + irec::WS_HEAD_BYTES + pl.z1_off[q]);
+        A.z1[q] = z1; P.z1[q] = z1;
+      }
+    }
+    A.z1_S1 = cd.stream_S1; P.z1_S1 = cd.stream_S1; P.lut2 = ctx->d_lut2;
     if (pl.n_tab > 0 && !(p->flags & IREC_FLAG_TABLES_PRESENT)) {
       P.table_kind = (pl.team || pl.chunk) ? 1 : 2;
       P.n_table_wgs = (int32_t)irec::prep_table_wgs(P.table_kind, p->n_samples, pl.K_tab, pl.n_tab, pl.tab_dim, &P.jobs);
+      if (cd.stream_S1 > 0) P.n_z1_wgs = irec::team_z1_wgs(p->n_samples, cd.stream_S1, pl.n_tab);
     }
   }
   HIP_TRY(irec::launch_prep(P, A, st));
diff --git a/relative-entropy-coding_amd/csrc/irec_internal.h b/relative-entropy-coding_amd/csrc/irec_internal.h
--- a/relative-entropy-coding_amd/csrc/irec_internal.h
+++ b/relative-entropy-coding_amd/csrc/irec_internal.h
@@ -13,6 +13,8 @@
 #define IREC_FLAG_TEST_SPLIT_ORPHAN 32
 #define IREC_FLAG_LISTED_ORDER 262144
 #define IREC_FLAG_NO_TEN 1048576
+#define IREC_FLAG_STREAM_SHIFT (24)
+#define IREC_FLAG_STREAM_MASK (0x7F << IREC_FLAG_STREAM_SHIFT)
 #define IREC_FLAG_SPLIT_SHIFT 12
 #define IREC_FLAG_SPLIT_MASK (0xF << IREC_FLAG_SPLIT_SHIFT)
 #define IREC_FLAG_SHAPE_SHIFT 8
@@ -32,6 +34,8 @@
   int64_t share_first, n_slots;
   int64_t slabs_in_workspace, slab_bytes, fixed_bytes;
   int32_t exchange_rows, exchange_keys;
+  int32_t stream_samples, stream_pad_;
+  int64_t stream_bytes;
 } irec_plan_detail;
 irec_status irec_test_plan(int32_t n_cu, int32_t clock_mhz, const irec_params *p, int64_t n_blocks, int32_t max_block_dim, int32_t max_K,
                            irec_plan_info *info, irec_plan_detail *detail);
diff --git a/relative-entropy-coding_amd/csrc/irec_kernels.h b/relative-entropy-coding_amd/csrc/irec_kernels.h
--- a/relative-entropy-coding_amd/csrc/irec_kernels.h
+++ b/relative-entropy-coding_amd/csrc/irec_kernels.h
@@ -37,6 +37,7 @@
   int32_t coop_beams;
   int32_t coop_test_orphan;
   float *out_margin;
+  const float *z1[4]; int32_t z1_S1;
   unsigned long long *dbg;
 };
 
@@ -68,6 +69,9 @@
 int team_count_for(int B, int S, int shape_override);
 int team_shareable(int B, int S, int shape_override);
 bool team_placeable(int B, int S, int shape_override);
+bool team_streams(int B, int S, int shape_override);
+size_t team_z1_bytes(int S, int S1, int D);
+int team_z1_wgs(int S, int S1, int n);
 int team_waves_for(int B, int S, int shape_override);
 size_t team_ws_extra_for(int B, int S, int shape_override);
 size_t team_ws_bytes_for(int B, int S, int shape_override, int max_K);
@@ -110,6 +114,7 @@
   uint32_t *head; TableStamps ts;
   int32_t n_granule, n_cost, n_table_wgs, table_kind;
   int64_t seed; int32_t S, K_tab; const uint16_t *dlog4r; ChoiceJobs jobs; uint32_t *cost;
+  int32_t n_z1_wgs, z1_S1; float *z1[4]; const float *lut2;
 };
 hipError_t launch_prep(const PrepArgs &P, const EncArgs &A, hipStream_t st);
 int64_t prep_table_wgs(int kind, int32_t S, int32_t K_tab, int n, const int32_t *dims, ChoiceJobs *jobs);
diff --git a/relative-entropy-coding_amd/csrc/irec_team.hip b/relative-entropy-coding_amd/csrc/irec_team.hip
--- a/relative-entropy-coding_amd/csrc/irec_team.hip
+++ b/relative-entropy-coding_amd/csrc/irec_team.hip
@@ -13,6 +13,9 @@
 #endif
 #ifndef IREC_PK_ADDR
 #define IREC_PK_ADDR 1
+#endif
+#ifndef IREC_SLAB_NT
+#define IREC_SLAB_NT 0
 #endif
 #if defined(IREC_TEAM_MARGIN_TU) || defined(IREC_TEAM_GANG_TU)
 #define IREC_TEAM_AUX_TU 1
@@ -53,6 +56,30 @@
 }
 __host__ __device__ inline size_t team_lds_total(int NB, int S, int SP, int teams, bool passes = false, int ps = 0) {
   return T3_BYTES + (size_t)teams * team_lds_one(NB, S, SP, teams, passes, ps);
+}
+
+typedef float slab_f4 __attribute__((ext_vector_type(4)));
+typedef __attribute__((address_space(1))) const char uniform_gchar;
+typedef __attribute__((address_space(1))) const slab_f4 uniform_gf4;
+__device__ __forceinline__ uniform_gchar *uniform_ptr(const void *p) {
+  const uint64_t a = (uint64_t)(uintptr_t)p;
+  const uint32_t lo = (uint32_t)__builtin_amdgcn_readfirstlane((int)(uint32_t)a), hi = (uint32_t)__builtin_amdgcn_readfirstlane((int)(uint32_t)(a >> 32));
+  return (uniform_gchar *)(uintptr_t)(((uint64_t)hi << 32) | lo);
+}
+__device__ __forceinline__ float4 slab_ld4(const float *p) {
+#if IREC_SLAB_NT
+  const slab_f4 v = __builtin_nontemporal_load(reinterpret_cast<const slab_f4 *>(p));
+  return make_float4(v.x, v.y, v.z, v.w);
+#else
+  return *reinterpret_cast<const float4 *>(p);
+#endif
+}
+__device__ __forceinline__ void slab_st4(float *p, float4 v) {
+#if IREC_SLAB_NT
+  __builtin_nontemporal_store((slab_f4){v.x, v.y, v.z, v.w}, reinterpret_cast<slab_f4 *>(p));
+#else
+  *reinterpret_cast<float4 *>(p) = v;
+#endif
 }
 
 #ifdef IREC_TEAM_STAMPS
@@ -78,6 +105,7 @@
   constexpr int SPC = BS >= 2 ? 1 : 20 / NBW;
   constexpr int RW = NBW * SPC;
   constexpr int ACC_ROOM = rsn_room(RW);
+  constexpr bool CAN_STREAM = NB == 20 && TEAMS == 3 && BS == 1 && !PASSES && !ONE && !SHARE && !MARGIN;
   extern __shared__ __attribute__((aligned(16))) char smem[];
   const int S = A.S, B = A.B;
   const int lane = threadIdx.x & 63;
@@ -208,6 +236,12 @@
       if (tid == 0 && qsh == 0) A.out_K[blk] = -1;
       continue;
     }
+    const float *z1t = nullptr;
+    if constexpr (CAN_STREAM) {
+#pragma unroll
+      for (int q = 0; q < 4; ++q)
+        if (A.tab_dim[q] == D && A.z1_S1 > 0) z1t = A.z1[q];
+    }
     const int Dp = (D + 3) & ~3;
     const int NG = (D + 255) >> 8;
     const int NSW = NW / NG;
@@ -297,15 +331,15 @@
     };
     auto park = [&]() {
       if (PARK && active) {
-        *reinterpret_cast<float4 *>(park_g + d0) = make_float4(c[0], c[1], c[2], c[3]);
-        *reinterpret_cast<float4 *>(park_g + FAST_MAX_DIM + d0) = make_float4(sa[0], sa[1], sa[2], sa[3]);
+        slab_st4(park_g + d0, make_float4(c[0], c[1], c[2], c[3]));
+        slab_st4(park_g + FAST_MAX_DIM + d0, make_float4(sa[0], sa[1], sa[2], sa[3]));
       }
     };
     auto unpark = [&]() {
       if (PARK && active) {
         asm volatile("" ::: "memory");
-        const float4 pc = *reinterpret_cast<const float4 *>(park_g + d0);
-        const float4 ps = *reinterpret_cast<const float4 *>(park_g + FAST_MAX_DIM + d0);
+        const float4 pc = slab_ld4(park_g + d0);
+        const float4 ps = slab_ld4(park_g + FAST_MAX_DIM + d0);
         c[0] = pc.x; c[1] = pc.y; c[2] = pc.z; c[3] = pc.w;
         sa[0] = ps.x; sa[1] = ps.y; sa[2] = ps.z; sa[3] = ps.w;
       }
@@ -332,6 +366,7 @@
     bool abandoned = false;
     int cur = 0, Bcur = 1;
     uint32_t bv_cur = 0u;
+    int32_t i1v = 0;
     for (int t = 0; t < K; ++t) {
 #ifdef IREC_TEAM_STAMPS
       st_acc[11] += 1ull;
@@ -361,9 +396,61 @@
           if (m < n_mine) r = *reinterpret_cast<const uint2 *>(tab_tu + ((uint32_t)(s_base + m * NSWe + swe) * (uint32_t)Dp + tab_lo));
           return r;
         };
+        int ch0_ = 0;
+        if constexpr (CAN_STREAM) {
+          const int S1 = A.z1_S1;
+          const int n_str = (t == 1 && z1t != nullptr && nlive == NBW && S1 > s_base + swe) ? min(n_mine, (S1 - s_base - swe + NSWe - 1) / NSWe) : 0;
+          if (n_str > 0) {
+            static_assert(!CAN_STREAM || (RW == 20 && SPC == 1 && NBW == 20), "the streamed step reduces one sample x 20 beams");
+#pragma unroll
+            for (int b = 0; b < NBW; ++b)
+#pragma unroll
+              for (int i = 0; i < 4; ++i) asm volatile("" : "+v"(G[b][i]));
+            constexpr int NR = 5;
+            static_assert(NBW % NR == 0, "the ring turns a whole number of times per sample");
+            uint32_t pl_[NBW];
+#pragma unroll
+            for (int b = 0; b < NBW; ++b) pl_[b] = (uint32_t)__builtin_amdgcn_readlane(i1v, b_lo + b) * (uint32_t)S1 * (uint32_t)Dp;
+            const uint32_t zoff = tab_lo * 4u;
+            slab_f4 zr[NR];
+#define IREC_ZISSUE(SLOT, SO, B) do { uint32_t zo_ = zoff; asm volatile("" : "+v"(zo_)); \
+                                      zr[SLOT] = *(uniform_gf4 *)(uniform_ptr(z1t + (size_t)(pl_[B] + (SO))) + zo_); } while (0)
+            uint32_t so_cur = (uint32_t)(s_base + swe) * (uint32_t)Dp;
+#pragma unroll
+            for (int b = 0; b < NR; ++b) IREC_ZISSUE(b, so_cur, b);
+            __builtin_amdgcn_sched_barrier(0);
+            for (int m = 0; m < n_str; ++m) {
+              const uint32_t so_nxt = (uint32_t)(s_base + (m + 1 < n_str ? m + 1 : m) * NSWe + swe) * (uint32_t)Dp;
+              rs_f2 a20[10];
+#pragma unroll
+              for (int k = 0; k < 10; ++k) a20[k] = (rs_f2){0.f, 0.f};
+#pragma unroll
+              for (int b = 0; b < NBW; ++b) {
+                asm volatile("" : "+v"(zr[b % NR]));
+                const float zv[4] = {zr[b % NR].x, zr[b % NR].y, zr[b % NR].z, zr[b % NR].w};
+                float a = (b & 1) ? a20[b >> 1].y : a20[b >> 1].x;
+#pragma unroll
+                for (int i = 0; i < 4; ++i) a = __builtin_fmaf(__builtin_fmaf(cH[i], zv[i], G[b][i]), zv[i], a);
+                if (b & 1) a20[b >> 1].y = a; else a20[b >> 1].x = a;
+                __builtin_amdgcn_sched_barrier(0);
+                if (b + NR < NBW) IREC_ZISSUE(b % NR, so_cur, b + NR);
+                else IREC_ZISSUE(b % NR, so_nxt, b + NR - NBW);
+                __builtin_amdgcn_sched_barrier(0);
+              }
+              const float tot = reduce_scatter_20(a20, lane);
+              if (rs_p20 >= 0 && (lane & 1) == 0 && rs_p20 < nlive) part_s[((size_t)g * SP + m * NSWe + swe) * PS + b_lo + rs_p20] = tot;
+              so_cur = so_nxt;
+            }
+#pragma unroll
+            for (int b = 0; b < NR; ++b) asm volatile("" : "+v"(zr[b]));
+#undef IREC_ZISSUE
+            ch0_ = n_str;
+          }
+        }
+        const int ch0 = CAN_STREAM ? ch0_ : 0;
         uint2 ap_cur[SPC], ap_nxt[SPC];
 #pragma unroll
-        for (int cc = 0; cc < SPC; ++cc) { ap_cur[cc] = row(cc); ap_nxt[cc] = row(SPC + cc); }
+        for (int cc = 0; cc < SPC; ++cc) { ap_cur[cc] = row(ch0 * SPC + cc); ap_nxt[cc] = row((ch0 + 1) * SPC + cc); }
 #define IREC_AL(CC, I) ((((I) & 2) ? (((I) & 1) ? (ap_cur[CC].y >> 16) : (ap_cur[CC].y & 0xFFFFu)) : (((I) & 1) ? (ap_cur[CC].x >> 16) : (ap_cur[CC].x & 0xFFFFu))) << 2)
         typedef float f2 __attribute__((ext_vector_type(2)));
         constexpr int NP = NBW / 2;
@@ -402,7 +489,7 @@
             for (int i = 0; i < 4; ++i) asm volatile("" : "+v"(G[b][i]));
         }
         IREC_ISSUE(zz[0], IREC_AL(0, 0), 0);
-        for (int ch = 0; ch < n_chunks; ++ch) {
+        for (int ch = ch0; ch < n_chunks; ++ch) {
           if constexpr (BS >= 2) {
             if ((((ch >> 2) + bs) % BS) == 0) __builtin_amdgcn_s_setprio(1);
             else __builtin_amdgcn_s_setprio(0);
@@ -752,6 +839,7 @@
         const int Bupd = last ? 1 : Bnew;
         const int32_t v_sp = sel_s[lane < Bnew ? lane : 0], v_bp = sel_b[lane < Bnew ? lane : 0];
         const uint32_t v_bo = sm->sel_bo[lane < Bnew ? lane : 0];
+        if constexpr (CAN_STREAM) { if (t == 0) i1v = v_sp; }
 #pragma unroll
         for (int j0 = 0; j0 < NBW; j0 += UB) {
           uint2 apv[UB];
@@ -769,7 +857,7 @@
               bet_old[u] = (uint32_t)__builtin_amdgcn_readlane((int)v_bo, j);
               apv[u] = *reinterpret_cast<const uint2 *>(tab_t + (size_t)sp_ * Dp);
 #ifndef IREC_ABLATE_SLAB
-              if (t) obv4[u] = *reinterpret_cast<const float4 *>(bold + (size_t)bp_ * FAST_MAX_DIM);
+              if (t) obv4[u] = slab_ld4(bold + (size_t)bp_ * FAST_MAX_DIM);
 #endif
             }
           }
@@ -808,7 +896,7 @@
                 }
               } else {
 #ifndef IREC_ABLATE_SLAB
-                if (sw == 0) *reinterpret_cast<float4 *>(bnew + (size_t)j * FAST_MAX_DIM) = make_float4(nb[0], nb[1], nb[2], nb[3]);
+                if (sw == 0) slab_st4(bnew + (size_t)j * FAST_MAX_DIM, make_float4(nb[0], nb[1], nb[2], nb[3]));
 #endif
                 if constexpr (LATE_G) {
 #pragma unroll
@@ -1605,6 +1693,31 @@
   }
 }
 
+__device__ __forceinline__ void z1_table_rows(const PrepArgs &P, uint32_t skip, int64_t wg, int64_t n_wg) {
+  const int S = P.S, S1 = P.z1_S1;
+  const int64_t per = (int64_t)S * S1, n_units = per * P.jobs.n;
+  const StepSeed ss = make_step_seed(P.seed + 1);
+  const int quad = (int)threadIdx.x;
+  for (int64_t u = wg; u < n_units; u += n_wg) {
+    const int q = (int)(u / per);
+    if (P.z1[q] == nullptr || ((skip >> q) & 1u)) continue;
+    const int r = (int)(u - (int64_t)q * per), i = r / S1, s = r - i * S1;
+    const int D = P.jobs.D[q], Dp = (D + 3) & ~3;
+    if (4 * quad >= Dp) continue;
+    uint32_t rm1[4];
+    draw_rm1_x4(ss, (uint64_t)s * (uint64_t)D + (uint64_t)(4 * quad), rm1);
+    const uint32_t beta = (uint32_t)P.dlog4r[hash_from_sum(69 * i) - 1u] >> 2;
+    float v[4];
+#pragma unroll
+    for (int k = 0; k < 4; ++k) {
+      uint32_t e = (4 * quad + k < D ? (uint32_t)P.dlog4r[rm1[k]] >> 2 : 0u) + beta;
+      if (e >= IREC_PM1) e -= IREC_PM1;
+      v[k] = P.lut2[e];
+    }
+    *reinterpret_cast<float4 *>(P.z1[q] + ((size_t)(i * S1 + s) * Dp + 4 * quad)) = make_float4(v[0], v[1], v[2], v[3]);
+  }
+}
+
 __global__ __launch_bounds__(256, IREC_CHOICE_WPE) void prep_kernel(PrepArgs P, EncArgs A) {
   const int t = (int)threadIdx.x;
   uint32_t *p = P.head;
@@ -1660,6 +1773,19 @@
     return;
   }
   wg -= P.n_table_wgs;
+  if (wg < P.n_z1_wgs) {
+    uint32_t skip = 0u;
+#pragma unroll
+    for (int q = 0; q < 4; ++q) {
+      bool same = P.ts.reuse != 0 && P.ts.w[q][0] != 0u;
+#pragma unroll
+      for (int k = 0; k < WS_STAMP_WORDS; ++k) same = same && __builtin_nontemporal_load(p + WS_STAMP_WORD + q * WS_STAMP_WORDS + k) == P.ts.w[q][k];
+      skip |= same ? (1u << q) : 0u;
+    }
+    z1_table_rows(P, skip, (int64_t)wg, (int64_t)P.n_z1_wgs);
+    return;
+  }
+  wg -= P.n_z1_wgs;
   if (wg < P.n_cost) {
     CostRow cr;
     cost_row_issue(A, wg, t, cr);
@@ -1712,6 +1838,12 @@
   const TeamShape sh = team_shape(B, S, ovr);
   return sh.nb == 20 && sh.teams == 2 && sh.bs == 1 && !sh.passes && !sh.one;
 }
+bool team_streams(int B, int S, int ovr) {
+  const TeamShape sh = team_shape(B, S, ovr);
+  return sh.nb == 20 && sh.teams == 3 && sh.bs == 1 && !sh.passes && !sh.one && B == 20 && S >= 20;
+}
+size_t team_z1_bytes(int S, int S1, int D) { return (size_t)S * S1 * ((D + 3) & ~3) * 4; }
+int team_z1_wgs(int S, int S1, int n) { return (int)std::min<int64_t>((int64_t)S * S1 * n, 2048); }
 int team_waves_for(int B, int S, int ovr) { const TeamShape sh = team_shape(B, S, ovr); return sh.teams * sh.bs * TEAM_NW; }
 size_t team_ws_extra_for(int B, int S, int ovr) {
   const TeamShape sh = team_shape(B, S, ovr);
@@ -1926,7 +2058,7 @@
   return end;
 }
 hipError_t launch_prep(const PrepArgs &P, const EncArgs &A, hipStream_t st) {
-  const int64_t grid = 1 + (int64_t)P.n_granule + P.n_table_wgs + P.n_cost;
+  const int64_t grid = 1 + (int64_t)P.n_granule + P.n_table_wgs + P.n_z1_wgs + P.n_cost;
   hipLaunchKernelGGL(prep_kernel, dim3((unsigned)grid), dim3(256), 0, st, P, A);
   return hipGetLastError();
 }
diff --git a/relative-entropy-coding_amd/irec/_lib.py b/relative-entropy-coding_amd/irec/_lib.py
--- a/relative-entropy-coding_amd/irec/_lib.py
+++ b/relative-entropy-coding_amd/irec/_lib.py
@@ -22,6 +22,7 @@
 IREC_FLAG_NO_TEN = 1048576
 IREC_FLAG_TABLES_PRESENT = 65536
 IREC_FLAG_REUSE_TABLES = 64
+IREC_FLAG_STREAM_SHIFT = 24
 IREC_FLAG_SHAPE_SHIFT = 8
 IREC_FLAG_SHAPE = {"default": 0, "2": 2 << 8, "3": 3 << 8, "1x2": 5 << 8, "team": 6 << 8}
 IREC_TABLE_STEPS_DEFAULT = 32
@@ -65,7 +66,8 @@
     _fields_ = [("kind", ctypes.c_int32), ("grid", ctypes.c_int32), ("teams_per_wg", ctypes.c_int32), ("coop_width", ctypes.c_int32),
                 ("coop_beams", ctypes.c_int32), ("gang_chunks", ctypes.c_int32), ("placed", ctypes.c_int32), ("split_blocks", ctypes.c_int32),
                 ("share_first", ctypes.c_int64), ("n_slots", ctypes.c_int64), ("slabs_in_workspace", ctypes.c_int64),
-                ("slab_bytes", ctypes.c_int64), ("fixed_bytes", ctypes.c_int64), ("exchange_rows", ctypes.c_int32), ("exchange_keys", ctypes.c_int32)]
+                ("slab_bytes", ctypes.c_int64), ("fixed_bytes", ctypes.c_int64), ("exchange_rows", ctypes.c_int32), ("exchange_keys", ctypes.c_int32),
+                ("stream_samples", ctypes.c_int32), ("stream_pad_", ctypes.c_int32), ("stream_bytes", ctypes.c_int64)]
 
     def as_dict(self):
         return {name: int(getattr(self, name)) for name, _ in self._fields_}
```
